# LucaAmbrogioni/Brancher

Measured on AMD Instinct MI355X. Metric: ELBO iters/sec at num_samples=300 per GPU (300-sample-equivalent iterations, whole job), higher is better.
Workload: dtype f32

## Files before the change

brancher_amd/csrc/bsvi_internal.h:

```cpp
#pragma once
#include <hip/hip_runtime.h>
#include <stdint.h>
#include <string>
#include <vector>

#include "bsvi.h"

int bsvi_fail(int code, const std::string& msg);
#define BSVI_CHECK_STRUCT(ptr, type)                                                                              \
    do {                                                                                                          \
        if ((ptr)->struct_size != sizeof(type))                                                                   \
            return bsvi_fail(BSVI_ERR_INVALID, std::string(#type "::struct_size is ") + std::to_string((ptr)->struct_size) + \
                             ", this library's sizeof is " + std::to_string(sizeof(type)) +                       \
                             ": the binding was written against another revision of include/bsvi.h");             \
    } while (0)
int bsvi_xgemm_nt(const uint16_t* X, const int32_t* rows, const uint16_t* Wp, long plane_stride, float* C, int ldc,
                  int M, int N, int Kp, void* stream);

int bsvi_xgemm_nt_t(const uint16_t* X, const int32_t* rows, const uint16_t* Wp, long plane_stride, float* Ct, int ldct,
                    int M, int N, int Kp, void* stream);
int bsvi_gemm_f32(int mode, const float* A, int lda, const float* B, int ldb, float* C, int ldc, int M, int N, int K, void* stream);

namespace bsvi_spec { struct Spec; }

struct bsvi_program {
    bsvi_program_desc d;
    void* dev_blob = nullptr;
    const uint4* code = nullptr;
    const uint4* aux = nullptr;
    const bsvi_record* records = nullptr;
    const bsvi_uniform_entry* uniform = nullptr;
    const float* consts = nullptr;
    const uint32_t* pu_ptr = nullptr;
    const uint32_t* pu_idx = nullptr;
    int max_lds = 0;
    bool generic = false;
    const bsvi_program* shares[8] = {};
    uint32_t n_shares = 0;
    bsvi_spec::Spec* spec = nullptr;
};

namespace bsvi_spec {

enum Mode { MODE_SUMS = 0, MODE_STEP = 1, MODE_LOOP = 2 };

Spec* create(const bsvi_program_desc& desc, std::string& why);
void destroy(Spec* s);
int upload(Spec* s);
const std::string& source(const Spec* s, int variant);
int compile(const std::string& src, std::vector<char>& code, std::string& log);
int obtain(const std::string& src, std::vector<char>& code, std::string& log, int* origin);
int last_origin();
std::string cache_directory();
std::string compiler_identity();
size_t workspace_bytes(const Spec* s, uint32_t n_local);
bool applies(const Spec* s, uint32_t n_local, int mode);
struct Launch {
    const bsvi_elbo_args* a = nullptr;
    int mode = MODE_SUMS;
    const bsvi_opt_cfg* cfg = nullptr;
    float* params = nullptr;
    float* state = nullptr;
    const uint8_t* mask = nullptr;
    const uint8_t* mask_first = nullptr;
    uint32_t pretraining_iterations = 0, n_iterations = 1;
    float* loss_slot = nullptr;
    float* finite_slot = nullptr;
    void* workspace = nullptr;
    const void* xchg = nullptr;
};
int launch(Spec* s, const bsvi_program* p, const Launch& L);
void geometry(const Spec* s, uint32_t n_local, int mode, uint32_t* n_blocks, uint32_t* n_threads, uint32_t* lds_bytes);

}

const void* bsvi_exchange_descriptor(bsvi_exchange* x, uint32_t n);
```

brancher_amd/csrc/elbo_kernel.hip:

```cpp
#include <hip/hip_runtime.h>
#include <stdint.h>
#include <stdio.h>
#include <stdlib.h>
#include <stdarg.h>
#include <string.h>
#include <mutex>
#include <type_traits>
#include <string>
#include <vector>

#include "bsvi.h"
#include "bsvi_device.h"
#include "bsvi_internal.h"

namespace bsvi {


struct KParams {
    const uint4* code;
    const uint4* aux;
    const bsvi_uniform_entry* uniform;
    const float* consts;
    const float* params;
    const float* obs;
// ... 1880 lines not shown
    for (uint32_t v = 0; v < n_shares; ++v) {
        if (!shares[v]) return fail(BSVI_ERR_INVALID, "null program share");
        if (shares[v]->d.n_uniform != p->d.n_uniform || shares[v]->d.n_uniform_grad != p->d.n_uniform_grad ||
            shares[v]->d.n_slots != p->d.n_slots || shares[v]->d.n_params != p->d.n_params ||
            shares[v]->d.n_code > p->d.n_code || (shares[v]->generic && !p->generic))
            return fail(BSVI_ERR_INVALID, "a program share does not match the program's tables");
    }
    for (uint32_t v = 0; v < n_shares; ++v) p->shares[v] = shares[v];
    p->n_shares = n_shares;
    return BSVI_OK;
}

extern "C" int bsvi_persistent_split_shares(const bsvi_program* p, uint32_t n_local) {
    if (!p || !n_local || !multi_persistent_applies(p, n_local)) return 1;
    if (p->spec && bsvi_spec::applies(p->spec, n_local, bsvi_spec::MODE_LOOP)) return 1;
    const char* e = getenv("BSVI_PERSISTENT_SHARES");
    const uint32_t waves = (n_local + 63) / 64;
    uint32_t want = e ? (uint32_t)atoi(e) : 2u;
    if (want > 8) want = 8;
    while (want > 1 && (waves * want > kMaxMultiWg || want == 5 || want == 7)) --want;
    return (int)(want < 1 ? 1 : want);
}

extern "C" int bsvi_train_persistent_split(const bsvi_program* p, const bsvi_program* const* shares, uint32_t n_shares,
                                           const bsvi_elbo_args* a, const bsvi_opt_cfg* cfg,
                                           float* params_dev, float* state_dev, const uint8_t* active_mask_dev,
                                           const uint8_t* active_mask_first_dev, uint32_t pretraining_iterations,
                                           uint32_t n_iterations, float* loss_curve_dev, float* finite_dev) {
    if (a) BSVI_CHECK_STRUCT(a, bsvi_elbo_args);
    if (!shares || n_shares < 2 || n_shares > 8) return fail(BSVI_ERR_INVALID, "2..8 program shares expected");
    for (uint32_t v = 0; v < n_shares; ++v) {
        if (!shares[v]) return fail(BSVI_ERR_INVALID, "null program share");
        if (shares[v]->d.n_uniform != p->d.n_uniform || shares[v]->d.n_uniform_grad != p->d.n_uniform_grad ||
            shares[v]->d.n_slots != p->d.n_slots || shares[v]->d.n_params != p->d.n_params ||
            shares[v]->d.n_code > p->d.n_code || (shares[v]->generic && !p->generic))
            return fail(BSVI_ERR_INVALID, "a program share does not match the program's tables");
    }
    return train_persistent_impl(p, shares, n_shares, a, cfg, params_dev, state_dev, active_mask_dev, active_mask_first_dev,
                                 pretraining_iterations, n_iterations, loss_curve_dev, finite_dev);
}

static int train_persistent_impl(const bsvi_program* p, const bsvi_program* const* shares, uint32_t n_shares,
                                 const bsvi_elbo_args* a, const bsvi_opt_cfg* cfg,
                                 float* params_dev, float* state_dev, const uint8_t* active_mask_dev,
                                 const uint8_t* active_mask_first_dev, uint32_t pretraining_iterations,
                                 uint32_t n_iterations, float* loss_curve_dev, float* finite_dev) {
    if (!p || !a) return fail(BSVI_ERR_INVALID, "null argument");
    int rc = check_cfg(cfg);
    if (rc) return rc;
    if (!a->out_dev || !params_dev || !active_mask_dev || !active_mask_first_dev || !loss_curve_dev || !finite_dev)
        return fail(BSVI_ERR_INVALID, "null argument");
    if (a->n_samples_local != a->n_samples_global) return fail(BSVI_ERR_INVALID, "persistent trainer is the single-GPU path");
    if (a->offset_dev) return fail(BSVI_ERR_INVALID, "the in-kernel training loop counts its own iterations: offset_dev must be null");
    {
        const int sp = try_spec(p, a, bsvi_spec::MODE_LOOP, cfg, params_dev, state_dev, active_mask_dev, active_mask_first_dev,
                                pretraining_iterations, n_iterations, loss_curve_dev, finite_dev);
        if (sp) return sp < 0 ? sp : BSVI_OK;
    }
    if (!state_dev) return fail(BSVI_ERR_INVALID, "state_dev is null and this call does not run on the specialised kernel");
    const bool multi = multi_persistent_applies(p, a->n_samples_local);
    Geometry g = choose_geometry(p, a->n_samples_local, true);
    if (multi && g.n_blocks != 1) {
        g = Geometry();
        g.n_waves = (a->n_samples_local + 63) / 64; g.n_blocks = 1; g.mode = SM_LACC; g.lpw = 64;
    }
    if (g.n_blocks != 1) return fail(BSVI_ERR_RESOURCE, "sample count does not fit one workgroup");
    PParams P;
    memset(&P, 0, sizeof(P));
    bsvi_elbo_args aa = *a;
    aa.params_dev = params_dev;
    rc = fill_kparams(p, &aa, g, P.K);
    if (rc) return rc;
    fill_rparams(p, g, P.K, params_dev, a->out_dev, P.R);
    P.R.state = state_dev; P.R.active_mask = active_mask_dev; P.R.cfg = *cfg; P.R.do_finalize = 1; P.R.do_step = 1;
    P.n_iterations = n_iterations; P.loss_curve = loss_curve_dev; P.finite_curve = finite_dev;
    P.active_mask_first = active_mask_first_dev; P.pretraining_iterations = pretraining_iterations;
    hipStream_t st = (hipStream_t)a->stream;
    if (shares && !multi) return fail(BSVI_ERR_INVALID, "program shares need the multi-workgroup trainer");
    if (multi) {
        const uint32_t sample_waves = g.n_waves;
        const uint32_t n_wg = sample_waves * (shares ? n_shares : 1u);
        if (n_wg > kMaxMultiWg) return fail(BSVI_ERR_INVALID, "too many workgroups for the exchange region");
        if (shares) {
            P.n_shares = n_shares;
            for (uint32_t v = 0; v < n_shares; ++v) {
                P.share_code[v] = shares[v]->code; P.share_aux[v] = shares[v]->aux; P.share_n_code[v] = shares[v]->d.n_code;
            }
        }
        Geometry g1 = g;
        g1.n_waves = 1; g1.n_blocks = n_wg;
        g1.stash = !p->generic && lds_need(p, 1, SM_LACC, 64, true) <= (size_t)p->max_lds;
        g1.lds_bytes = lds_need(p, 1, SM_LACC, 64, g1.stash);
        g1.n_pad = n_wg * 64;
        rc = fill_kparams(p, &aa, g1, P.K);
        if (rc) return rc;
        char* region = (char*)a->workspace_dev + base_ws_bytes(p, a->n_samples_local);
        P.mw_counter = (uint32_t*)region;
        P.mw_xchg = (float*)(region + 256);
        P.mw_params = P.mw_xchg + mw_xchg_floats(p);
        P.mw_stride = mw_stride(p);
        P.mw_state = P.mw_params + (size_t)(kMaxMultiWg - 1) * P.mw_stride;
        HIP_TRY(hipMemsetAsync(region, 0, 256 + mw_xchg_floats(p) * sizeof(float), st));
        dim3 mgrid(n_wg), mblock(64);
        if (p->generic) hipLaunchKernelGGL((persistent_multi_kernel<SM_LACC, true>), mgrid, mblock, g1.lds_bytes, st, P);
        else hipLaunchKernelGGL((persistent_multi_kernel<SM_LACC, false>), mgrid, mblock, g1.lds_bytes, st, P);
        HIP_TRY(hipGetLastError());
        return BSVI_OK;
    }
    dim3 grid(1), block(g.n_waves * 64);
#define BSVI_LAUNCH_P(SM_, GEN_) hipLaunchKernelGGL((persistent_kernel<SM_, GEN_>), grid, block, g.lds_bytes, st, P)
    if (p->generic) {
        if (g.mode == SM_LACC) BSVI_LAUNCH_P(SM_LACC, true); else if (g.mode == SM_ZG) BSVI_LAUNCH_P(SM_ZG, true); else BSVI_LAUNCH_P(SM_WSUM, true);
    } else {
        if (g.mode == SM_LACC) BSVI_LAUNCH_P(SM_LACC, false); else if (g.mode == SM_ZG) BSVI_LAUNCH_P(SM_ZG, false); else BSVI_LAUNCH_P(SM_WSUM, false);
    }
#undef BSVI_LAUNCH_P
    HIP_TRY(hipGetLastError());
    return BSVI_OK;
}

extern "C" size_t bsvi_program_source(const bsvi_program_desc* desc, int variant, char* buf, size_t capacity) {
    if (validate(desc) != BSVI_OK) return 0;
    std::string why;
    bsvi_spec::Spec* sp = bsvi_spec::create(*desc, why);
    if (!sp) { fail(BSVI_ERR_UNSUPPORTED, "program not specialised: " + why); return 0; }
    const std::string& src = bsvi_spec::source(sp, variant);
    const size_t need = src.size() + 1;
    if (buf && capacity >= need) memcpy(buf, src.c_str(), need);
    bsvi_spec::destroy(sp);
    return need;
}

extern "C" int bsvi_jit_compile(const char* source, size_t* code_bytes) {
    if (!source) return fail(BSVI_ERR_INVALID, "null source");
    std::vector<char> code;
    std::string log;
    const int rc = bsvi_spec::compile(source, code, log);
    if (rc) return fail(rc, log);
    if (code_bytes) *code_bytes = code.size();
    return BSVI_OK;
}

extern "C" int bsvi_jit_load(const char* source, size_t* code_bytes, int* origin) {
    if (!source) return fail(BSVI_ERR_INVALID, "null source");
    std::vector<char> code;
    std::string log;
    const int rc = bsvi_spec::obtain(source, code, log, origin);
    if (rc) return fail(rc, log);
    if (code_bytes) *code_bytes = code.size();
    return BSVI_OK;
}

extern "C" int bsvi_jit_last_origin(void) { return bsvi_spec::last_origin(); }

extern "C" size_t bsvi_jit_cache_dir(char* buf, size_t capacity) {
    const std::string dir = bsvi_spec::cache_directory();
    if (buf && capacity > dir.size()) memcpy(buf, dir.c_str(), dir.size() + 1);
    return dir.size() + 1;
}

extern "C" size_t bsvi_jit_compiler_identity(char* buf, size_t capacity) {
    const std::string id = bsvi_spec::compiler_identity();
    if (buf && capacity > id.size()) memcpy(buf, id.c_str(), id.size() + 1);
    return id.size() + 1;
}

extern "C" int bsvi_program_engine(const bsvi_program* p, uint32_t n_local, int mode, uint32_t* n_blocks, uint32_t* n_threads,
                                   uint32_t* lds_bytes) {
    if (!p) return 0;
    if (!p->spec || !bsvi_spec::applies(p->spec, n_local, mode)) return 0;
    bsvi_spec::geometry(p->spec, n_local, mode, n_blocks, n_threads, lds_bytes);
    return 1;
}

extern "C" int bsvi_max_lds_bytes(const bsvi_program* p) { return p ? p->max_lds : 0; }

extern "C" int bsvi_query_geometry(const bsvi_program* p, uint32_t n_local, uint32_t* n_blocks, uint32_t* n_waves,
                                   uint32_t* zglobal, uint64_t* lds_bytes) {
    if (!p) return fail(BSVI_ERR_INVALID, "null argument");
    Geometry g = choose_geometry(p, n_local, false);
    if (!g.n_blocks) return fail(BSVI_ERR_RESOURCE, "program does not fit the LDS budget");
    if (n_blocks) *n_blocks = g.n_blocks;
    if (n_waves) *n_waves = g.n_waves;
    if (zglobal) *zglobal = (uint32_t)g.mode | (g.lpw << 8);
    if (lds_bytes) *lds_bytes = g.lds_bytes;
    return BSVI_OK;
}

extern "C" int bsvi_debug_math(int fn, int dist, const float* x_dev, const float* p0_dev, const float* p1_dev,
                               float* out_dev, uint32_t n, void* stream) {
    if (!x_dev || !p0_dev || !p1_dev || !out_dev || !n) return fail(BSVI_ERR_INVALID, "null argument");
    hipLaunchKernelGGL(debug_math_kernel, dim3((n + 127) / 128), dim3(128), 0, (hipStream_t)stream, fn, dist, x_dev,
                       p0_dev, p1_dev, out_dev, n);
    HIP_TRY(hipGetLastError());
    return BSVI_OK;
}

#include "dense_kernel.inc"
#include "bnn_kernel.inc"

namespace bsvi {
__global__ void __launch_bounds__(256) minibatch_gather_kernel(const float* dataset, uint32_t DS, uint32_t row, uint32_t B, const int32_t* indices_in,
                                                                uint32_t seed_lo, uint32_t seed_hi, uint32_t off_lo, uint32_t off_hi, float* dst, int32_t* indices_out) {
    const uint32_t i = blockIdx.x * 256u + threadIdx.x;
    if (i >= B * row) return;
    const uint32_t b = i / row, e = i - b * row;
    DParams Dm;
    Dm.indices_in = indices_in; Dm.DS = DS;
    Dm.offset_lo = off_lo; Dm.offset_hi = off_hi; Dm.seed_lo = seed_lo; Dm.seed_hi = seed_hi;
    const uint32_t r = minibatch_index(Dm, b);
    dst[i] = dataset[(size_t)r * row + e];
    if (indices_out && e == 0u) indices_out[b] = (int32_t)r;
}
}

extern "C" int bsvi_minibatch_gather(const float* dataset_dev, uint32_t dataset_size, uint32_t row_floats, uint32_t batch_size,
                                     const int32_t* indices_dev, uint64_t seed, uint64_t offset, float* dst_dev, int32_t* indices_out_dev,
                                     void* stream) {
    if (!dataset_dev || !dst_dev || !dataset_size || !row_floats || !batch_size) return fail(BSVI_ERR_INVALID, "null argument");
    if (batch_size > dataset_size) return fail(BSVI_ERR_INVALID, "bsvi_minibatch_gather: batch_size exceeds dataset_size");
    if ((uint64_t)batch_size * row_floats >= (1ull << 31)) return fail(BSVI_ERR_RESOURCE, "bsvi_minibatch_gather: minibatch too large");
    const uint32_t n = batch_size * row_floats;
    hipLaunchKernelGGL(bsvi::minibatch_gather_kernel, dim3((n + 255) / 256), dim3(256), 0, (hipStream_t)stream, dataset_dev, dataset_size,
                       row_floats, batch_size, indices_dev, (uint32_t)seed, (uint32_t)(seed >> 32), (uint32_t)offset, (uint32_t)(offset >> 32),
                       dst_dev, indices_out_dev);
    HIP_TRY(hipGetLastError());
    return BSVI_OK;
}
```

brancher_amd/csrc/spec_main.h:

```cpp
#pragma once

namespace bsvi {

#if defined(__HIP_DEVICE_COMPILE__)
#define SPEC_CONST_AS __attribute__((address_space(4)))
#define SPEC_RELOAD_ARGS() asm volatile("" : "+s"(ka))
#else
#define SPEC_CONST_AS
#define SPEC_RELOAD_ARGS()
#endif

#define SPEC_TAB_PTR (4 * SPEC_N_UNIFORM)
#define SPEC_TAB_POS (SPEC_TAB_PTR + SPEC_N_PARAMS + 1)
#define SPEC_TAB_IDX (SPEC_TAB_POS + SPEC_N_POS)
#define SPEC_TAB_MASK (SPEC_TAB_IDX + SPEC_N_POS)

__device__ __forceinline__ void spec_lds_barrier() {
#if defined(__HIP_DEVICE_COMPILE__)
    asm volatile("s_waitcnt lgkmcnt(0)\n\ts_barrier" ::: "memory");
#endif
}

__device__ __noinline__ float spec_utransform_rare(uint32_t t, float x) { return utransform((int)t, x); }
__device__ __noinline__ float spec_utransform_grad_rare(uint32_t t, float x) { return utransform_grad((int)t, x); }
#ifndef SPEC_RARE_TRANSFORMS
#define SPEC_RARE_TRANSFORMS 1
#endif
#ifndef SPEC_UT_MASK
#define SPEC_UT_MASK 0xFFu
#endif
__device__ __forceinline__ float utransform_common(uint32_t t, float x) {
#if SPEC_RARE_TRANSFORMS
    if (t > BSVI_UT_SIGMOID) return spec_utransform_rare(t, x);
#endif
    const float soft = ((SPEC_UT_MASK >> BSVI_UT_SOFTPLUS) & 1u) ? softplusf_(x) : x;
    const float sig = ((SPEC_UT_MASK >> BSVI_UT_SIGMOID) & 1u) ? sigmoidf_(x) : x;
    return t == BSVI_UT_IDENTITY ? x : (t == BSVI_UT_SOFTPLUS ? soft : sig);
}
__device__ __forceinline__ float spec_utransform_grad(uint32_t t, float x) {
#if SPEC_RARE_TRANSFORMS
    if (t > BSVI_UT_SIGMOID) return spec_utransform_grad_rare(t, x);
#endif
    const float s = spec_rcp(1.0f + __expf(-x));
    const float soft = x > 20.0f ? 1.0f : s;
    return t == BSVI_UT_IDENTITY ? 1.0f : (t == BSVI_UT_SOFTPLUS ? soft : s * (1.0f - s));
}
__device__ __forceinline__ void spec_store_uniform(uint32_t k, float u) {
    spec_lds[k] = u;
    spec_lds[SPEC_OFF_UR + k] = spec_rcp(u);
    spec_lds[SPEC_OFF_UL + k] = spec_log(u);
}
__device__ __forceinline__ void spec_publish_uniform(const uint32_t* TAB, uint32_t k, float x) {
    const uint32_t w1 = TAB[4 * k + 1];
    spec_store_uniform(k, __uint_as_float(TAB[4 * k + 2]) + __uint_as_float(TAB[4 * k + 3]) * utransform_common(w1 & 0xFFu, x));
}

struct SpecOwn {
    float theta, s0, s1, s2, st;
    float a[2], b[2];
    uint32_t pos[2], k[2], tr[2];
    uint32_t n, mask;
    double p1, p2;
};
__device__ __forceinline__ void spec_own_store_products(spec_f4* row, const SpecOwn& o) {
    const unsigned long long a = __double_as_longlong(o.p1), b = __double_as_longlong(o.p2);
    row[4] = spec_f4{__uint_as_float((uint32_t)a), __uint_as_float((uint32_t)(a >> 32)), __uint_as_float((uint32_t)b), __uint_as_float((uint32_t)(b >> 32))};
}
__device__ __forceinline__ void spec_own_store(spec_f4* row, const SpecOwn& o) {
    row[0] = spec_f4{o.theta, o.s0, o.s1, o.s2};
    row[1] = spec_f4{o.st, o.a[0], o.b[0], o.a[1]};
    row[2] = spec_f4{o.b[1], __uint_as_float(o.pos[0]), __uint_as_float(o.pos[1]), __uint_as_float(o.k[0])};
    row[3] = spec_f4{__uint_as_float(o.k[1]), __uint_as_float(o.tr[0] | (o.tr[1] << 8) | (o.n << 16) | (o.mask << 24)), 0.0f, 0.0f};
    spec_own_store_products(row, o);
}
__device__ __forceinline__ SpecOwn spec_own_load(const spec_f4* row) {
    const spec_f4 q0 = row[0], q1 = row[1], q2 = row[2], q3 = row[3], q4 = row[4];
    SpecOwn o;
    o.p1 = __longlong_as_double((long long)(((unsigned long long)__float_as_uint(q4.y) << 32) | __float_as_uint(q4.x)));
    o.p2 = __longlong_as_double((long long)(((unsigned long long)__float_as_uint(q4.w) << 32) | __float_as_uint(q4.z)));
    o.theta = q0.x; o.s0 = q0.y; o.s1 = q0.z; o.s2 = q0.w;
    o.st = q1.x; o.a[0] = q1.y; o.b[0] = q1.z; o.a[1] = q1.w;
    o.b[1] = q2.x; o.pos[0] = __float_as_uint(q2.y); o.pos[1] = __float_as_uint(q2.z); o.k[0] = __float_as_uint(q2.w);
    o.k[1] = __float_as_uint(q3.x);
    const uint32_t meta = __float_as_uint(q3.y);
    o.tr[0] = meta & 0xFFu; o.tr[1] = (meta >> 8) & 0xFFu; o.n = (meta >> 16) & 0xFFu; o.mask = meta >> 24;
    return o;
}

#if defined(SPEC_WITH_EXCHANGE) && !SPEC_DIAG && !SPEC_ACCUMULATE_CHUNKS
#define SPEC_EXCHANGE 1
__device__ __forceinline__ unsigned long long* spec_xentry(unsigned char* region, uint32_t parity, uint32_t r, uint32_t capacity, uint32_t world) {
    return reinterpret_cast<unsigned long long*>(region + XCHG_HEADER_WORDS * 4 + (size_t)2 * world * capacity * 4) + ((size_t)parity * world + r) * capacity;
}
__device__ __forceinline__ void spec_xput(const SpecExchange* xg, uint32_t seq, uint32_t k, float v) {
    const uint32_t world = xg->world, rank = xg->rank, cap = xg->capacity, parity = seq & 1u;
    const unsigned long long e = ((unsigned long long)seq << 32) | __float_as_uint(v);
    for (uint32_t p = 0; p < world; ++p)
        __hip_atomic_store(spec_xentry(xg->peer[p], parity, rank, cap, world) + k, e, __ATOMIC_RELAXED, __HIP_MEMORY_SCOPE_SYSTEM);
}
__device__ __forceinline__ bool spec_xget(const SpecExchange* xg, uint32_t seq, uint32_t k, float& v) {
    const uint32_t world = xg->world, rank = xg->rank, cap = xg->capacity, parity = seq & 1u;
    unsigned char* const region = xg->peer[rank];
    uint32_t* const abort_word = reinterpret_cast<uint32_t*>(region) + XCHG_MAX_RANKS * XCHG_FLAG_STRIDE;
    unsigned long long t0 = 0;
    for (uint32_t round = 0;; ++round) {
        unsigned long long e[XCHG_MAX_RANKS];
#pragma unroll
        for (uint32_t r = 0; r < XCHG_MAX_RANKS; ++r) {
            e[r] = (unsigned long long)seq << 32;
            if (r < world) e[r] = __hip_atomic_load(spec_xentry(region, parity, r, cap, world) + k, __ATOMIC_RELAXED, __HIP_MEMORY_SCOPE_SYSTEM);
        }
        bool all = true;
        float t = 0.0f;
#pragma unroll
        for (uint32_t r = 0; r < XCHG_MAX_RANKS; ++r) {
            all = all && (uint32_t)(e[r] >> 32) == seq;
            if (r < world) t += __uint_as_float((uint32_t)e[r]);
        }
        if (all) {
            v = t;
            return __hip_atomic_load(abort_word, __ATOMIC_RELAXED, __HIP_MEMORY_SCOPE_SYSTEM) == 0u;
        }
        if (round == 0u) t0 = wall_clock64();
        if (__hip_atomic_load(abort_word, __ATOMIC_RELAXED, __HIP_MEMORY_SCOPE_SYSTEM) != 0u) return false;
        if (wall_clock64() - t0 > xg->timeout_ticks) {
            for (uint32_t p = 0; p < world; ++p)
                __hip_atomic_store(reinterpret_cast<uint32_t*>(xg->peer[p]) + XCHG_MAX_RANKS * XCHG_FLAG_STRIDE, seq, __ATOMIC_RELAXED, __HIP_MEMORY_SCOPE_SYSTEM);
            return false;
        }
        __builtin_amdgcn_s_sleep(1);
    }
}
#if !SPEC_GENERIC_OWNERS
__device__ __forceinline__ bool spec_exchange(const SpecExchange* xg, uint32_t seq, uint32_t l, bool has_param, float& vs, float& vb, float& gsum) {
    const uint32_t world = xg->world, rank = xg->rank, cap = xg->capacity, parity = seq & 1u;
    uint32_t* const abort_word = reinterpret_cast<uint32_t*>(xg->peer[rank]) + XCHG_MAX_RANKS * XCHG_FLAG_STRIDE;
    const uint32_t aborted = __hip_atomic_load(abort_word, __ATOMIC_RELAXED, __HIP_MEMORY_SCOPE_SYSTEM);
    const unsigned long long tag = (unsigned long long)seq << 32;
    for (uint32_t p = 0; p < world; ++p) {
        unsigned long long* const row = spec_xentry(xg->peer[p], parity, rank, cap, world);
        if (l == 0u) {
            __hip_atomic_store(row, tag | __float_as_uint(vs), __ATOMIC_RELAXED, __HIP_MEMORY_SCOPE_SYSTEM);
            __hip_atomic_store(row + 1, tag | __float_as_uint(vb), __ATOMIC_RELAXED, __HIP_MEMORY_SCOPE_SYSTEM);
        }
        if (has_param) __hip_atomic_store(row + BSVI_OUT_HEADER + l, tag | __float_as_uint(gsum), __ATOMIC_RELAXED, __HIP_MEMORY_SCOPE_SYSTEM);
    }
    unsigned char* const region = xg->peer[rank];
    unsigned long long t0 = 0;
    bool gave_up = false;
    float ts, tb, tg;
    for (uint32_t round = 0;; ++round) {
        unsigned long long e0[XCHG_MAX_RANKS], e1[XCHG_MAX_RANKS], eg[XCHG_MAX_RANKS];
#pragma unroll
        for (uint32_t r = 0; r < XCHG_MAX_RANKS; ++r) {
            e0[r] = e1[r] = eg[r] = tag;
            if (r < world) {
                const unsigned long long* const row = spec_xentry(region, parity, r, cap, world);
                e0[r] = __hip_atomic_load(row, __ATOMIC_RELAXED, __HIP_MEMORY_SCOPE_SYSTEM);
                e1[r] = __hip_atomic_load(row + 1, __ATOMIC_RELAXED, __HIP_MEMORY_SCOPE_SYSTEM);
                if (has_param) eg[r] = __hip_atomic_load(row + BSVI_OUT_HEADER + l, __ATOMIC_RELAXED, __HIP_MEMORY_SCOPE_SYSTEM);
            }
        }
        bool all = true;
        ts = 0.0f; tb = 0.0f; tg = 0.0f;
#pragma unroll
        for (uint32_t r = 0; r < XCHG_MAX_RANKS; ++r) {
            all = all && (uint32_t)(e0[r] >> 32) == seq && (uint32_t)(e1[r] >> 32) == seq && (uint32_t)(eg[r] >> 32) == seq;
            if (r < world) { ts += __uint_as_float((uint32_t)e0[r]); tb += __uint_as_float((uint32_t)e1[r]); tg += __uint_as_float((uint32_t)eg[r]); }
        }
        if (__all((int)all)) break;
        if (round == 0u) t0 = wall_clock64();
        if (__hip_atomic_load(abort_word, __ATOMIC_RELAXED, __HIP_MEMORY_SCOPE_SYSTEM) != 0u) { gave_up = true; break; }
        if (wall_clock64() - t0 > xg->timeout_ticks) {
            gave_up = true;
            if (l < world) __hip_atomic_store(reinterpret_cast<uint32_t*>(xg->peer[l]) + XCHG_MAX_RANKS * XCHG_FLAG_STRIDE, seq, __ATOMIC_RELAXED, __HIP_MEMORY_SCOPE_SYSTEM);
            if (l == 0u) atomicAdd(abort_word + 1, 1u);
            break;
        }
        __builtin_amdgcn_s_sleep(1);
    }
    if (gave_up || aborted != 0u) return false;
    vs = ts; vb = tb; gsum = tg;
    return true;
}
#endif
#else
#define SPEC_EXCHANGE 0
#endif

#if defined(SPEC_WAVES_PER_EU)
#define SPEC_VGPR_ATTR __attribute__((amdgpu_waves_per_eu(SPEC_WAVES_PER_EU, SPEC_WAVES_PER_EU)))
#elif defined(SPEC_NUM_VGPR)
#define SPEC_VGPR_ATTR __attribute__((amdgpu_num_vgpr(SPEC_NUM_VGPR)))
#else
#define SPEC_VGPR_ATTR
#endif
#ifndef SPEC_BOUND_THREADS
#define SPEC_BOUND_THREADS SPEC_MAX_THREADS
#endif
extern "C" __global__ void __launch_bounds__(SPEC_BOUND_THREADS) SPEC_VGPR_ATTR bsvi_spec_kernel(const SpecArgs A_unused) {
    (void)A_unused;
    const SPEC_CONST_AS char* ka = (const SPEC_CONST_AS char*)__builtin_amdgcn_kernarg_segment_ptr();
#define SPEC_A ((const SPEC_CONST_AS SpecArgs*)ka)
    const uint32_t tid = threadIdx.x, nthreads = blockDim.x, W = nthreads >> 6, wave = tid >> 6, lane = tid & 63u;
    const uint32_t G = gridDim.x;
    float* const WS = spec_lds + SPEC_OFF_WS;
    float* const RED = spec_lds + SPEC_OFF_RED;
    float* const PS = spec_lds + SPEC_OFF_PS;
    uint32_t* const TAB = reinterpret_cast<uint32_t*>(spec_lds + SPEC_OFF_TAB);
    float* const WSw = WS + wave * SPEC_WS_PAD;

    SpecLane T;
    T.lane = lane;
    T.n = blockIdx.x * nthreads + tid;
    T.active = false; T.nc = 0; T.nidx = 0;
    T.vz = T.n >> 31;
    T.tile = wave * SPEC_TR_FLOATS + lane;
    const uint32_t sample_base = SPEC_A->sample_base;
    const uint32_t n_chunks = (SPEC_A->n_local + G * nthreads - 1u) / (G * nthreads);
    const uint32_t mode = SPEC_A->mode;
    const bool step = mode != SPEC_MODE_SUMS;
    const uint32_t n_it = (mode == SPEC_MODE_LOOP) ? SPEC_A->n_iterations : 1u;

    {
        const uint32_t* uniform = reinterpret_cast<const uint32_t*>(SPEC_A->uniform);
        const uint32_t* pu_ptr = SPEC_A->pu_ptr;
        const uint32_t* pu_pos = SPEC_A->pu_pos;
        const uint32_t* pu_idx = SPEC_A->pu_idx;
        const float* obs = SPEC_A->obs;
        const float* params = SPEC_A->params;
        const float* state = SPEC_A->state;
        const uint8_t* mask = SPEC_A->mask;
        const uint8_t* mask_first = SPEC_A->mask_first;
        const bool h_uni = tid < 4u * SPEC_N_UNIFORM, h_ptr = tid < SPEC_N_PARAMS + 1u, h_pos = tid < SPEC_N_POS,
                   h_obs = tid < SPEC_N_OBS, h_par = tid < SPEC_N_PARAMS;
        uint32_t r_uni = 0, r_ptr = 0, r_pos = 0, r_idx = 0, r_mask = 0;
        float r_obs = 0.0f, r_par = 0.0f, r_st[4] = {0.0f, 0.0f, 0.0f, 0.0f};
        const bool h_uni2 = tid + nthreads < 4u * SPEC_N_UNIFORM;
        uint32_t r_uni2 = 0;
        if (h_uni) r_uni = uniform[tid];
        if (h_uni2) r_uni2 = uniform[tid + nthreads];
        if (h_ptr) r_ptr = pu_ptr[tid];
        if (h_pos) { r_pos = pu_pos[tid]; r_idx = pu_idx[tid]; }
        if (h_obs) r_obs = obs[tid];
        if (h_par) {
            r_par = params[tid];
            if (step) {
                if (state) {
#pragma unroll
                    for (uint32_t s = 0; s < 4u; ++s) r_st[s] = state[(size_t)s * SPEC_N_PARAMS + tid];
                }
                r_mask = (mask[tid] ? 1u : 0u) | (mask_first[tid] ? 2u : 0u);
            }
        }
        asm volatile("" ::: "memory");
        if (h_uni) TAB[tid] = r_uni;
        if (h_uni2) TAB[tid + nthreads] = r_uni2;
        if (h_ptr) TAB[SPEC_TAB_PTR + tid] = r_ptr;
        if (h_pos) { TAB[SPEC_TAB_POS + tid] = r_pos; TAB[SPEC_TAB_IDX + tid] = r_idx; }
        if (h_obs) spec_lds[SPEC_N_UNIFORM + tid] = r_obs;
        if (h_par) {
            PS[tid] = r_par;
            if (step) {
#pragma unroll
                for (uint32_t s = 0; s < 4u; ++s) PS[(1u + s) * SPEC_NP_PAD + tid] = r_st[s];
                TAB[SPEC_TAB_MASK + tid] = r_mask;
            }
        }
        for (uint32_t i = tid + 2u * nthreads; i < 4u * SPEC_N_UNIFORM; i += nthreads) TAB[i] = uniform[i];
        for (uint32_t i = tid + nthreads; i < SPEC_N_PARAMS + 1u; i += nthreads) TAB[SPEC_TAB_PTR + i] = pu_ptr[i];
        for (uint32_t j = tid + nthreads; j < SPEC_N_POS; j += nthreads) { TAB[SPEC_TAB_POS + j] = pu_pos[j]; TAB[SPEC_TAB_IDX + j] = pu_idx[j]; }
        for (uint32_t i = tid + nthreads; i < SPEC_N_OBS; i += nthreads) spec_lds[SPEC_N_UNIFORM + i] = obs[i];
        for (uint32_t i = tid + nthreads; i < SPEC_N_PARAMS; i += nthreads) {
            PS[i] = params[i];
            if (step) {
#pragma unroll
                for (uint32_t s = 0; s < 4u; ++s)
                    PS[(1u + s) * SPEC_NP_PAD + i] = state ? state[(size_t)s * SPEC_N_PARAMS + i] : 0.0f;
                TAB[SPEC_TAB_MASK + i] = (mask[i] ? 1u : 0u) | (mask_first[i] ? 2u : 0u);
            }
        }
        __syncthreads();
        const float* consts = SPEC_A->consts;
        for (uint32_t k = tid; k < SPEC_N_UNIFORM; k += nthreads) {
            const uint32_t src = TAB[4 * k], w1 = TAB[4 * k + 1];
            spec_publish_uniform(TAB, k, ((w1 >> 8) & 0xFFu) ? PS[src] : consts[src]);
        }
    }

    spec_f4* const OWN = reinterpret_cast<spec_f4*>(spec_lds + SPEC_OFF_OWN);
#ifndef SPEC_OWNER_WAVE
#define SPEC_OWNER_WAVE 1u
#endif
#if SPEC_TILE && SPEC_KEEP_NOISE && SPEC_KEEP_NOISE <= 68 && !SPEC_GENERIC_OWNERS && !SPEC_DIAG && !SPEC_ACCUMULATE_CHUNKS \
    && !defined(SPEC_DEBUG_NO_DRAW) && !defined(SPEC_NO_EARLY_DRAW) && !defined(SPEC_DEBUG_LATE_FREE) && defined(SPEC_WITH_DRAW_WAVE)
#define SPEC_DRAW_WAVE 1
    const uint32_t WSN = (SPEC_A->n_local + 63u) / 64u;
    const bool has_draw_wave = mode == SPEC_MODE_LOOP && G == 1u && W >= 2u && WSN < W;
    const uint32_t fed_index = W == 2u ? 0u : 1u;
    const bool draw_service = has_draw_wave && W - WSN >= 3u;
    const bool draw_wave = __builtin_amdgcn_readfirstlane((has_draw_wave && (draw_service ? wave >= WSN : wave == W - 1u)) ? 1 : 0) != 0;
    const bool fed_wave = __builtin_amdgcn_readfirstlane((has_draw_wave && (draw_service ? wave < WSN : wave == fed_index)) ? 1 : 0) != 0;
    float* const NZ = spec_lds + SPEC_OFF_TR + (draw_service ? WSN * SPEC_TR_FLOATS + wave * (SPEC_KEEP_NOISE * 64u) : (W - 1u) * SPEC_TR_FLOATS) + lane;
    float* const NZB = spec_lds + SPEC_OFF_TR + WSN * SPEC_TR_FLOATS + lane;
    if (draw_wave) for (uint32_t k = lane; k < SPEC_WS_PAD; k += 64u) WSw[k] = 0.0f;
#else
#define SPEC_DRAW_WAVE 0
    const bool has_draw_wave = false, draw_wave = false, fed_wave = false;
    const uint32_t fed_index = 1u;
#endif
#if SPEC_DRAW_WAVE && defined(SPEC_WITH_DRAW_OWNERS) && !SPEC_EXCHANGE
#define SPEC_DRAW_OWNERS 1
    const uint32_t own_wave = WSN + ((1u - WSN) & 3u);
#else
#define SPEC_DRAW_OWNERS 0
#endif
#if SPEC_DRAW_OWNERS
    const uint32_t own_base = own_wave * 64u;
#else
    const uint32_t own_base = has_draw_wave ? fed_index * 64u
                            : (!SPEC_GENERIC_OWNERS && SPEC_OWNER_WAVE * 64u + SPEC_N_PARAMS <= nthreads) ? SPEC_OWNER_WAVE * 64u : 0u;
#endif
    const uint32_t oid = tid - own_base;
    bool own_fast = false;
#if SPEC_DRAW_OWNERS
    SpecOwn own = {};
#endif
    if (oid < SPEC_N_PARAMS) {
        const uint32_t j0 = TAB[SPEC_TAB_PTR + oid], j1 = TAB[SPEC_TAB_PTR + oid + 1];
        if (j1 - j0 <= 2u) {
            own_fast = true;
#if !SPEC_DRAW_OWNERS
            SpecOwn own;
#endif
            own.n = j1 - j0;
            own.mask = 0;
            own.theta = PS[oid];
            own.s0 = own.s1 = own.s2 = own.st = 0.0f;
            own.p1 = own.p2 = 1.0;
            own.a[0] = own.a[1] = own.b[0] = own.b[1] = 0.0f;
            own.pos[0] = own.pos[1] = own.k[0] = own.k[1] = own.tr[0] = own.tr[1] = 0;
            if (step) {
                own.s0 = PS[SPEC_NP_PAD + oid]; own.s1 = PS[2 * SPEC_NP_PAD + oid];
                own.s2 = PS[3 * SPEC_NP_PAD + oid]; own.st = PS[4 * SPEC_NP_PAD + oid];
                own.mask = TAB[SPEC_TAB_MASK + oid];
                const bsvi_opt_cfg cfg0 = SPEC_A->cfg;
                if (cfg0.kind != BSVI_OPT_SGD && own.st != 0.0f) {
                    own.p1 = pow((double)cfg0.beta1, (double)own.st);
                    own.p2 = pow((double)cfg0.beta2, (double)own.st);
                }
            }
#pragma unroll
            for (uint32_t e = 0; e < 2u; ++e) {
                if (e < own.n) {
                    const uint32_t k = TAB[SPEC_TAB_IDX + j0 + e];
                    own.pos[e] = TAB[SPEC_TAB_POS + j0 + e];
                    own.k[e] = k;
                    own.tr[e] = TAB[4 * k + 1] & 0xFFu;
                    own.a[e] = __uint_as_float(TAB[4 * k + 2]);
                    own.b[e] = __uint_as_float(TAB[4 * k + 3]);
                }
            }
#if !SPEC_DRAW_OWNERS
            spec_own_store(OWN + 5 * oid, own);
#endif
        }
    }

    SPEC_RELOAD_ARGS();
    SpecBody B0;
    B0.n_local = SPEC_A->n_local;
    B0.seed_lo = SPEC_A->seed_lo;
    B0.seed_hi = SPEC_A->seed_hi;
#if SPEC_DIAG
    B0.noise = SPEC_A->noise;
    B0.samples_out = SPEC_A->samples_out;
    B0.noise_out = SPEC_A->noise_out;
    B0.fvalue_out = SPEC_A->fvalue_out;
    B0.f_weight = SPEC_A->f_weight;
    B0.q_weight = SPEC_A->q_weight;
#else
    B0.noise = nullptr; B0.samples_out = nullptr; B0.noise_out = nullptr; B0.fvalue_out = nullptr;
    B0.f_weight = nullptr; B0.q_weight = nullptr;
#endif
    unsigned long long off0 = ((unsigned long long)SPEC_A->offset_hi << 32) | SPEC_A->offset_lo;
    if (const unsigned long long* const offset_dev = SPEC_A->offset_dev) off0 += *offset_dev;
    const uint32_t n_global = SPEC_A->n_global;
    const uint32_t pretraining = SPEC_A->pretraining_iterations;
#if SPEC_ACCUMULATE_CHUNKS
#define SPEC_LOOP_MANY 1
#define SPEC_GEN_OVER 0x7fff0000u
    const unsigned int gen0 = 0;
    if (G > 1 && mode == SPEC_MODE_LOOP && blockIdx.x != 0 &&
        __hip_atomic_load(SPEC_A->ticket + 64, __ATOMIC_RELAXED, __HIP_MEMORY_SCOPE_AGENT) >= SPEC_GEN_OVER) return;
#else
#define SPEC_LOOP_MANY 0
#endif
#if SPEC_EXCHANGE
    uint32_t xseq0 = 0;
    if (const SpecExchange* const xg0 = SPEC_A->xchg) xseq0 = reinterpret_cast<const uint32_t*>(xg0->peer[xg0->rank])[XCHG_CALLS_WORD + 1];
#endif

#if defined(SPEC_DEBUG_STAMPS)
    unsigned long long stamp[12] = {0, 0, 0, 0, 0, 0, 0, 0, 0, 0, 0, 0};
#define SPEC_STAMP(i) if (it == n_it / 2) stamp[i] = __builtin_amdgcn_s_memtime()
    unsigned long long rstamp[6] = {0, 0, 0, 0, 0, 0};
#define SPEC_RSTAMP(i) if (it == n_it / 2) rstamp[i] = __builtin_amdgcn_s_memtime()
#define SPEC_RSTAMP_NEXT() if (it == n_it / 2 + 1u) rstamp[5] = __builtin_amdgcn_s_memtime()
#define SPEC_RSTAMP_WRITE()                                                                                              \
    if (lane == 0u && SPEC_A->loss_slot && n_it > 16u + 8u * SPEC_MAX_WAVES) {                                           \
        asm volatile("s_waitcnt vmcnt(0)" ::: "memory");                                                                 \
        for (int i = 1; i < 6; ++i) SPEC_A->loss_slot[16u + 8u * wave + i] = (float)(rstamp[i] - rstamp[0]);               \
        SPEC_A->loss_slot[16u + 8u * wave] = 1.0f;                                                                       \
    }
#else
#define SPEC_STAMP(i)
#define SPEC_RSTAMP(i)
#define SPEC_RSTAMP_NEXT()
#define SPEC_RSTAMP_WRITE()
#endif
#if SPEC_KEEP_NOISE && !SPEC_DIAG && !SPEC_ACCUMULATE_CHUNKS && !defined(SPEC_DEBUG_NO_DRAW) && !defined(SPEC_NO_EARLY_DRAW)
#define SPEC_EARLY_DRAW 1
    SpecNoise Z;
    bool noise_ready = false;
#else
#define SPEC_EARLY_DRAW 0
#endif
#if SPEC_DRAW_WAVE
    if (draw_service && draw_wave) {
        if (lane == 0u) { RED[8 + 2 * wave] = 0.0f; RED[9 + 2 * wave] = 0.0f; }
        const uint32_t n_draw = W - WSN, k = wave - WSN;
        const uint32_t first = k;
        uint32_t before = 0;
        for (uint32_t j = 0; j < k; ++j) before += (((WSN + j) & 3u) != 1u) ? 1u : 0u;
        const uint32_t second = n_draw + before;
        const bool has_first = first < WSN, has_second = (wave & 3u) != 1u && second < WSN;
        auto draw_for = [&](uint32_t target, unsigned long long offn, SpecNoise& Zd) {
            SpecLane Tn = T;
            Tn.n = target * 64u + lane;
            Tn.active = Tn.n < B0.n_local;
            Tn.nc = Tn.active ? Tn.n : (B0.n_local - 1u);
            Tn.nidx = sample_base + Tn.nc;
            Tn.off_lo = (uint32_t)offn;
            Tn.off_hi = (uint32_t)(offn >> 32);
            Tn.vz = T.vz;
            spec_draw(B0, Tn, Zd);
        };
#if SPEC_DRAW_OWNERS
        (void)has_first; (void)has_second;
        const uint32_t kown = own_wave - WSN, n_other = n_draw - 1u, rest = WSN - 1u;
        const uint32_t j = k < kown ? k : k - 1u, per = rest / n_other, extra = rest % n_other;
        const uint32_t set_a = __builtin_amdgcn_readfirstlane(1u + j * per + (j < extra ? j : extra));
        const uint32_t n_sets = __builtin_amdgcn_readfirstlane(per + (j < extra ? 1u : 0u));
        const bool owners = __builtin_amdgcn_readfirstlane(wave == own_wave ? 1 : 0) != 0;
        for (uint32_t it = 0; it < n_it; ++it) {
            const bool more = it + 1u < n_it, last = !more;
            spec_lds_barrier();
            SPEC_RSTAMP(0);
            SPEC_RSTAMP_NEXT();
            SpecNoise Za, Zb;
            float fac[2] = {0.0f, 0.0f};
            AdamBias bias = {1.0, 1.0, 0.0f, 0.0f};
            if (owners) {
                SPEC_RELOAD_ARGS();
                const bsvi_opt_cfg cfg = SPEC_A->cfg;
#pragma unroll
                for (uint32_t e = 0; e < 2u; ++e) fac[e] = own.b[e] * spec_utransform_grad(own.tr[e], own.theta);
                if (cfg.kind != BSVI_OPT_SGD) bias = optimizer_adam_bias(cfg, own.p1, own.p2);
                if (more) {
                    draw_for(0u, off0 + it + 1u, Za);
                    float* const buf = NZB + (((it + 1u) & 1u) ? WSN * (SPEC_KEEP_NOISE * 64u) : 0u);
#pragma unroll
                    for (uint32_t r = 0; r < SPEC_KEEP_NOISE; ++r) buf[64u * r] = Za.z[r];
                }
            } else if (more) {
                draw_for(set_a, off0 + it + 1u, Za);
                if (n_sets > 1u) draw_for(set_a + 1u, off0 + it + 1u, Zb);
            }
            SPEC_RSTAMP(1);
            spec_lds_barrier();
            SPEC_RSTAMP(2);
            if (owners) {
                SPEC_RELOAD_ARGS();
                float* const out = SPEC_A->out;
                float* const loss_slot = SPEC_A->loss_slot;
                float* const finite_slot = SPEC_A->finite_slot;
                const bsvi_opt_cfg cfg = SPEC_A->cfg;
                float vs = 0.0f, vb = 0.0f;
#pragma unroll
                for (uint32_t w = 0; w < SPEC_MAX_WAVES; ++w) {
                    const float a = RED[8 + 2 * w], b = RED[9 + 2 * w];
                    vs += w < W ? a : 0.0f;
                    vb += w < W ? b : 0.0f;
                }
                float tot[2];
#pragma unroll
                for (uint32_t e = 0; e < 2u; ++e) tot[e] = spec_pos_total(WS, own.pos[e], W);
                const float finite = isfinite(vs) ? 1.0f : 0.0f;
                const float loss = -vs / (float)n_global;
                if (oid == 0u) {
                    if (last) { out[0] = vs; out[1] = vb; out[2] = loss; out[3] = finite; }
                    if (loss_slot) loss_slot[it] = loss;
                    if (finite_slot) finite_slot[it] = finite;
                }
                const float scale = -1.0f / (float)n_global;
                const uint32_t mask_bit = it <= pretraining ? 2u : 1u;
                if (own_fast) {
                    float gsum = 0.0f;
#pragma unroll
                    for (uint32_t e = 0; e < 2u; ++e) {
                        const float term = tot[e] * fac[e];
                        gsum += e < own.n ? term : 0.0f;
                    }
                    const float grad = gsum * scale;
                    SPEC_RSTAMP(3);
                    if (last) out[BSVI_OUT_HEADER + oid] = grad;
                    if (finite != 0.0f && (own.mask & mask_bit)) {
                        if (cfg.kind == BSVI_OPT_SGD) {
                            optimizer_apply(cfg, own.theta, own.s0, own.s1, own.s2, own.st, grad);
                        } else {
                            optimizer_apply_adam_biased(cfg, own.theta, own.s0, own.s1, own.s2, own.st, grad, bias);
                            own.p1 = bias.p1;
                            own.p2 = bias.p2;
                        }
                    }
                    if (last) {
                        float* const params = SPEC_A->params;
                        float* const state = SPEC_A->state;
                        params[oid] = own.theta;
                        if (state) {
                            state[oid] = own.s0;
                            state[(size_t)SPEC_N_PARAMS + oid] = own.s1;
                            state[2 * (size_t)SPEC_N_PARAMS + oid] = own.s2;
                            state[3 * (size_t)SPEC_N_PARAMS + oid] = own.st;
                        }
                    } else {
                        const float g0 = utransform_common(own.tr[0], own.theta);
                        float g1 = g0;
                        if (own.n == 2u && own.tr[1] != own.tr[0]) g1 = utransform_common(own.tr[1], own.theta);
                        if (own.n > 0u) spec_store_uniform(own.k[0], own.a[0] + own.b[0] * g0);
                        if (own.n > 1u) spec_store_uniform(own.k[1], own.a[1] + own.b[1] * g1);
                    }
                }
            } else if (more) {
#pragma unroll
                for (uint32_t r = 0; r < SPEC_KEEP_NOISE; ++r) NZB[set_a * (SPEC_KEEP_NOISE * 64u) + 64u * r] = Za.z[r];
                if (n_sets > 1u) {
#pragma unroll
                    for (uint32_t r = 0; r < SPEC_KEEP_NOISE; ++r) NZB[(set_a + 1u) * (SPEC_KEEP_NOISE * 64u) + 64u * r] = Zb.z[r];
                }
            }
            SPEC_RSTAMP(4);
        }
        SPEC_RSTAMP_WRITE();
        return;
#else
        for (uint32_t it = 0; it < n_it; ++it) {
            const bool more = it + 1u < n_it;
            spec_lds_barrier();
            SPEC_RSTAMP(0);
            SPEC_RSTAMP_NEXT();
            SpecNoise Za;
            if (more && has_first) draw_for(first, off0 + it + 1u, Za);
            SPEC_RSTAMP(1);
            spec_lds_barrier();
            SPEC_RSTAMP(2);
            if (more) {
                if (has_first) {
#pragma unroll
                    for (uint32_t r = 0; r < SPEC_KEEP_NOISE; ++r) NZB[first * (SPEC_KEEP_NOISE * 64u) + 64u * r] = Za.z[r];
                }
                if (has_second) {
                    SpecNoise Zb;
                    draw_for(second, off0 + it + 1u, Zb);
#pragma unroll
                    for (uint32_t r = 0; r < SPEC_KEEP_NOISE; ++r) NZB[second * (SPEC_KEEP_NOISE * 64u) + 64u * r] = Zb.z[r];
                }
            }
            SPEC_RSTAMP(4);
        }
        SPEC_RSTAMP_WRITE();
        return;
#endif
    }
#endif
    for (uint32_t it = 0; it < n_it; ++it) {
        SPEC_STAMP(0);
        float lane_value = 0.0f, lane_bad = 0.0f;
        for (uint32_t chunk = 0; chunk < n_chunks; ++chunk) {
            SpecBody B = B0;
#if SPEC_DIAG
            if (B.noise) B.noise += (size_t)it * SPEC_N_NOISE * B.n_local;
#endif
            T.n = (chunk * G + blockIdx.x) * nthreads + tid;
            T.active = T.n < B.n_local;
            T.nc = T.active ? T.n : (B.n_local - 1u);
            T.nidx = sample_base + T.nc;
            const unsigned long long off = off0 + it;
            T.f = 0.0f;
            T.lq = 0.0f;
#if SPEC_DIAG
            T.gw = B.f_weight ? B.f_weight[T.nc] : 1.0f;
#else
            T.gw = 1.0f;
#endif
            T.off_lo = (uint32_t)off;
            T.off_hi = (uint32_t)(off >> 32);
#if !SPEC_EARLY_DRAW
            SpecNoise Z;
#endif
#if defined(SPEC_DEBUG_NO_DRAW)
            for (uint32_t r = 0; r < (SPEC_KEEP_NOISE ? SPEC_KEEP_NOISE : 1); ++r) Z.z[r] = 0.25f;
#elif SPEC_EARLY_DRAW
#if defined(SPEC_DEBUG_LATE_FREE)
            if (!noise_ready && (!((SPEC_DEBUG_LATE_FREE >> wave) & 1u) || it == 0u)) spec_draw(B, T, Z);
#else
            if (!noise_ready && !draw_wave && !(fed_wave && it > 0u)) spec_draw(B, T, Z);
#endif
#else
            spec_draw(B, T, Z);
#endif
            SPEC_STAMP(1);
            if (chunk == 0) {
                spec_lds_barrier();
                SPEC_RSTAMP(0);
                SPEC_RSTAMP_NEXT();
#if SPEC_ACCUMULATE_CHUNKS
                for (uint32_t k = lane; k < SPEC_WS_CELLS; k += 64u) WSw[k] = 0.0f;
#endif
            }
#if SPEC_DRAW_WAVE
            if (fed_wave && it > 0u) {
#if SPEC_DRAW_OWNERS
                const float* const nz = NZ + ((wave == 0u && (it & 1u)) ? WSN * (SPEC_KEEP_NOISE * 64u) : 0u);
#else
                const float* const nz = NZ;
#endif
#pragma unroll
                for (uint32_t r = 0; r < SPEC_KEEP_NOISE; ++r) Z.z[r] = nz[64u * r];
            }
#endif
            SPEC_STAMP(2);
#if !defined(SPEC_DEBUG_NO_BODY)
            if (!draw_wave) {
                spec_body(B, T, Z, WSw);
#if SPEC_TILE
                spec_du_flush(spec_lds + SPEC_OFF_TR + wave * SPEC_TR_FLOATS, WSw, lane);
#endif
            }
#endif
            SPEC_STAMP(3);
            const float value = (SPEC_ESTIMATOR == BSVI_EST_BLACKBOX) ? (T.lq * T.f + T.f) : T.f;
            lane_value += T.active ? value : 0.0f;
            lane_bad += (T.active && !isfinite(value)) ? 1.0f : 0.0f;
        }
        const float vsum = wave_sum(lane_value);
        const float bad = wave_sum(lane_bad);
        if (lane == 0) { RED[8 + 2 * wave] = vsum; RED[9 + 2 * wave] = bad; }
        SPEC_STAMP(4);
#if SPEC_EARLY_DRAW
        noise_ready = false;
#ifndef SPEC_EARLY_MASK
#define SPEC_EARLY_MASK (1u | (1u << SPEC_OWNER_WAVE))
#endif
#if defined(SPEC_DEBUG_LATE_FREE)
        if (((SPEC_EARLY_MASK >> wave) & 1u) && !((SPEC_DEBUG_LATE_FREE >> wave) & 1u) && n_chunks == 1u && it + 1u < n_it) {
#else
        if (((SPEC_EARLY_MASK >> wave) & 1u) && !has_draw_wave && n_chunks == 1u && it + 1u < n_it) {
#endif
            const unsigned long long off = off0 + it + 1u;
            SpecLane Tn = T;
            Tn.off_lo = (uint32_t)off;
            Tn.off_hi = (uint32_t)(off >> 32);
            spec_draw(B0, Tn, Z);
            noise_ready = true;
        }
#endif
        SPEC_RSTAMP(1);
        spec_lds_barrier();
        SPEC_STAMP(5);
        SPEC_RSTAMP(2);
#if SPEC_DRAW_OWNERS
        SPEC_RSTAMP(4);
        continue;
#endif
#if SPEC_DRAW_WAVE
        if (draw_wave && it + 1u < n_it) {
            const unsigned long long off = off0 + it + 1u;
            SpecLane Tn = T;
            Tn.n = fed_index * 64u + lane;
            Tn.active = Tn.n < B0.n_local;
            Tn.nc = Tn.active ? Tn.n : (B0.n_local - 1u);
            Tn.nidx = sample_base + Tn.nc;
            Tn.off_lo = (uint32_t)off;
            Tn.off_hi = (uint32_t)(off >> 32);
            SpecNoise Zf;
            spec_draw(B0, Tn, Zf);
#pragma unroll
            for (uint32_t r = 0; r < SPEC_KEEP_NOISE; ++r) NZ[64u * r] = Zf.z[r];
        }
#endif

        uint32_t rows = W;
        if (G > 1) {
            SPEC_RELOAD_ARGS();
            float* const partials = SPEC_A->partials;
            unsigned int* const ticket = SPEC_A->ticket;
            const uint32_t stride = 2u + SPEC_N_POS;
            float* mine = partials + (size_t)blockIdx.x * stride;
            for (uint32_t k = tid; k < SPEC_N_POS; k += nthreads) mine[2 + k] = spec_pos_total(WS, k, W);
            if (tid == 0) {
                float s = 0.0f, c = 0.0f;
                for (uint32_t w = 0; w < W; ++w) { s += RED[8 + 2 * w]; c += RED[9 + 2 * w]; }
                mine[0] = s;
                mine[1] = c;
            }
            __syncthreads();
#if SPEC_LOOP_MANY
            if (mode == SPEC_MODE_LOOP) {
                unsigned int* const gen = ticket + 64;
                const unsigned int target = gen0 + it + 1u;
                if (blockIdx.x != 0) {
                    if (tid == 0) {
                        __hip_atomic_fetch_add(ticket, 1u, __ATOMIC_RELEASE, __HIP_MEMORY_SCOPE_AGENT);
                        const unsigned long long t0 = wall_clock64();
                        unsigned int seen;
                        bool over = false;
                        while ((int)((seen = __hip_atomic_load(gen, __ATOMIC_ACQUIRE, __HIP_MEMORY_SCOPE_AGENT)) - target) < 0) {
                            if (wall_clock64() - t0 > 400000000ull) { over = true; break; }
                            __builtin_amdgcn_s_sleep(2);
                        }
                        RED[3] = (over || seen >= SPEC_GEN_OVER) ? 1.0f : 0.0f;
                    }
                    __syncthreads();
                    if (RED[3] != 0.0f) return;
                    if (it + 1u == n_it) return;
                    float* const params = SPEC_A->params;
                    for (uint32_t i = tid; i < SPEC_N_PARAMS; i += nthreads)
                        PS[i] = __hip_atomic_load(params + i, __ATOMIC_RELAXED, __HIP_MEMORY_SCOPE_AGENT);
                    __syncthreads();
                    const float* const consts = SPEC_A->consts;
                    (void)consts;
                    for (uint32_t k = tid; k < SPEC_N_UNIFORM; k += nthreads) {
                        const uint32_t src = TAB[4 * k], w1 = TAB[4 * k + 1];
                        if ((w1 >> 8) & 0xFFu) spec_publish_uniform(TAB, k, PS[src]);
                    }
                    continue;
                }
                if (tid == 0) {
                    const unsigned long long t0 = wall_clock64();
                    bool late = false;
                    while (__hip_atomic_load(ticket, __ATOMIC_ACQUIRE, __HIP_MEMORY_SCOPE_AGENT) != G - 1u) {
                        if (wall_clock64() - t0 > 400000000ull) { late = true; break; }
                        __builtin_amdgcn_s_sleep(2);
                    }
                    RED[3] = late ? 1.0f : 0.0f;
                }
                __syncthreads();
                if (RED[3] != 0.0f) {
                    SPEC_RELOAD_ARGS();
                    float* const loss_slot = SPEC_A->loss_slot;
                    float* const finite_slot = SPEC_A->finite_slot;
                    float* const out = SPEC_A->out;
                    const float nanv = __int_as_float(0x7fc00000);
                    for (uint32_t k = it + tid; k < n_it; k += nthreads) {
                        if (loss_slot) loss_slot[k] = nanv;
                        if (finite_slot) finite_slot[k] = 0.0f;
                    }
                    if (tid == 0) {
                        out[0] = nanv; out[1] = 1.0f; out[2] = nanv; out[3] = 0.0f;
                        __hip_atomic_store(ticket, 0u, __ATOMIC_RELAXED, __HIP_MEMORY_SCOPE_AGENT);
                        __hip_atomic_store(gen, SPEC_GEN_OVER, __ATOMIC_RELEASE, __HIP_MEMORY_SCOPE_AGENT);
                    }
                    return;
                }
            } else
#endif
            {
                if (tid == 0) {
                    const unsigned int t = __hip_atomic_fetch_add(ticket, 1u, __ATOMIC_ACQ_REL, __HIP_MEMORY_SCOPE_AGENT);
                    RED[2] = (t == G - 1u) ? 1.0f : 0.0f;
                }
                __syncthreads();
                if (RED[2] == 0.0f) return;
            }
            float* const SL = spec_lds + SPEC_OFF_SCR;
            for (uint32_t i = tid; i < 4u * stride; i += nthreads) {
                const uint32_t sl = i & 3u, c = i >> 2;
                float s = 0.0f;
                uint32_t b = sl;
                for (; b + 28u < G; b += 32u) {
                    float v[8];
#pragma unroll
                    for (uint32_t u = 0; u < 8u; ++u)
                        v[u] = __hip_atomic_load(&partials[(size_t)(b + 4u * u) * stride + c], __ATOMIC_RELAXED, __HIP_MEMORY_SCOPE_AGENT);
#pragma unroll
                    for (uint32_t u = 0; u < 8u; ++u) s += v[u];
                }
                for (; b < G; b += 4u)
                    s += __hip_atomic_load(&partials[(size_t)b * stride + c], __ATOMIC_RELAXED, __HIP_MEMORY_SCOPE_AGENT);
                SL[i] = s;
            }
            __syncthreads();
            for (uint32_t c = tid; c < stride; c += nthreads) {
                const float s = (SL[4 * c] + SL[4 * c + 1]) + (SL[4 * c + 2] + SL[4 * c + 3]);
                if (c < 2u) {
                    RED[8 + c] = s;
                } else {
                    WS[SPEC_WS_CELL(c - 2u)] = s;
#if !SPEC_TILE
                    WS[4u * (c - 2u) + 1u] = 0.0f; WS[4u * (c - 2u) + 2u] = 0.0f; WS[4u * (c - 2u) + 3u] = 0.0f;
#endif
                }
            }
            if (tid == 0) {
                __hip_atomic_store(ticket, 0u, __ATOMIC_RELAXED, __HIP_MEMORY_SCOPE_AGENT);
            }
            __syncthreads();
            rows = 1;
        }

        SPEC_RELOAD_ARGS();
        float* const out = SPEC_A->out;
        float* const loss_slot = SPEC_A->loss_slot;
        float* const finite_slot = SPEC_A->finite_slot;
        const bsvi_opt_cfg cfg = SPEC_A->cfg;
        float vs = 0.0f, vb = 0.0f;
#pragma unroll
        for (uint32_t w = 0; w < SPEC_MAX_WAVES; ++w) {
            const float a = RED[8 + 2 * w], b = RED[9 + 2 * w];
            vs += w < rows ? a : 0.0f;
            vb += w < rows ? b : 0.0f;
        }
#if SPEC_EXCHANGE
        const SpecExchange* const xg = SPEC_A->xchg;
#if SPEC_GENERIC_OWNERS
        const bool xrun = xg != nullptr && mode == SPEC_MODE_LOOP;
        float xgsum = 0.0f;
        if (xrun) {
            const uint32_t xseq = xseq0 + it + 1u;
            if (tid == own_base) { spec_xput(xg, xseq, 0u, vs); spec_xput(xg, xseq, 1u, vb); }
            if (own_fast) {
                const SpecOwn own = spec_own_load(OWN + 5 * oid);
                float g = 0.0f;
#pragma unroll
                for (uint32_t e = 0; e < 2u; ++e) {
                    const float term = spec_pos_total(WS, own.pos[e], rows) * (own.b[e] * spec_utransform_grad(own.tr[e], own.theta));
                    g += e < own.n ? term : 0.0f;
                }
                spec_xput(xg, xseq, BSVI_OUT_HEADER + oid, g);
            }
            for (uint32_t i = tid; i < SPEC_N_PARAMS; i += nthreads) {
                if (i == oid && own_fast) continue;
                const float theta = PS[i];
                const uint32_t j0 = TAB[SPEC_TAB_PTR + i], j1 = TAB[SPEC_TAB_PTR + i + 1];
                float g = 0.0f;
                for (uint32_t j = j0; j < j1; ++j) {
                    const uint32_t pos = TAB[SPEC_TAB_POS + j], k = TAB[SPEC_TAB_IDX + j];
                    g += spec_pos_total(WS, pos, rows) * (__uint_as_float(TAB[4 * k + 3]) * spec_utransform_grad(TAB[4 * k + 1] & 0xFFu, theta));
                }
                spec_xput(xg, xseq, BSVI_OUT_HEADER + i, g);
            }
            bool ok = spec_xget(xg, xseq, 0u, vs);
            ok = spec_xget(xg, xseq, 1u, vb) && ok;
            if (own_fast) ok = spec_xget(xg, xseq, BSVI_OUT_HEADER + oid, xgsum) && ok;
            if (!ok) vs = __int_as_float(0x7fc00000);
            if (tid == own_base && it + 1u == n_it) reinterpret_cast<uint32_t*>(xg->peer[xg->rank])[XCHG_CALLS_WORD + 1] = xseq0 + n_it;
        }
#else
        const bool xrun = xg != nullptr && mode == SPEC_MODE_LOOP && (tid >> 6) == (own_base >> 6);
        float xgsum = 0.0f;
        if (xrun) {
            if (own_fast) {
                const SpecOwn own = spec_own_load(OWN + 5 * oid);
                float tot[2];
#pragma unroll
                for (uint32_t e = 0; e < 2u; ++e) tot[e] = spec_pos_total(WS, own.pos[e], rows);
#pragma unroll
                for (uint32_t e = 0; e < 2u; ++e) {
                    const float term = tot[e] * (own.b[e] * spec_utransform_grad(own.tr[e], own.theta));
                    xgsum += e < own.n ? term : 0.0f;
                }
            }
            if (!spec_exchange(xg, xseq0 + it + 1u, oid, own_fast, vs, vb, xgsum)) vs = __int_as_float(0x7fc00000);
            if (oid == 0u && it + 1u == n_it) reinterpret_cast<uint32_t*>(xg->peer[xg->rank])[XCHG_CALLS_WORD + 1] = xseq0 + n_it;
        }
#endif
#endif
        const float finite = isfinite(vs) ? 1.0f : 0.0f;
        const float loss = -vs / (float)n_global;
        SPEC_STAMP(7);
        if (tid == own_base) {
            if (it + 1u == n_it) { out[0] = vs; out[1] = vb; }
            if (step) {
                if (it + 1u == n_it) { out[2] = loss; out[3] = finite; }
                if (loss_slot) loss_slot[it] = loss;
                if (finite_slot) finite_slot[it] = finite;
            }
        }
        const float scale = step ? -1.0f / (float)n_global : 1.0f;
        const bool last = it + 1u == n_it;
        const uint32_t mask_bit = (mode == SPEC_MODE_LOOP && it <= pretraining) ? 2u : 1u;
        if (own_fast) {
            SpecOwn own = spec_own_load(OWN + 5 * oid);
            float tot[2];
#pragma unroll
            for (uint32_t e = 0; e < 2u; ++e) tot[e] = spec_pos_total(WS, own.pos[e], rows);
            float gsum = 0.0f;
#pragma unroll
            for (uint32_t e = 0; e < 2u; ++e) {
                const float term = tot[e] * (own.b[e] * spec_utransform_grad(own.tr[e], own.theta));
                gsum += e < own.n ? term : 0.0f;
            }
#if SPEC_EXCHANGE
            if (xrun) gsum = xgsum;
#endif
            const float grad = gsum * scale;
            SPEC_STAMP(8);
            SPEC_RSTAMP(3);
            if (last || !step) out[BSVI_OUT_HEADER + oid] = grad;
            if (step) {
                if (finite != 0.0f && (own.mask & mask_bit))
                    optimizer_apply_running(cfg, own.theta, own.s0, own.s1, own.s2, own.st, grad, own.p1, own.p2);
                SPEC_STAMP(9);
#if SPEC_LOOP_MANY
                if (G > 1 && !last) __hip_atomic_store(SPEC_A->params + oid, own.theta, __ATOMIC_RELAXED, __HIP_MEMORY_SCOPE_AGENT);
#endif
                if (last) {
                    float* const params = SPEC_A->params;
                    float* const state = SPEC_A->state;
                    params[oid] = own.theta;
                    if (state) {
                        state[oid] = own.s0;
                        state[(size_t)SPEC_N_PARAMS + oid] = own.s1;
                        state[2 * (size_t)SPEC_N_PARAMS + oid] = own.s2;
                        state[3 * (size_t)SPEC_N_PARAMS + oid] = own.st;
                    }
                } else {
#pragma unroll
                    for (uint32_t e = 0; e < 2u; ++e)
                        if (e < own.n) spec_store_uniform(own.k[e], own.a[e] + own.b[e] * utransform_common(own.tr[e], own.theta));
                    OWN[5 * oid] = spec_f4{own.theta, own.s0, own.s1, own.s2};
                    spec_lds[SPEC_OFF_OWN + SPEC_OWN_WORDS * oid + 4] = own.st;
                    if (cfg.kind != BSVI_OPT_SGD) spec_own_store_products(OWN + 5 * oid, own);
                }
            }
        }
#if SPEC_GENERIC_OWNERS
        for (uint32_t i = tid; i < SPEC_N_PARAMS; i += nthreads) {
            if (i == oid && own_fast) continue;
            const float theta = PS[i];
            const uint32_t j0 = TAB[SPEC_TAB_PTR + i], j1 = TAB[SPEC_TAB_PTR + i + 1];
            float gsum = 0.0f;
            for (uint32_t j = j0; j < j1; ++j) {
                const uint32_t pos = TAB[SPEC_TAB_POS + j], k = TAB[SPEC_TAB_IDX + j];
                gsum += spec_pos_total(WS, pos, rows) * (__uint_as_float(TAB[4 * k + 3]) * spec_utransform_grad(TAB[4 * k + 1] & 0xFFu, theta));
            }
#if SPEC_EXCHANGE
            bool xok = true;
            if (xrun) xok = spec_xget(xg, xseq0 + it + 1u, BSVI_OUT_HEADER + i, gsum);
#else
            const bool xok = true;
#endif
            const float grad = gsum * scale;
            if (last || !step) out[BSVI_OUT_HEADER + i] = grad;
            if (step && xok && finite != 0.0f && (TAB[SPEC_TAB_MASK + i] & mask_bit))
                optimizer_update(cfg, PS, PS + SPEC_NP_PAD, SPEC_NP_PAD, i, grad);
            if (!step) continue;
            if (last) {
                float* const params = SPEC_A->params;
                float* const state = SPEC_A->state;
                params[i] = PS[i];
                if (state) {
#pragma unroll
                    for (uint32_t s = 0; s < 4u; ++s) state[(size_t)s * SPEC_N_PARAMS + i] = PS[(1u + s) * SPEC_NP_PAD + i];
                }
            } else {
                const float theta2 = PS[i];
                for (uint32_t j = j0; j < j1; ++j) spec_publish_uniform(TAB, TAB[SPEC_TAB_IDX + j], theta2);
#if SPEC_LOOP_MANY
                if (G > 1) __hip_atomic_store(SPEC_A->params + i, theta2, __ATOMIC_RELAXED, __HIP_MEMORY_SCOPE_AGENT);
#endif
            }
        }
#endif
#if SPEC_LOOP_MANY
        if (G > 1 && mode == SPEC_MODE_LOOP) {
            __threadfence();
            __syncthreads();
            if (tid == 0) __hip_atomic_store(SPEC_A->ticket + 64, gen0 + it + 1u, __ATOMIC_RELEASE, __HIP_MEMORY_SCOPE_AGENT);
        }
#endif
        SPEC_STAMP(6);
        SPEC_RSTAMP(4);
    }
    SPEC_RSTAMP_WRITE();
#if defined(SPEC_DEBUG_STAMPS)
    float* const loss_slot = SPEC_A->loss_slot;
    if (tid == 0 && loss_slot && n_it > 16) {
        asm volatile("s_waitcnt vmcnt(0)" ::: "memory");
        for (int i = 1; i < 12; ++i) loss_slot[i] = (float)(stamp[i] - stamp[0]);
    }
#endif
#undef SPEC_A
}

}
```

brancher_amd/csrc/spec_prelude.h:

```cpp
#pragma once
#include "bsvi_device.h"
#include "spec_args.h"

namespace bsvi {

struct SpecBody {
    const float* noise;
    float* samples_out;
    float* noise_out;
    float* fvalue_out;
    const float* f_weight;
    const float* q_weight;
    uint32_t n_local, seed_lo, seed_hi;
};

struct SpecLane {
    float f, lq;
    float gw;
    uint32_t n, nc;
    uint32_t nidx;
    uint32_t lane;
    uint32_t off_lo, off_hi;
    uint32_t vz;
    uint32_t tile;
    bool active;
};

#ifndef SPEC_KEEP_NOISE
#define SPEC_KEEP_NOISE 0
#endif
struct SpecNoise { float z[SPEC_KEEP_NOISE ? SPEC_KEEP_NOISE : 1]; };

__device__ __forceinline__ float spec_log(float x) { return __builtin_amdgcn_logf(x) * 0.6931471805599453f; }
__device__ __forceinline__ float spec_rcp(float x) { return __builtin_amdgcn_rcpf(x); }

__device__ __forceinline__ float spec_naff_lp(float v, float loc, float rS, float lS) {
    const float u = (v - loc) * rS;
    return -0.5f * (u * u) - lS - kLogSqrt2Pi;
}
__device__ __forceinline__ void spec_naff_sink(float w, float v, float loc, float rS, float lS, float& f, float& gloc, float& gS) {
    const float u = (v - loc) * rS;
    f += w * (-0.5f * (u * u) - lS - kLogSqrt2Pi);
    gloc = w * u * rS;
    gS = w * (u * u - 1.0f) * rS;
}
__device__ __forceinline__ void spec_naff_lp_bwd(float gw, float v, float loc, float rS, float& gv, float& gloc, float& gS) {
    const float d = v - loc, t = d * (rS * rS);
    gv = -gw * t;
    gloc = gw * t;
    gS = gw * (d * t * rS - rS);
}

__device__ __forceinline__ void spec_normals4(const SpecBody& A, const SpecLane& T, uint32_t g,
                                              float& z0, float& z1, float& z2, float& z3) {
    const u32x4 x = philox4x32(T.nidx, g | 0x80000000u, T.off_lo, T.off_hi, A.seed_lo, A.seed_hi);
    box_muller_fast(x.x, x.y, z0, z1);
    box_muller_fast(x.z, x.w, z2, z3);
}
__device__ __forceinline__ uint32_t spec_opaque(uint32_t x) {
#if defined(__HIP_DEVICE_COMPILE__)
    asm volatile("" : "+s"(x));
#endif
    return x;
}
__device__ __forceinline__ PhiloxKey spec_key(const SpecBody& A, const SpecLane& T) {
    return PhiloxKey{T.nidx, A.seed_lo, A.seed_hi, T.off_lo, T.off_hi};
}

#ifndef SPEC_GENERIC_OWNERS
#define SPEC_GENERIC_OWNERS 1
#endif
#ifndef SPEC_ACCUMULATE_CHUNKS
#define SPEC_ACCUMULATE_CHUNKS 0
#endif
#define SPEC_MAX_WAVES (SPEC_MAX_THREADS / 64)
#define SPEC_U_PAD ((SPEC_N_UNIFORM + SPEC_N_OBS + 3) / 4 * 4)
#define SPEC_NU_PAD ((SPEC_N_UNIFORM + 3) / 4 * 4)
#ifndef SPEC_TILE
#define SPEC_TILE 0
#endif
#if SPEC_TILE
#define SPEC_WS_PAD ((SPEC_N_POS + 3) / 4 * 4 + 4)
#define SPEC_TR_STRIDE 68
#define SPEC_TR_FLOATS (64 * SPEC_TR_STRIDE)
#else
#define SPEC_WS_PAD (4 * SPEC_N_POS + 4)
#define SPEC_TR_FLOATS 0
#endif
#define SPEC_RED_FLOATS (2 * SPEC_MAX_WAVES + 8)
#define SPEC_NP_PAD ((SPEC_N_PARAMS + 3) / 4 * 4 + 4)
#define SPEC_TAB_WORDS ((4 * SPEC_N_UNIFORM + (2 * SPEC_N_PARAMS + 1) + 2 * SPEC_N_POS + 3) / 4 * 4 + 4)
#define SPEC_SCR_FLOATS (4 * (SPEC_N_POS + 2) + 4)
#define SPEC_OFF_UR SPEC_U_PAD
#define SPEC_OFF_UL (SPEC_OFF_UR + SPEC_NU_PAD)
#define SPEC_OFF_WS (SPEC_OFF_UL + SPEC_NU_PAD)
#define SPEC_OFF_RED (SPEC_OFF_WS + SPEC_MAX_WAVES * SPEC_WS_PAD)
#define SPEC_OFF_PS (SPEC_OFF_RED + SPEC_RED_FLOATS)
#define SPEC_OFF_TAB (SPEC_OFF_PS + 5 * SPEC_NP_PAD)
#define SPEC_OWN_ROWS (SPEC_N_PARAMS < SPEC_MAX_THREADS ? SPEC_N_PARAMS : SPEC_MAX_THREADS)
#define SPEC_OFF_OWN (SPEC_OFF_TAB + SPEC_TAB_WORDS)
#define SPEC_OWN_WORDS 20
#define SPEC_OFF_SCR (SPEC_OFF_OWN + SPEC_OWN_WORDS * SPEC_OWN_ROWS)
#define SPEC_OFF_TR (SPEC_OFF_SCR + SPEC_SCR_FLOATS)
#define SPEC_LDS_FLOATS (SPEC_OFF_TR + SPEC_MAX_WAVES * SPEC_TR_FLOATS)
__shared__ __attribute__((aligned(16))) float spec_lds[SPEC_LDS_FLOATS];

#define SPEC_U(k) spec_lds[(k) + T.vz]
#define SPEC_UR(k) spec_lds[SPEC_OFF_UR + (k) + T.vz]
#define SPEC_UL(k) spec_lds[SPEC_OFF_UL + (k) + T.vz]

typedef float spec_f4 __attribute__((ext_vector_type(4)));

__device__ __forceinline__ float spec_row_sum(float x) {
    x += dpp_f<0xB1>(x);
    x += dpp_f<0x4E>(x);
    x += dpp_f<0x141>(x);
    x += dpp_f<0x140>(x);
    return x;
}
#if SPEC_TILE
#define SPEC_DU(pos, val) spec_lds[SPEC_OFF_TR + T.tile + (pos) * SPEC_TR_STRIDE] = T.active ? (val) : 0.0f
__device__ __forceinline__ void spec_du_flush(const float* TRw, float* WSw, uint32_t lane) {
    asm volatile("s_waitcnt lgkmcnt(0)" ::: "memory");
    if (lane < SPEC_N_POS) {
        const spec_f4* row = reinterpret_cast<const spec_f4*>(TRw + lane * SPEC_TR_STRIDE);
        spec_f4 s = row[0];
#pragma unroll
        for (uint32_t q = 1; q < 16u; ++q) s += row[q];
        const float t = (s.x + s.y) + (s.z + s.w);
#if SPEC_ACCUMULATE_CHUNKS
        WSw[lane] += t;
#else
        WSw[lane] = t;
#endif
    }
    asm volatile("s_waitcnt lgkmcnt(0)" ::: "memory");
}
#elif SPEC_ACCUMULATE_CHUNKS
#define SPEC_DU(pos, val) { float* const c_ = WSw + 4u * (pos) + (T.lane >> 4); *c_ = *c_ + spec_row_sum(T.active ? (val) : 0.0f); }
#else
#define SPEC_DU(pos, val) WSw[4u * (pos) + (T.lane >> 4)] = spec_row_sum(T.active ? (val) : 0.0f)
#endif
#if SPEC_TILE
#define SPEC_WS_CELLS SPEC_N_POS
#define SPEC_WS_CELL(pos) (pos)
#else
#define SPEC_WS_CELLS (4u * SPEC_N_POS)
#define SPEC_WS_CELL(pos) (4u * (pos))
#endif
__device__ __forceinline__ float spec_pos_total(const float* WS, uint32_t pos, uint32_t rows) {
    float s = 0.0f;
#pragma unroll
    for (uint32_t w = 0; w < SPEC_MAX_WAVES; ++w) {
#if SPEC_TILE
        const float t = WS[w * SPEC_WS_PAD + pos];
#else
        const spec_f4 q = *reinterpret_cast<const spec_f4*>(WS + w * SPEC_WS_PAD + 4u * pos);
        const float t = (q.x + q.y) + (q.z + q.w);
#endif
        s += w < rows ? t : 0.0f;
    }
    return s;
}

}
```

brancher_amd/csrc/specialize.cpp:

```cpp
#include <hip/hip_runtime.h>
#include <hip/hiprtc.h>
#include <math.h>
#include <stdarg.h>
#include <stdio.h>
#include <stdlib.h>
#include <string.h>
#include <dlfcn.h>
#include <errno.h>
#include <fcntl.h>
#include <link.h>
#include <sys/stat.h>
#include <sys/types.h>
#include <unistd.h>

#include <algorithm>
#include <map>
#include <mutex>
#include <set>
#include <string>
#include <vector>

#include "bsvi.h"
#include "bsvi_internal.h"
#include "spec_args.h"
#include "jit_headers.inc"

namespace bsvi_spec {

using bsvi::SpecArgs;

namespace {

struct Insn { uint32_t w0, dst, a, b, c, s, imm0, imm1; };

constexpr size_t kMaxVisits = 12000;
constexpr uint32_t kKeepEpsRows = 64;
constexpr uint32_t kRescheduleAboveSlots = 40;
constexpr uint32_t kFenceAboveCode = 100;
constexpr const char* kJitOptionMark = "// bsvi-jit-option: ";
constexpr uint32_t kFenceEvery = 4;
constexpr uint32_t kBasicRegallocAboveCode = 700;
constexpr uint32_t kAccumulateEntries = 1u << 30;

std::string fmt(const char* f, ...) {
    char buf[512];
    va_list ap;
    va_start(ap, f);
    vsnprintf(buf, sizeof buf, f, ap);
    va_end(ap);
    return buf;
}

std::string flit(uint32_t bits) {
    float x;
    memcpy(&x, &bits, 4);
    if (!isfinite(x)) return fmt("__uint_as_float(0x%08xu)", bits);
    if (x == (float)(long long)x && fabsf(x) < 1e6f) return fmt("%.1ff", (double)x);
    return fmt("%.9gf", (double)x);
}

class Emitter {
public:
    Emitter(const bsvi_program_desc& d, bool diag) : d_(d), diag_(diag) {
        keep_eps_ = d.n_noise <= kKeepEpsRows;
        direct_du_ = d.n_uniform_grad > kAccumulateEntries;
        reschedule_ = d.n_slots > kRescheduleAboveSlots;
        for (uint32_t pc = 0; pc < d.n_code; ++pc) {
            const Insn I = insn(pc);
            const uint32_t op = I.w0 & 0xFFu;
            if ((op == BSVI_OP_NAFF || op == BSVI_OP_NODE) && (((I.w0 >> 8) & 0xFFu) & BSVI_F_WF) && d.estimator != BSVI_EST_BLACKBOX) reschedule_ = false;
        }
        two_pass_ = reschedule_ && d.estimator == BSVI_EST_BLACKBOX && !(getenv("BSVI_SPEC_TWO_PASS") && getenv("BSVI_SPEC_TWO_PASS")[0] == '0');
        if (d.estimator == BSVI_EST_BLACKBOX && !two_pass_) reschedule_ = false;
        du_total_.assign(d.n_uniform_grad, 0);
        du_seen_.assign(d.n_uniform_grad, 0);
    }

    bool run(std::string& why) {
        counting_ = true;
        walk();
        if (visits_ > kMaxVisits) { why = fmt("unrolled stream has %zu instruction visits (limit %zu)", visits_, kMaxVisits); return false; }
        counting_ = false;
        body_.clear();
        fwd_groups_.clear(); rev_groups_.clear(); node_rows_.clear();
        walk();
        for (uint32_t k = 0; k < d_.n_uniform_grad; ++k)
            if (!du_total_[k]) complete(k, "0.0f");
        return true;
    }

    const std::string& body() const { return body_; }
    bool keeps_noise() const { return keep_eps_; }
    std::string draw() const {
        std::string s;
        if (!keep_eps_) return s;
        std::set<uint32_t> groups;
        for (uint32_t r : normal_rows_) groups.insert(r >> 2);
        std::string philox;
        for (uint32_t g : groups) {
            philox += fmt("        { float z0, z1, z2, z3; spec_normals4(A, T, %uu, z0, z1, z2, z3);", g);
            for (uint32_t j = 0; j < 4; ++j)
                if (normal_rows_.count(4 * g + j)) philox += fmt(" Z.z[%u] = z%u;", 4 * g + j, j);
            philox += " }\n";
        }
        if (!diag_) return "    {\n" + philox + "    }\n";
        s += "    if (A.noise) {\n";
        for (uint32_t r : normal_rows_) s += fmt("        Z.z[%u] = A.noise[(size_t)%uu * A.n_local + T.nc];\n", r, r);
        s += "    } else {\n" + philox + "    }\n";
        return s;
    }
    const std::vector<uint32_t>& order() const { return order_; }
    std::string declarations() const {
        std::string s;
        for (uint32_t i = 0; i < d_.n_slots; ++i) s += fmt("    float v_%u = 0.0f, a_%u = 0.0f;\n", i, i);
        if (!direct_du_) for (uint32_t k = 0; k < d_.n_uniform_grad; ++k) if (du_total_[k]) s += fmt("    float du_%u = 0.0f;\n", k);
        for (uint32_t g : all_groups_) s += fmt("    float pn_%u_0 = 0.0f, pn_%u_1 = 0.0f, pn_%u_2 = 0.0f, pn_%u_3 = 0.0f;\n", g, g, g, g);
        for (uint32_t r : eps_rows_) s += fmt("    float ez_%u = 0.0f;\n", r);
        for (uint32_t r : all_node_rows_) s += fmt("    float ns_%u = 0.0f;\n", r);
        return s;
    }

private:
    const bsvi_program_desc& d_;
    bool diag_;
    bool keep_eps_ = true, counting_ = true, direct_du_ = false, reschedule_ = true, two_pass_ = false;
    int sink_mode_ = 0;
    size_t visits_ = 0;
    std::string body_;
    std::vector<uint32_t> du_total_, du_seen_, order_;
    std::set<uint32_t> fwd_groups_, rev_groups_, all_groups_, eps_rows_, node_rows_, all_node_rows_, normal_rows_;

    Insn insn(uint32_t pc) const {
        Insn I;
        memcpy(&I, d_.code + 8 * (size_t)pc, 32);
        return I;
    }
    void line(const std::string& s) { if (!counting_) { body_ += "    "; body_ += s; body_ += "\n"; } }

    struct Opnd { bool lane; uint32_t idx; };
    static Opnd resolve(uint32_t o, uint32_t e) {
        const bool lane = o >> 31;
        const uint32_t step = ((o >> 30) & 1u) * (lane ? 8u : 4u);
        const uint32_t off = (o & 0x3FFFFFFFu) + e * step;
        return Opnd{lane, lane ? off / 8u : off / 4u};
    }
    std::string val(uint32_t o, uint32_t e) const {
        const Opnd p = resolve(o, e);
        return p.lane ? fmt("v_%u", p.idx) : fmt("SPEC_U(%u)", p.idx);
    }
    void complete(uint32_t k, const std::string& expr) {
        if (counting_) return;
        const uint32_t pos = (uint32_t)order_.size();
        order_.push_back(k);
        line(fmt("SPEC_DU(%uu, %s);", pos, expr.c_str()));
    }
    void add_adj(uint32_t o, uint32_t e, const std::string& expr) {
        const Opnd p = resolve(o, e);
        if (p.lane) { line(fmt("a_%u += %s;", p.idx, expr.c_str())); return; }
        if (p.idx >= d_.n_uniform_grad) return;
        if (counting_) { ++du_total_[p.idx]; return; }
        if (direct_du_) { complete(p.idx, expr); return; }
        line(fmt("du_%u += %s;", p.idx, expr.c_str()));
        if (++du_seen_[p.idx] == du_total_[p.idx]) complete(p.idx, fmt("du_%u", p.idx));
    }

    std::string rcp_of(uint32_t o, uint32_t e) const {
        const Opnd p = resolve(o, e);
        return p.lane ? fmt("spec_rcp(v_%u)", p.idx) : fmt("SPEC_UR(%u)", p.idx);
    }
    std::string log_of(uint32_t o, uint32_t e) const {
        const Opnd p = resolve(o, e);
        return p.lane ? fmt("spec_log(v_%u)", p.idx) : fmt("SPEC_UL(%u)", p.idx);
    }

    std::string normal_var(uint32_t row, bool reverse) {
        const uint32_t g = row >> 2, j = row & 3u;
        std::set<uint32_t>& have = (reverse && !keep_eps_) ? rev_groups_ : fwd_groups_;
        if (!have.count(g)) {
            have.insert(g);
            all_groups_.insert(g);
            const std::string gs = (reverse && !keep_eps_) ? std::string("spec_opaque(") + fmt("%uu", g) + ")" : fmt("%uu", g);
            if (diag_) line(fmt("if (!noise) spec_normals4(A, T, %s, pn_%u_0, pn_%u_1, pn_%u_2, pn_%u_3);", gs.c_str(), g, g, g, g));
            else line(fmt("spec_normals4(A, T, %s, pn_%u_0, pn_%u_1, pn_%u_2, pn_%u_3);", gs.c_str(), g, g, g, g));
        }
        return fmt("pn_%u_%u", g, j);
    }
    std::string eps_forward(uint32_t row) {
        if (keep_eps_) { normal_rows_.insert(row); return fmt("Z.z[%u]", row); }
        const std::string pn = normal_var(row, false);
        if (!diag_) return pn;
        eps_rows_.insert(row);
        line(fmt("ez_%u = noise ? noise[(size_t)%uu * A.n_local + T.nc] : %s;", row, row, pn.c_str()));
        return fmt("ez_%u", row);
    }
    std::string eps_reverse(uint32_t row) {
        if (keep_eps_) return fmt("Z.z[%u]", row);
        const std::string pn = normal_var(row, true);
        if (!diag_) return pn;
        line(fmt("ez_%u = noise ? noise[(size_t)%uu * A.n_local + T.nc] : %s;", row, row, pn.c_str()));
        return fmt("ez_%u", row);
    }
    void diag_outputs(uint32_t row, const std::string& v, const std::string& noise) {
        if (!diag_) return;
        line(fmt("if (T.active) { if (A.samples_out) A.samples_out[(size_t)%uu * A.n_local + T.n] = %s; "
                 "if (A.noise_out) A.noise_out[(size_t)%uu * A.n_local + T.n] = %s; }", row, v.c_str(), row, noise.c_str()));
    }

    void forward(const Insn& I, uint32_t e, bool nodes) {
        const uint32_t op = I.w0 & 0xFFu, flags = (I.w0 >> 8) & 0xFFu, dist = (I.w0 >> 16) & 0xFFu;
        if (op == BSVI_OP_NAFF) {
            if (!nodes) return;
            ++visits_;
            if (counting_) return;
            line("{");
            line(fmt("  const float loc = %s * %s + %s;", val(I.a, e).c_str(), val(I.b, e).c_str(), val(I.c, e).c_str()));
            std::string v = val(I.dst, e);
            if (flags & BSVI_F_SAMPLE) {
                const uint32_t row = resolve(I.dst, e).idx;
                const std::string eps = eps_forward(row);
                if (flags & BSVI_F_GIVEN) line(fmt("  %s = %s;", v.c_str(), eps.c_str()));
                else line(fmt("  %s = loc + %s * %s;", v.c_str(), eps.c_str(), val(I.s, e).c_str()));
                diag_outputs(row, v, eps);
            }
            if (flags & (BSVI_F_ENT | BSVI_F_LOGP | BSVI_F_WF)) line(fmt("  const float lS = %s;", log_of(I.s, e).c_str()));
            if (flags & BSVI_F_ENT) line(fmt("  %s += %s * (kHalfLog2PiE + lS);", ftarget(), flit(I.imm1).c_str()));
            if (flags & (BSVI_F_LOGP | BSVI_F_WF)) {
                line(fmt("  const float lp = spec_naff_lp(%s, loc, %s, lS);", v.c_str(), rcp_of(I.s, e).c_str()));
                line(fmt("  %s += %s * lp;", ftarget(), flit(I.imm0).c_str()));
                if ((flags & BSVI_F_WF) && sink_mode_ != 2) line("  T.lq += lp;");
            }
            line("}");
        } else if (op == BSVI_OP_BIN) {
            ++visits_;
            if (counting_) return;
            const std::string a = val(I.a, e), b = val(I.b, e), y = val(I.dst, e);
            switch (flags) {
            case BSVI_B_ADD: line(fmt("%s = %s + %s;", y.c_str(), a.c_str(), b.c_str())); break;
            case BSVI_B_SUB: line(fmt("%s = %s - %s;", y.c_str(), a.c_str(), b.c_str())); break;
            case BSVI_B_MUL: line(fmt("%s = %s * %s;", y.c_str(), a.c_str(), b.c_str())); break;
            case BSVI_B_DIV: line(fmt("%s = %s / %s;", y.c_str(), a.c_str(), b.c_str())); break;
            case BSVI_B_POW: line(fmt("%s = pow_ff(%s, %s);", y.c_str(), a.c_str(), b.c_str())); break;
            default: line(fmt("%s = (%s == %s) ? 1.0f : 0.0f;", y.c_str(), a.c_str(), b.c_str())); break;
            }
        } else if (op == BSVI_OP_UN) {
            ++visits_;
            if (counting_) return;
            line(fmt("%s = unop<true>(%uu, %s, %s);", val(I.dst, e).c_str(), flags, val(I.a, e).c_str(), flit(I.imm0).c_str()));
        } else if (op == BSVI_OP_NODE) {
            if (!nodes) return;
            ++visits_;
            if (counting_) return;
            line("{");
            line(fmt("  const float p0 = %s, p1 = %s;", val(I.a, e).c_str(), val(I.b, e).c_str()));
            const std::string v = val(I.dst, e);
            if (flags & BSVI_F_SAMPLE) {
                const uint32_t row = resolve(I.dst, e).idx;
                node_rows_.insert(row);
                all_node_rows_.insert(row);
                const std::string draw = fmt("{ const float2 dr = philox_draw(spec_key(A, T), %u, p0, p1, %uu); %s = dr.x; ns_%u = dr.y; }",
                                             dist, row, v.c_str(), row);
                if (diag_) {
                    const std::string given = (flags & BSVI_F_GIVEN) ? fmt("ns_%u", row) : fmt("sample_from_noise_generic(%u, p0, p1, ns_%u)", dist, row);
                    line(fmt("  if (noise) { ns_%u = noise[(size_t)%uu * A.n_local + T.nc]; %s = %s; } else %s", row, row, v.c_str(), given.c_str(), draw.c_str()));
                } else {
                    line("  " + draw);
                }
                diag_outputs(row, v, fmt("ns_%u", row));
            }
            if (flags & BSVI_F_ENT) line(fmt("  %s += %s * entropy_generic(%u, p0, p1);", ftarget(), flit(I.imm1).c_str(), dist));
            if (flags & (BSVI_F_LOGP | BSVI_F_WF)) {
                line(fmt("  const float lp = logp_generic(%u, %s, p0, p1);", dist, v.c_str()));
                line(fmt("  %s += %s * lp;", ftarget(), flit(I.imm0).c_str()));
                if ((flags & BSVI_F_WF) && sink_mode_ != 2) line("  T.lq += lp;");
            }
            line("}");
        }
    }

    const char* ftarget() const { return sink_mode_ == 2 ? "f_dead" : "T.f"; }

    std::string wg(uint32_t imm) const { return diag_ ? "(" + flit(imm) + " * T.gw)" : flit(imm); }

    void naff_sink(const Insn& I, uint32_t e) {
        ++visits_;
        const std::string A = val(I.a, e), B = val(I.b, e);
        if (sink_mode_ == 1) {
            line(fmt("T.f += %s * spec_naff_lp(%s, %s * %s + %s, %s, %s);", flit(I.imm0).c_str(), val(I.dst, e).c_str(), A.c_str(), B.c_str(),
                     val(I.c, e).c_str(), rcp_of(I.s, e).c_str(), log_of(I.s, e).c_str()));
            return;
        }
        if (!counting_) {
            line("{");
            line(fmt("  float gl, gs; spec_naff_sink(%s, %s, %s * %s + %s, %s, %s, %s, gl, gs);", flit(I.imm0).c_str(), val(I.dst, e).c_str(),
                     A.c_str(), B.c_str(), val(I.c, e).c_str(), rcp_of(I.s, e).c_str(), log_of(I.s, e).c_str(), ftarget()));
            if (diag_) line("  gl *= T.gw; gs *= T.gw;");
        }
        add_adj(I.dst, e, "-gl");
        add_adj(I.a, e, "gl * " + B);
        add_adj(I.b, e, "gl * " + A);
        add_adj(I.c, e, "gl");
        add_adj(I.s, e, "gs");
        line("}");
    }

    void backward(const Insn& I, uint32_t e) {
        const uint32_t op = I.w0 & 0xFFu, flags = (I.w0 >> 8) & 0xFFu, dist = (I.w0 >> 16) & 0xFFu;
        ++visits_;
        if (op == BSVI_OP_NAFF) {
            const std::string A = val(I.a, e), B = val(I.b, e), v = val(I.dst, e);
            if (!counting_) {
                line("{");
                line(fmt("  const float rS = %s, loc = %s * %s + %s;", rcp_of(I.s, e).c_str(), A.c_str(), B.c_str(), val(I.c, e).c_str()));
                line("  float gv = 0.0f, gl = 0.0f, gs = 0.0f;");
                if (flags & (BSVI_F_LOGP | BSVI_F_WF)) {
                    const std::string gw = (flags & BSVI_F_WF) ? fmt("(%s + fweight)", wg(I.imm0).c_str()) : wg(I.imm0);
                    line(fmt("  spec_naff_lp_bwd(%s, %s, loc, rS, gv, gl, gs);", gw.c_str(), v.c_str()));
                }
                if (flags & BSVI_F_ENT) line(fmt("  gs += %s * rS;", wg(I.imm1).c_str()));
            }
            if (flags & BSVI_F_SAMPLE) {
                if (!counting_) {
                    const Opnd dst = resolve(I.dst, e);
                    const std::string eps = eps_reverse(dst.idx);
                    line(fmt("  const float zb = a_%u + gv;", dst.idx));
                    line("  gl += zb;");
                    line(fmt("  gs += zb * %s;", eps.c_str()));
                }
            } else {
                add_adj(I.dst, e, "gv");
            }
            add_adj(I.a, e, "gl * " + B);
            add_adj(I.b, e, "gl * " + A);
            add_adj(I.c, e, "gl");
            add_adj(I.s, e, "gs");
            line("}");
        } else if (op == BSVI_OP_BIN) {
            const std::string a = val(I.a, e), b = val(I.b, e);
            const Opnd dst = resolve(I.dst, e);
            const std::string g = fmt("a_%u", dst.idx), y = fmt("v_%u", dst.idx);
            switch (flags) {
            case BSVI_B_ADD: add_adj(I.a, e, g); add_adj(I.b, e, g); break;
            case BSVI_B_SUB: add_adj(I.a, e, g); add_adj(I.b, e, "-" + g); break;
            case BSVI_B_MUL: add_adj(I.a, e, g + " * " + b); add_adj(I.b, e, g + " * " + a); break;
            case BSVI_B_DIV:
                line(fmt("{ const float ga = %s / %s;", g.c_str(), b.c_str()));
                add_adj(I.a, e, "ga");
                add_adj(I.b, e, "-ga * " + y);
                line("}");
                break;
            case BSVI_B_POW:
                line(fmt("{ const float g = %s, pa = %s, pb = %s;", g.c_str(), a.c_str(), b.c_str()));
                add_adj(I.a, e, "g * pb * pow_ff(pa, pb - 1.0f)");
                add_adj(I.b, e, "((g == 0.0f) ? 0.0f : g * " + y + " * logf(pa))");
                line("}");
                break;
            default: break;
            }
        } else if (op == BSVI_OP_UN) {
            const Opnd dst = resolve(I.dst, e);
            const std::string a = val(I.a, e);
            add_adj(I.a, e, fmt("a_%u * unop_grad<true>(%uu, %s, v_%u, %s)", dst.idx, flags, a.c_str(), dst.idx, flit(I.imm0).c_str()));
        } else if (op == BSVI_OP_NODE) {
            const std::string v = val(I.dst, e);
            if (!counting_) {
                line("{");
                line(fmt("  const float p0 = %s, p1 = %s;", val(I.a, e).c_str(), val(I.b, e).c_str()));
                line("  float gv = 0.0f, g0 = 0.0f, g1 = 0.0f;");
                if (flags & (BSVI_F_LOGP | BSVI_F_WF)) {
                    const std::string gw = (flags & BSVI_F_WF) ? fmt("(%s + fweight)", wg(I.imm0).c_str()) : wg(I.imm0);
                    line(fmt("  { const float4 r = logp_bwd_generic(%u, %s, p0, p1, %s); gv += r.x; g0 += r.y; g1 += r.z; }", dist, v.c_str(), gw.c_str()));
                }
                if (flags & BSVI_F_ENT)
                    line(fmt("  { const float2 r = entropy_bwd_generic(%u, p0, p1, %s); g0 += r.x; g1 += r.y; }", dist, wg(I.imm1).c_str()));
            }
            if (flags & BSVI_F_SAMPLE) {
                if (!counting_) {
                    const Opnd dst = resolve(I.dst, e);
                    const bool base = dist == BSVI_DIST_LOGNORMAL || dist == BSVI_DIST_CAUCHY || dist == BSVI_DIST_LAPLACE;
                    const std::string noise = base ? fmt("ns_%u", dst.idx) : v;
                    line(fmt("  { const float2 r = sample_bwd_generic(%u, %s, p0, p1, %s, a_%u + gv); g0 += r.x; g1 += r.y; }",
                             dist, v.c_str(), noise.c_str(), dst.idx));
                }
            } else {
                add_adj(I.dst, e, "gv");
            }
            add_adj(I.a, e, "g0");
            add_adj(I.b, e, "g1");
            line("}");
        }
    }

    void zero_temps(uint32_t base, uint32_t n) {
        for (uint32_t t = 0; t < n; ++t) line(fmt("a_%u = 0.0f;", base + t));
    }

    struct Item { uint32_t first, n, n_elems, temp_base, n_temps; bool bracket, sink; };
    std::vector<Item> items() const {
        std::vector<Item> v;
        for (uint32_t pc = 0; pc < d_.n_code;) {
            const Insn I = insn(pc);
            const bool sink = (I.w0 >> 24) & BSVI_R_SINK;
            if ((I.w0 & 0xFFu) == BSVI_OP_REC_BEGIN) {
                v.push_back(Item{pc + 1, I.dst, I.a, I.b, I.c, true, sink});
                pc += I.dst + 2;
            } else {
                v.push_back(Item{pc, 1, 1, 0, 0, false, sink});
                pc += 1;
            }
        }
        return v;
    }
    void emit_forward(const Item& R) {
        if (!R.bracket) {
            const Insn I = insn(R.first);
            if (R.sink && (I.w0 & 0xFFu) == BSVI_OP_NAFF) { naff_sink(I, 0); return; }
            forward(I, 0, true);
            if (R.sink && sink_mode_ != 1) backward(I, 0);
            return;
        }
        for (uint32_t e = 0; e < R.n_elems && visits_ <= kMaxVisits; ++e) {
            for (uint32_t j = 0; j < R.n; ++j) forward(insn(R.first + j), e, true);
            if (R.sink && sink_mode_ != 1) {
                zero_temps(R.temp_base, R.n_temps);
                for (uint32_t j = R.n; j-- > 0;) backward(insn(R.first + j), e);
            }
        }
    }
    void emit_reverse(const Item& R) {
        if (!R.bracket) { backward(insn(R.first), 0); return; }
        for (uint32_t e = R.n_elems; e-- > 0 && visits_ <= kMaxVisits;) {
            for (uint32_t j = 0; j < R.n; ++j) forward(insn(R.first + j), e, false);
            zero_temps(R.temp_base, R.n_temps);
            for (uint32_t j = R.n; j-- > 0;) backward(insn(R.first + j), e);
        }
    }
    void slots_of(const Item& R, std::set<uint32_t>& reads, std::set<uint32_t>& writes) const {
        for (uint32_t j = 0; j < R.n; ++j) {
            const Insn I = insn(R.first + j);
            const uint32_t op = I.w0 & 0xFFu, flags = (I.w0 >> 8) & 0xFFu;
            const uint32_t ops[5] = {I.dst, I.a, I.b, I.c, I.s};
            const int n_opnd = (op == BSVI_OP_NAFF) ? 5 : ((op == BSVI_OP_UN) ? 2 : 3);
            const bool defines = op == BSVI_OP_BIN || op == BSVI_OP_UN || (flags & BSVI_F_SAMPLE);
            for (uint32_t e = 0; e < R.n_elems; ++e)
                for (int k = 0; k < n_opnd; ++k) {
                    const Opnd p = resolve(ops[k], e);
                    if (!p.lane) continue;
                    if (k == 0 && defines) writes.insert(p.idx); else reads.insert(p.idx);
                }
        }
    }

    void walk() {
        visits_ = 0;
        const std::vector<Item> recs = items();
        std::vector<std::pair<int, int>> key(recs.size(), std::make_pair(-1, -1));
        std::vector<int> def_of(d_.n_slots, -1);
        std::vector<uint32_t> rorder;
        for (uint32_t r = 0; r < recs.size(); ++r) {
            if (recs[r].sink) continue;
            std::set<uint32_t> rd, wr;
            slots_of(recs[r], rd, wr);
            bool samples = false;
            for (uint32_t j = 0; j < recs[r].n; ++j) {
                const Insn I = insn(recs[r].first + j);
                const uint32_t op = I.w0 & 0xFFu;
                if ((op == BSVI_OP_NAFF || op == BSVI_OP_NODE) && (((I.w0 >> 8) & 0xFFu) & BSVI_F_SAMPLE)) samples = true;
            }
            int anchor = (int)r;
            if (!samples && reschedule_) {
                int a = -1;
                for (uint32_t sl : rd) {
                    if (sl >= recs[r].temp_base && sl < recs[r].temp_base + recs[r].n_temps) continue;
                    if (def_of[sl] >= 0 && key[def_of[sl]].first > a) a = key[def_of[sl]].first;
                }
                if (a >= 0) anchor = a;
            }
            key[r] = std::make_pair(anchor, (int)r);
            for (uint32_t sl : wr) def_of[sl] = (int)r;
            rorder.push_back(r);
        }
        std::sort(rorder.begin(), rorder.end(), [&](uint32_t x, uint32_t y) { return key[x] > key[y]; });
        std::vector<std::vector<uint32_t>> deferred(recs.size());
        std::vector<int> home(recs.size(), -1);
        if (reschedule_) {
            for (uint32_t r = 0; r < recs.size(); ++r) {
                if (!recs[r].sink) continue;
                std::set<uint32_t> rd, wr;
                slots_of(recs[r], rd, wr);
                int first = -1;
                for (uint32_t sl : rd) {
                    if (sl >= recs[r].temp_base && sl < recs[r].temp_base + recs[r].n_temps) continue;
                    const int dr = def_of[sl];
                    if (dr >= 0 && (uint32_t)dr < r && (first < 0 || key[dr] > key[first])) first = dr;
                }
                if (first >= 0) { home[r] = first; deferred[first].push_back(r); }
            }
        }
        const bool fence = d_.n_code > kFenceAboveCode;
        uint32_t since = 0;
        auto maybe_fence = [&]() { if (fence && ++since >= kFenceEvery) { since = 0; line("asm volatile(\"\" ::: \"memory\"); __builtin_amdgcn_sched_barrier(0);"); } };
        if (two_pass_) line("float f_dead = 0.0f; (void)f_dead;");
        for (uint32_t r = 0; r < recs.size(); ++r) {
            if (home[r] >= 0 && !two_pass_) continue;
            sink_mode_ = home[r] >= 0 ? 1 : 0;
            emit_forward(recs[r]);
            sink_mode_ = 0;
            maybe_fence();
            if (visits_ > kMaxVisits) return;
        }
        if (diag_) line("const float fweight = A.q_weight ? A.q_weight[T.nc] : T.f * T.gw; (void)fweight;");
        else line("const float fweight = T.f; (void)fweight;");
        if (fence) {
            line("asm volatile(\"\" ::: \"memory\");");
            for (uint32_t s0 = 0; s0 < d_.n_slots; s0 += 16) {
                std::string ops;
                for (uint32_t sl = s0; sl < d_.n_slots && sl < s0 + 16; ++sl) ops += fmt("%s\"+v\"(v_%u)", sl == s0 ? "" : ", ", sl);
                line("asm volatile(\"\" : " + ops + ");");
            }
        }
        for (uint32_t r : rorder) {
            sink_mode_ = two_pass_ ? 2 : 0;
            for (uint32_t sidx : deferred[r]) emit_forward(recs[sidx]);
            sink_mode_ = 0;
            emit_reverse(recs[r]);
            maybe_fence();
            if (visits_ > kMaxVisits) return;
        }
        if (diag_) line("if (A.fvalue_out && T.active) { A.fvalue_out[T.n] = T.f; A.fvalue_out[(size_t)A.n_local + T.n] = T.lq; }");
    }
};

}

struct Variant {
    std::string src;
    hipModule_t module = nullptr;
    hipFunction_t fn = nullptr;
    bool failed = false;
    int per_cu = 0;
};

enum { GEOM_ONE = 0, GEOM_MANY = 1 };
struct Geom { uint32_t max_threads = 0, lds_bytes = 0; };

struct Spec {
    uint32_t n_params = 0, n_uniform = 0, n_ugrad = 0, n_obs = 0, n_noise = 0;
    uint32_t n_pos = 0;
    Geom geom[2];
    std::vector<uint32_t> pu_ptr_host, pu_pos_host, pu_idx_host;
    Variant variant[7];
    bool exchange_ok = false;
    void* dev = nullptr;
    unsigned int* tickets = nullptr;
    const uint32_t* pu_ptr = nullptr;
    const uint32_t* pu_pos = nullptr;
    const uint32_t* pu_idx = nullptr;
    uint32_t n_cus = 256;
    bool draw_wave_ok = false;
    uint32_t launch_seq = 0;
    std::mutex mu;
};

static uint32_t many_waves() {
    static const uint32_t w = [] { const char* e = getenv("BSVI_SPEC_MANY_WAVES"); const int v = e ? atoi(e) : 2; return (uint32_t)(v < 2 ? 2 : v > 4 ? 4 : v); }();
    return w;
}
static bool tiled(uint32_t n_pos, int geom) {
    static const bool many_tile = [] { const char* e = getenv("BSVI_SPEC_MANY_TILE"); return !(e && e[0] == '0'); }();
    if (geom == 1  && (!many_tile || many_waves() > 2)) return false;
    return n_pos <= 64;
}
static uint32_t lds_floats(uint32_t n_params, uint32_t n_uniform, uint32_t n_obs, uint32_t n_pos, uint32_t max_threads, int geom) {
    const uint32_t W = max_threads / 64;
    const uint32_t u_pad = (n_uniform + n_obs + 3) / 4 * 4, nu_pad = (n_uniform + 3) / 4 * 4;
    const uint32_t ws_pad = tiled(n_pos, geom) ? (n_pos + 3) / 4 * 4 + 4 : 4 * n_pos + 4;
    const uint32_t np_pad = (n_params + 3) / 4 * 4 + 4, tab = (4 * n_uniform + (2 * n_params + 1) + 2 * n_pos + 3) / 4 * 4 + 4;
    const uint32_t own = 20 * (n_params < max_threads ? n_params : max_threads), scr = 4 * (n_pos + 2) + 4;
    return u_pad + 2 * nu_pad + W * ws_pad + (2 * W + 8) + 5 * np_pad + tab + own + scr + (tiled(n_pos, geom) ? W * 64 * 68 : 0);
}

Spec* create(const bsvi_program_desc& d, std::string& why) {
    if (!d.n_code) { why = "empty program"; return nullptr; }
    Spec* s = new Spec();
    s->n_params = d.n_params; s->n_uniform = d.n_uniform; s->n_ugrad = d.n_uniform_grad; s->n_obs = d.n_obs; s->n_noise = d.n_noise;
    {
        Emitter E(d, false);
        if (!E.run(why)) { delete s; return nullptr; }
        const std::vector<uint32_t>& order = E.order();
        s->n_pos = (uint32_t)order.size();
        std::vector<std::vector<uint32_t>> pos_of(d.n_uniform_grad);
        for (uint32_t p = 0; p < order.size(); ++p) pos_of[order[p]].push_back(p);
        s->pu_ptr_host.assign(1, 0u);
        for (uint32_t i = 0; i < d.n_params; ++i) {
            for (uint32_t j = d.param_uniform_ptr[i]; j < d.param_uniform_ptr[i + 1]; ++j)
                for (uint32_t p : pos_of[d.param_uniform_idx[j]]) { s->pu_pos_host.push_back(p); s->pu_idx_host.push_back(d.param_uniform_idx[j]); }
            s->pu_ptr_host.push_back((uint32_t)s->pu_pos_host.size());
        }
    }
    const uint32_t live = 2 * d.n_slots + (d.n_noise <= kKeepEpsRows ? d.n_noise : 0) + (d.n_uniform_grad <= kAccumulateEntries ? d.n_uniform_grad : 0) + 40;
    auto fit = [&](uint32_t threads, Geom& g) {
        g.max_threads = threads;
        g.lds_bytes = lds_floats(d.n_params, d.n_uniform, d.n_obs, s->n_pos, threads, (int)(&g - s->geom)) * 4u;
        return g.lds_bytes <= 160u * 1024u;
    };
    bool ok = (live <= 232 && fit(512, s->geom[GEOM_ONE])) || fit(256, s->geom[GEOM_ONE]);
    ok = ok && fit(256, s->geom[GEOM_MANY]);
    if (!ok) { why = "the program's tables do not fit LDS"; delete s; return nullptr; }
    bool all_fast = d.n_params <= 64;
    for (uint32_t i = 0; i < d.n_params && all_fast; ++i) all_fast = s->pu_ptr_host[i + 1] - s->pu_ptr_host[i] <= 2;
    s->draw_wave_ok = all_fast && tiled(s->n_pos, GEOM_ONE) && d.n_noise > 0 && d.n_noise <= kKeepEpsRows;
    uint32_t ut_mask = 0;
    for (uint32_t k = 0; k < d.n_uniform; ++k) ut_mask |= 1u << (d.uniform[k].transform & 31u);
    const bool rare_transforms = (ut_mask >> (BSVI_UT_SIGMOID + 1)) != 0;
    for (int gi = 0; gi < 2; ++gi) {
        const Geom& G = s->geom[gi];
        for (int v = 0; v < 2; ++v) {
            Emitter E(d, v == 1);
            if (!E.run(why)) { delete s; return nullptr; }
            std::string src;
            src += "// generated by libbsvi (specialize.cpp) from a model program: do not edit\n";
            src += "#define BSVI_SPECIALIZED 1\n";
            const char* const slp = getenv("BSVI_JIT_SLP");
            if (slp ? slp[0] == '0' : (d.n_code > kFenceAboveCode && d.estimator == BSVI_EST_BLACKBOX))
                src += std::string(kJitOptionMark) + "-fno-slp-vectorize\n";
            const char* const ra = getenv("BSVI_JIT_REGALLOC");
            if (ra ? ra[0] == 'b' : d.n_code > kBasicRegallocAboveCode)
                src += std::string(kJitOptionMark) + "-mllvm\n" + kJitOptionMark + "-vgpr-regalloc=basic\n";
            src += fmt("#define SPEC_N_PARAMS %u\n#define SPEC_N_UNIFORM %u\n#define SPEC_N_UGRAD %u\n#define SPEC_N_OBS %u\n#define SPEC_N_NOISE %u\n",
                       d.n_params, d.n_uniform, d.n_uniform_grad, d.n_obs, d.n_noise);
            src += fmt("#define SPEC_N_POS %u\n", s->n_pos);
            src += fmt("#define SPEC_ESTIMATOR %u\n#define SPEC_MAX_THREADS %u\n#define SPEC_DIAG %d\n", d.estimator, G.max_threads, v);
            src += fmt("#define SPEC_ACCUMULATE_CHUNKS %d\n#define SPEC_TILE %d\n", gi == GEOM_MANY ? 1 : 0, tiled(s->n_pos, gi) ? 1 : 0);
            if (gi == GEOM_MANY && many_waves() > 2) src += fmt("#define SPEC_BOUND_THREADS %u\n", 256u * many_waves());
            src += fmt("#define SPEC_KEEP_NOISE %u\n", E.keeps_noise() ? d.n_noise : 0u);
            src += fmt("#define SPEC_GENERIC_OWNERS %d\n", all_fast ? 0 : 1);
            src += fmt("#define SPEC_RARE_TRANSFORMS %d\n#define SPEC_UT_MASK 0x%xu\n", rare_transforms ? 1 : 0, ut_mask);
            src += "#include \"spec_prelude.h\"\n";
            src += "namespace bsvi {\n";
            src += "__device__ __forceinline__ void spec_draw(const SpecBody& A, const SpecLane& T, SpecNoise& Z) {\n";
            src += "    (void)A; (void)T; (void)Z;\n";
            src += E.draw();
            src += "}\n";
            src += "__device__ __forceinline__ void spec_body(const SpecBody& A, SpecLane& T, const SpecNoise& Z, float* WSw) {\n";
            src += "    (void)Z;\n";
            if (v == 1) src += "    const float* const noise = A.noise;\n";
            src += E.declarations();
            src += E.body();
            src += "}\n}  // namespace bsvi\n";
            src += "#include \"spec_main.h\"\n";
            s->variant[2 * gi + v].src = std::move(src);
        }
    }
    s->variant[4].src = "#define SPEC_WITH_DRAW_WAVE 1\n" + s->variant[0].src;
    s->variant[6].src = "#define SPEC_WITH_DRAW_WAVE 1\n#define SPEC_WITH_DRAW_OWNERS 1\n" + s->variant[0].src;
    s->exchange_ok = true;
    s->variant[5].src = std::string("#define SPEC_WITH_EXCHANGE 1\n") + (s->draw_wave_ok ? "#define SPEC_WITH_DRAW_WAVE 1\n" : "") + s->variant[0].src;
    return s;
}

void destroy(Spec* s) {
    if (!s) return;
    for (Variant& v : s->variant) if (v.module) (void)hipModuleUnload(v.module);
    if (s->dev) (void)hipFree(s->dev);
    delete s;
}

int upload(Spec* s) {
    const size_t n_ptr = s->pu_ptr_host.size(), n_pos = s->pu_pos_host.size();
    const size_t bytes = 512 + (n_ptr + 2 * n_pos) * 4 + 256;
    hipError_t e = hipMalloc(&s->dev, bytes);
    if (e != hipSuccess) return bsvi_fail(BSVI_ERR_HIP, std::string("hipMalloc (specialiser tables): ") + hipGetErrorString(e));
    std::vector<uint32_t> host(128 + n_ptr + 2 * n_pos, 0u);
    std::copy(s->pu_ptr_host.begin(), s->pu_ptr_host.end(), host.begin() + 128);
    std::copy(s->pu_pos_host.begin(), s->pu_pos_host.end(), host.begin() + 128 + n_ptr);
    std::copy(s->pu_idx_host.begin(), s->pu_idx_host.end(), host.begin() + 128 + n_ptr + n_pos);
    e = hipMemset(s->dev, 0, bytes);
    if (e == hipSuccess) e = hipMemcpy(s->dev, host.data(), host.size() * 4, hipMemcpyHostToDevice);
    if (e != hipSuccess) return bsvi_fail(BSVI_ERR_HIP, std::string("specialiser tables: ") + hipGetErrorString(e));
    s->tickets = (unsigned int*)s->dev;
    s->pu_ptr = (const uint32_t*)s->dev + 128;
    s->pu_pos = s->pu_ptr + n_ptr;
    s->pu_idx = s->pu_pos + n_pos;
    int dev = 0, cus = 0;
    if (hipGetDevice(&dev) == hipSuccess && hipDeviceGetAttribute(&cus, hipDeviceAttributeMultiprocessorCount, dev) == hipSuccess && cus > 0)
        s->n_cus = (uint32_t)cus;
    return BSVI_OK;
}

const std::string& source(const Spec* s, int variant) { return s->variant[(variant >= 4 && variant <= 6) ? variant : (variant & 3)].src; }

static const char* kJitOptions[] = {"--offload-arch=gfx950", "-O3", "-std=c++17", "-Xclang", "-target-feature", "-Xclang", "-packed-fp32-ops"};
static const int kJitOptionCount = (int)(sizeof(kJitOptions) / sizeof(kJitOptions[0]));

int compile(const std::string& src, std::vector<char>& code, std::string& log) {
    hiprtcProgram prog = nullptr;
    hiprtcResult r = hiprtcCreateProgram(&prog, src.c_str(), "bsvi_spec.hip", kJitHeaderCount, kJitHeaderTexts, kJitHeaderNames);
    if (r != HIPRTC_SUCCESS) { log = std::string("hiprtcCreateProgram: ") + hiprtcGetErrorString(r); return BSVI_ERR_HIP; }
    std::vector<std::string> extra;
    for (size_t at = src.find(kJitOptionMark); at != std::string::npos; at = src.find(kJitOptionMark, at + 1)) {
        const size_t b = at + strlen(kJitOptionMark), e = src.find('\n', b);
        extra.push_back(src.substr(b, e == std::string::npos ? std::string::npos : e - b));
    }
    std::vector<const char*> opts(kJitOptions, kJitOptions + kJitOptionCount);
    for (const std::string& o : extra) opts.push_back(o.c_str());
    r = hiprtcCompileProgram(prog, (int)opts.size(), opts.data());
    size_t n = 0;
    if (hiprtcGetProgramLogSize(prog, &n) == HIPRTC_SUCCESS && n > 1) {
        log.resize(n);
        (void)hiprtcGetProgramLog(prog, &log[0]);
    }
    if (r != HIPRTC_SUCCESS) {
        log = std::string("hiprtcCompileProgram: ") + hiprtcGetErrorString(r) + "\n" + log;
        (void)hiprtcDestroyProgram(&prog);
        return BSVI_ERR_HIP;
    }
    size_t cs = 0;
    r = hiprtcGetCodeSize(prog, &cs);
    if (r == HIPRTC_SUCCESS) { code.resize(cs); r = hiprtcGetCode(prog, code.data()); }
    (void)hiprtcDestroyProgram(&prog);
    if (r != HIPRTC_SUCCESS) { log = std::string("hiprtcGetCode: ") + hiprtcGetErrorString(r); return BSVI_ERR_HIP; }
    if (const char* dump = getenv("BSVI_JIT_DUMP")) {
        if (FILE* f = fopen(dump, "wb")) { fwrite(code.data(), 1, code.size(), f); fclose(f); }
    }
    return BSVI_OK;
}

static std::mutex g_cache_mu;
static std::map<std::string, std::vector<char>> g_code_cache;

namespace disk_cache {

struct Hash128 { uint64_t a = 0xcbf29ce484222325ull, b = 0x9ae16a3b2f90404full; };
static void feed(Hash128& h, const void* data, size_t n) {
    const unsigned char* p = (const unsigned char*)data;
    for (size_t i = 0; i < n; ++i) {
        h.a = (h.a ^ p[i]) * 0x100000001b3ull;
        h.b = (h.b + p[i] + 0x9e3779b97f4a7c15ull) * 0xff51afd7ed558ccdull;
        h.b ^= h.b >> 29;
    }
}
static void feed(Hash128& h, const std::string& s) { const uint64_t n = s.size(); feed(h, &n, 8); feed(h, s.data(), s.size()); }

static bool enabled() {
    const char* e = getenv("BSVI_JIT_CACHE");
    return !(e && e[0] == '0');
}

static std::string directory() {
    if (const char* d = getenv("BSVI_CACHE_DIR")) if (d[0]) return d;
    if (const char* x = getenv("XDG_CACHE_HOME")) if (x[0]) return std::string(x) + "/brancher_amd/jit";
    if (const char* h = getenv("HOME")) if (h[0]) return std::string(h) + "/.cache/brancher_amd/jit";
    return fmt("/tmp/brancher_amd-%u/jit", (unsigned)getuid());
}

static bool make_dirs(const std::string& path) {
    for (size_t i = 1; i <= path.size(); ++i)
        if (i == path.size() || path[i] == '/') {
            const std::string part = path.substr(0, i);
            if (mkdir(part.c_str(), 0700) != 0 && errno != EEXIST) return false;
        }
    return true;
}

static bool trusted(const std::string& dir) {
    struct stat st;
    if (lstat(dir.c_str(), &st) != 0) return false;
    return S_ISDIR(st.st_mode) && st.st_uid == getuid() && (st.st_mode & (S_IWGRP | S_IWOTH)) == 0;
}

static int identity_cb(struct dl_phdr_info* info, size_t, void* data) {
    const char* name = info->dlpi_name;
    if (!name || !*name) return 0;
    const char* base = strrchr(name, '/');
    base = base ? base + 1 : name;
    const char* const parts[] = {"libamd_comgr", "libhiprtc", "libLLVM", "libclang-cpp", "libclang.so"};
    bool is_part = false;
    for (const char* p : parts) is_part = is_part || strncmp(base, p, strlen(p)) == 0;
    if (!is_part) return 0;
    struct stat st;
    std::string& id = *(std::string*)data;
    id += name;
    if (stat(name, &st) == 0) id += fmt(":%lld:%lld", (long long)st.st_size, (long long)st.st_mtime);
    id += ";";
    return 0;
}
std::string compiler_identity() {
    std::string s;
    dl_iterate_phdr(identity_cb, &s);
    return s;
}
static bool identity_resolved(const std::string& id) { return id.find("amd_comgr") != std::string::npos; }

static std::string key_of(const std::string& src) {
    static const Hash128 base = [] {
        Hash128 h;
        for (int i = 0; i < kJitHeaderCount; ++i) { feed(h, std::string(kJitHeaderNames[i])); feed(h, std::string(kJitHeaderTexts[i])); }
        for (int i = 0; i < kJitOptionCount; ++i) feed(h, std::string(kJitOptions[i]));
        int major = 0, minor = 0, runtime = 0;
        (void)hiprtcVersion(&major, &minor);
        (void)hipRuntimeGetVersion(&runtime);
        feed(h, fmt("hiprtc %d.%d runtime %d abi %d", major, minor, runtime, BSVI_ABI_VERSION));
        return h;
    }();
    Hash128 h = base;
    feed(h, compiler_identity());
    feed(h, src);
    return fmt("%016llx%016llx", (unsigned long long)h.a, (unsigned long long)h.b);
}

struct Header { char magic[8]; uint64_t size, ha, hb; };
static const char kMagic[8] = {'B', 'S', 'V', 'I', 'C', 'O', '0', '1'};

static bool load(const std::string& key, std::vector<char>& code) {
    const std::string dir = directory();
    if (!trusted(dir)) return false;
    const std::string path = dir + "/" + key + ".co";
    const int fd = open(path.c_str(), O_RDONLY | O_NOFOLLOW | O_CLOEXEC);
    FILE* f = fd >= 0 ? fdopen(fd, "rb") : nullptr;
    if (!f) { if (fd >= 0) close(fd); return false; }
    Header H;
    bool ok = fread(&H, sizeof H, 1, f) == 1 && memcmp(H.magic, kMagic, 8) == 0 && H.size > 0 && H.size < (1ull << 30);
    if (ok) {
        code.resize(H.size);
        ok = fread(code.data(), 1, H.size, f) == H.size && fgetc(f) == EOF;
    }
    fclose(f);
    if (ok) {
        Hash128 h;
        feed(h, code.data(), code.size());
        ok = h.a == H.ha && h.b == H.hb;
    }
    if (!ok) code.clear();
    return ok;
}

static void store(const std::string& key, const std::vector<char>& code) {
    const std::string dir = directory();
    if (!make_dirs(dir) || !trusted(dir)) return;
    Header H;
    memcpy(H.magic, kMagic, 8);
    H.size = code.size();
    Hash128 h;
    feed(h, code.data(), code.size());
    H.ha = h.a; H.hb = h.b;
    const std::string tmp = dir + "/" + key + fmt(".tmp.%d", (int)getpid());
    const int fd = open(tmp.c_str(), O_WRONLY | O_CREAT | O_EXCL | O_NOFOLLOW | O_CLOEXEC, 0600);
    FILE* f = fd >= 0 ? fdopen(fd, "wb") : nullptr;
    if (!f) { if (fd >= 0) close(fd); return; }
    const bool ok = fwrite(&H, sizeof H, 1, f) == 1 && fwrite(code.data(), 1, code.size(), f) == code.size();
    if (fclose(f) != 0 || !ok || rename(tmp.c_str(), (dir + "/" + key + ".co").c_str()) != 0) (void)remove(tmp.c_str());
}

}

static thread_local int t_last_source = 0;

int obtain(const std::string& text, std::vector<char>& code, std::string& log, int* origin) {
    {
        std::lock_guard<std::mutex> g(g_cache_mu);
        auto it = g_code_cache.find(text);
        if (it != g_code_cache.end()) code = it->second;
    }
    int from = 2;
    if (code.empty()) {
        std::string src = text;
        const bool tuned = getenv("BSVI_SPEC_DEFINES") != nullptr;
        if (tuned) src = std::string(getenv("BSVI_SPEC_DEFINES")) + "\n" + src;
        const bool on_disk = disk_cache::enabled() && !getenv("BSVI_JIT_DUMP");
        const bool lookup = on_disk && disk_cache::identity_resolved(disk_cache::compiler_identity());
        if (lookup && disk_cache::load(disk_cache::key_of(src), code)) {
            from = 3;
        } else {
            const int rc = compile(src, code, log);
            if (rc) return rc;
            from = 1;
            if (on_disk && disk_cache::identity_resolved(disk_cache::compiler_identity())) disk_cache::store(disk_cache::key_of(src), code);
        }
        std::lock_guard<std::mutex> g(g_cache_mu);
        if (!tuned) g_code_cache[text] = code;
    }
    t_last_source = from;
    if (origin) *origin = from;
    return BSVI_OK;
}

int last_origin() { return t_last_source; }
std::string cache_directory() { return disk_cache::enabled() ? disk_cache::directory() : std::string(); }
std::string compiler_identity() { return disk_cache::compiler_identity(); }

static int ensure_compiled(Spec* s, int v) {
    Variant& V = s->variant[v];
    if (V.fn) return BSVI_OK;
    if (V.failed) return BSVI_ERR_UNSUPPORTED;
    std::vector<char> code;
    std::string log;
    if (obtain(V.src, code, log, nullptr)) {
        V.failed = true;
        if (getenv("BSVI_DEBUG")) fprintf(stderr, "bsvi: specialised kernel did not compile:\n%s\n", log.c_str());
        return bsvi_fail(BSVI_ERR_UNSUPPORTED, "specialised kernel did not compile: " + log.substr(0, 400));
    }
    hipError_t e = hipModuleLoadData(&V.module, code.data());
    if (e == hipSuccess) e = hipModuleGetFunction(&V.fn, V.module, "bsvi_spec_kernel");
    if (e != hipSuccess) {
        V.failed = true;
        V.fn = nullptr;
        return bsvi_fail(BSVI_ERR_HIP, std::string("loading the specialised kernel: ") + hipGetErrorString(e));
    }
    return BSVI_OK;
}

struct Geo { uint32_t blocks, threads; int geom; bool draw_wave = false; uint32_t extra_waves = 0; bool draw_owners = false; };
static bool draw_wave() {
    const char* e = getenv("BSVI_SPEC_DRAW_WAVE");
    return !(e && e[0] == '0');
}
static bool draw_service() {
    const char* e = getenv("BSVI_SPEC_DRAW_SERVICE");
    return !(e && e[0] == '0');
}
static bool owner_wave() {
    const char* e = getenv("BSVI_SPEC_OWNER_WAVE");
    return !(e && e[0] == '0');
}
static Geo geo(const Spec* s, uint32_t n_local, int mode = MODE_SUMS, bool exchange = false) {
    const uint32_t waves = (n_local + 63) / 64;
    if (waves <= s->geom[GEOM_ONE].max_threads / 64) {
        const bool extra = mode == MODE_LOOP && s->draw_wave_ok && draw_wave() && waves <= 4 && waves + 1 <= s->geom[GEOM_ONE].max_threads / 64
                           && !s->variant[exchange ? 5 : 4].failed;
        const uint32_t n_service = waves == 4 ? 4u : 3u;
        const bool service = mode == MODE_LOOP && s->draw_wave_ok && draw_wave() && draw_service() && waves >= 4 && waves <= 5
                             && waves + n_service <= s->geom[GEOM_ONE].max_threads / 64 && (size_t)s->n_noise * 64u * waves <= (size_t)n_service * 64u * 68u
                             && !s->variant[exchange ? 5 : 4].failed;
        const uint32_t more = service ? n_service : extra ? 1u : 0u;
        const bool owners = service && (size_t)s->n_noise * 64u * (waves + 1u) <= (size_t)n_service * 64u * 68u;
        return Geo{1, (waves + more) * 64, GEOM_ONE, more != 0u, more, owners};
    }
    const uint32_t threads = s->geom[GEOM_MANY].max_threads;
    uint32_t blocks = (n_local + threads - 1) / threads;
    uint32_t per_cu = many_waves();
    while (per_cu > 1u && s->geom[GEOM_MANY].lds_bytes * per_cu > 160u * 1024u) --per_cu;
    if (blocks > per_cu * s->n_cus) blocks = per_cu * s->n_cus;
    return Geo{blocks, threads, GEOM_MANY};
}

void geometry(const Spec* s, uint32_t n_local, int mode, uint32_t* n_blocks, uint32_t* n_threads, uint32_t* lds_bytes) {
    const Geo g = geo(s, n_local, mode);
    if (n_blocks) *n_blocks = g.blocks;
    if (n_threads) *n_threads = g.threads;
    if (lds_bytes) *lds_bytes = s->geom[g.geom].lds_bytes;
}

size_t workspace_bytes(const Spec* s, uint32_t n_local) {
    const Geo g = geo(s, n_local);
    return ((size_t)g.blocks * (2 + s->n_pos) * 4 + 255) / 256 * 256 + 256;
}

bool applies(const Spec* s, uint32_t n_local, int mode) {
    if (!s || !n_local) return false;
    const char* e = getenv("BSVI_JIT");
    if (e && e[0] == '0') return false;
    const Geo g = geo(s, n_local);
    if (s->variant[2 * g.geom].failed || s->variant[2 * g.geom + 1].failed) return false;
    if (mode == MODE_LOOP && g.blocks != 1) {
        const char* m = getenv("BSVI_SPEC_LOOP_MANY");
        return !(m && m[0] == '0');
    }
    return true;
}

int launch(Spec* s, const bsvi_program* p, const Launch& L) {
    const bsvi_elbo_args* a = L.a;
    if (!a->params_dev && s->n_params) return bsvi_fail(BSVI_ERR_INVALID, "params_dev is null");
    if (!a->obs_dev && s->n_obs) return bsvi_fail(BSVI_ERR_INVALID, "obs_dev is null");
    if (!a->out_dev) return bsvi_fail(BSVI_ERR_INVALID, "out_dev is null");
    if (!a->n_samples_local || !a->n_samples_global) return bsvi_fail(BSVI_ERR_INVALID, "zero samples");
    Geo g = geo(s, a->n_samples_local, L.mode, L.xchg != nullptr);
    int v = 2 * g.geom + ((a->noise_dev || a->samples_out_dev || a->noise_out_dev || a->fvalue_out_dev || a->f_weight_dev || a->q_weight_dev) ? 1 : 0);
    if (L.xchg && !(L.mode == MODE_LOOP && g.blocks == 1 && v == 0 && s->exchange_ok))
        return bsvi_fail(BSVI_ERR_UNSUPPORTED, "the in-loop exchange serves the one-workgroup training loop with Philox noise and no per-sample outputs");
    uint32_t seq;
    {
        std::lock_guard<std::mutex> lock(s->mu);
        if (L.xchg) {
            const int rc5 = ensure_compiled(s, 5);
            if (rc5) return rc5;
            v = 5;
        }
        else if (g.draw_owners && v == 0 && owner_wave()) {
            const int rc6 = ensure_compiled(s, 6);
            if (rc6) return rc6;
            v = 6;
        }
        else if (g.draw_wave && v == 0 && ensure_compiled(s, 4) == BSVI_OK) v = 4;
        else if (g.draw_wave) { g.threads -= 64 * g.extra_waves; g.draw_wave = false; }
        const int rc = ensure_compiled(s, v);
        if (rc) return rc;
        seq = s->launch_seq++;
    }
    if (g.blocks > 1 && !L.workspace) return bsvi_fail(BSVI_ERR_INVALID, "workspace_dev is null");
    SpecArgs A;
    memset(&A, 0, sizeof A);
    A.uniform = p->uniform; A.consts = p->consts;
    A.params = L.params ? L.params : const_cast<float*>(a->params_dev);
    A.obs = a->obs_dev; A.noise = a->noise_dev;
    A.samples_out = a->samples_out_dev; A.noise_out = a->noise_out_dev; A.fvalue_out = a->fvalue_out_dev;
    A.out = a->out_dev;
    A.partials = (float*)L.workspace;
    A.ticket = s->tickets + (seq % 64u);
    A.pu_ptr = s->pu_ptr; A.pu_pos = s->pu_pos; A.pu_idx = s->pu_idx;
    A.state = L.state; A.mask = L.mask; A.mask_first = L.mask_first ? L.mask_first : L.mask;
    A.loss_slot = L.loss_slot; A.finite_slot = L.finite_slot;
    A.n_local = a->n_samples_local; A.n_global = a->n_samples_global; A.sample_base = a->sample_base;
    A.mode = (uint32_t)L.mode;
    A.seed_lo = (uint32_t)a->seed; A.seed_hi = (uint32_t)(a->seed >> 32);
    A.offset_lo = (uint32_t)a->offset; A.offset_hi = (uint32_t)(a->offset >> 32);
    A.offset_dev = (const unsigned long long*)a->offset_dev;
    A.f_weight = a->f_weight_dev; A.q_weight = a->q_weight_dev;
    A.xchg = (const bsvi::SpecExchange*)L.xchg;
    A.n_iterations = L.n_iterations; A.pretraining_iterations = L.pretraining_iterations; A.n_params = s->n_params;
    if (L.cfg) A.cfg = *L.cfg;
    if (g.blocks > 1) {
        int per_cu = s->variant[v].per_cu;
        if (!per_cu) {
            if (hipModuleOccupancyMaxActiveBlocksPerMultiprocessor(&per_cu, s->variant[v].fn, (int)g.threads, 0) != hipSuccess || per_cu <= 0) {
                (void)hipGetLastError();
                per_cu = -1;
            }
            s->variant[v].per_cu = per_cu;
        }
        if (per_cu > 0 && g.blocks > (uint32_t)per_cu * s->n_cus) g.blocks = (uint32_t)per_cu * s->n_cus;
        if (L.mode == MODE_LOOP) {
            hipError_t me = hipMemsetAsync(A.ticket, 0, 4, (hipStream_t)a->stream);
            if (me == hipSuccess) me = hipMemsetAsync(A.ticket + 64, 0, 4, (hipStream_t)a->stream);
            if (me != hipSuccess) return bsvi_fail(BSVI_ERR_HIP, std::string("hipMemsetAsync (loop ticket): ") + hipGetErrorString(me));
        }
    }
    size_t size = sizeof A;
    void* config[] = {HIP_LAUNCH_PARAM_BUFFER_POINTER, &A, HIP_LAUNCH_PARAM_BUFFER_SIZE, &size, HIP_LAUNCH_PARAM_END};
    const hipError_t e = hipModuleLaunchKernel(s->variant[v].fn, g.blocks, 1, 1, g.threads, 1, 1, 0, (hipStream_t)a->stream, nullptr, config);
    if (e != hipSuccess) return bsvi_fail(BSVI_ERR_HIP, std::string("hipModuleLaunchKernel (specialised kernel): ") + hipGetErrorString(e));
    return BSVI_OK;
}

}
```

brancher_amd/native.py:

```python
import ctypes as C
import os

import numpy as np

_HERE = os.path.dirname(os.path.abspath(__file__))
LIB_PATH = os.path.join(_HERE, "libbsvi.so")
ABI_VERSION = 11
OUT_HEADER = 4


class NativeError(RuntimeError):
    pass


class Sized(C.Structure):

    def __init__(self, *args, **kw):
        super().__init__(*args, **kw)
        self.struct_size = C.sizeof(self)


class UniformEntry(C.Structure):
    _fields_ = [("src", C.c_uint32), ("transform", C.c_uint8), ("is_param", C.c_uint8),
                ("reserved", C.c_uint16), ("a", C.c_float), ("b", C.c_float)]


class Record(C.Structure):
    _fields_ = [("code_begin", C.c_uint32), ("code_end", C.c_uint32), ("n_elems", C.c_uint32),
                ("temp_base", C.c_uint32), ("n_temps", C.c_uint32), ("flags", C.c_uint32)]


class ProgramDesc(Sized):
    _fields_ = [("struct_size", C.c_uint32), ("abi_version", C.c_uint32), ("n_params", C.c_uint32), ("n_consts", C.c_uint32),
                ("n_obs", C.c_uint32), ("n_slots", C.c_uint32), ("n_noise", C.c_uint32),
                ("n_uniform", C.c_uint32), ("n_uniform_grad", C.c_uint32), ("n_records", C.c_uint32),
                ("n_code", C.c_uint32), ("estimator", C.c_uint32),
                ("uniform", C.c_void_p), ("records", C.c_void_p), ("code", C.c_void_p), ("consts", C.c_void_p),
                ("param_uniform_ptr", C.c_void_p), ("param_uniform_idx", C.c_void_p)]


class ElboArgs(Sized):
    _fields_ = [("struct_size", C.c_uint32), ("reserved0", C.c_uint32),
                ("params_dev", C.c_void_p), ("obs_dev", C.c_void_p), ("noise_dev", C.c_void_p),
                ("seed", C.c_uint64), ("offset", C.c_uint64),
                ("n_samples_local", C.c_uint32), ("n_samples_global", C.c_uint32),
                ("sample_base", C.c_uint32), ("reserved", C.c_uint32),
                ("out_dev", C.c_void_p), ("samples_out_dev", C.c_void_p), ("noise_out_dev", C.c_void_p),
                ("fvalue_out_dev", C.c_void_p), ("workspace_dev", C.c_void_p), ("stream", C.c_void_p),
                ("offset_dev", C.c_void_p), ("f_weight_dev", C.c_void_p), ("q_weight_dev", C.c_void_p)]


class OptCfg(C.Structure):
    _fields_ = [("kind", C.c_uint32), ("lr", C.c_float), ("momentum", C.c_float), ("dampening", C.c_float),
                ("weight_decay", C.c_float), ("nesterov", C.c_uint32), ("beta1", C.c_float), ("beta2", C.c_float),
                ("eps", C.c_float), ("amsgrad", C.c_uint32), ("maximize", C.c_uint32)]


class DenseDesc(Sized):
    _fields_ = [("struct_size", C.c_uint32), ("abi_version", C.c_uint32), ("n_params", C.c_uint32), ("n_consts", C.c_uint32),
                ("n_uniform", C.c_uint32), ("n_uniform_grad", C.c_uint32),
                ("n_classes", C.c_uint32), ("n_features", C.c_uint32), ("dataset_size", C.c_uint32),
                ("batch_size", C.c_uint32), ("likelihood", C.c_uint32),
                ("q_loc_u", C.c_uint32), ("q_scale_u", C.c_uint32), ("prior_loc_u", C.c_uint32),
                ("prior_scale_u", C.c_uint32), ("q_loc_stride", C.c_uint32), ("q_scale_stride", C.c_uint32),
                ("prior_loc_stride", C.c_uint32), ("prior_scale_stride", C.c_uint32),
                ("lik_weight", C.c_float), ("prior_weight", C.c_float), ("entropy_weight", C.c_float),
                ("estimator", C.c_uint32), ("reserved", C.c_uint32),
                ("uniform", C.c_void_p), ("consts", C.c_void_p), ("param_uniform_ptr", C.c_void_p),
                ("param_uniform_idx", C.c_void_p), ("dataset", C.c_void_p), ("labels", C.c_void_p)]


class DenseArgs(Sized):
    _fields_ = [("struct_size", C.c_uint32), ("reserved0", C.c_uint32),
                ("params_dev", C.c_void_p), ("noise_dev", C.c_void_p), ("indices_dev", C.c_void_p),
                ("seed", C.c_uint64), ("offset", C.c_uint64),
                ("n_samples_local", C.c_uint32), ("n_samples_global", C.c_uint32),
                ("sample_base", C.c_uint32), ("reserved", C.c_uint32),
                ("out_dev", C.c_void_p), ("noise_out_dev", C.c_void_p), ("indices_out_dev", C.c_void_p),
                ("fvalue_out_dev", C.c_void_p), ("workspace_dev", C.c_void_p), ("stream", C.c_void_p),
                ("f_weight_dev", C.c_void_p), ("q_weight_dev", C.c_void_p), ("logq_out_dev", C.c_void_p)]


DENSE_EXPORTS = {
    "bsvi_dense_create": (C.c_int, [C.POINTER(DenseDesc), C.POINTER(C.c_void_p)]),
    "bsvi_dense_destroy": (None, [C.c_void_p]),
    "bsvi_dense_workspace_bytes": (C.c_size_t, [C.c_void_p, C.c_uint32]),
    "bsvi_dense_exact_data": (C.c_int, [C.c_void_p]),
    "bsvi_dense_fwd_bwd": (C.c_int, [C.c_void_p, C.POINTER(DenseArgs)]),
    "bsvi_dense_finalize": (C.c_int, [C.c_void_p, C.c_void_p, C.c_uint32, C.c_void_p]),
    "bsvi_dense_step": (C.c_int, [C.c_void_p, C.POINTER(DenseArgs), C.POINTER(OptCfg), C.c_void_p, C.c_void_p,
                                  C.c_void_p, C.c_void_p, C.c_void_p]),
}



EXPORTS = {
    "bsvi_program_create": (C.c_int, [C.POINTER(ProgramDesc), C.POINTER(C.c_void_p)]),
    "bsvi_program_destroy": (None, [C.c_void_p]),
    "bsvi_workspace_bytes": (C.c_size_t, [C.c_void_p, C.c_uint32]),
    "bsvi_elbo_fwd_bwd": (C.c_int, [C.c_void_p, C.POINTER(ElboArgs)]),
    "bsvi_finalize": (C.c_int, [C.c_void_p, C.c_void_p, C.c_uint32, C.c_void_p]),
    "bsvi_optimizer_step": (C.c_int, [C.POINTER(OptCfg), C.c_void_p, C.c_void_p, C.c_void_p, C.c_void_p,
                                      C.c_uint32, C.c_void_p]),
    "bsvi_finalize_step": (C.c_int, [C.POINTER(OptCfg), C.c_void_p, C.c_void_p, C.c_void_p, C.c_void_p, C.c_uint32,
                                     C.c_uint32, C.c_void_p, C.c_void_p, C.c_void_p]),
    "bsvi_finalize_step_counted": (C.c_int, [C.POINTER(OptCfg), C.c_void_p, C.c_void_p, C.c_void_p, C.c_void_p, C.c_void_p,
                                             C.c_uint32, C.c_uint32, C.c_uint32, C.c_void_p, C.c_void_p, C.c_void_p,
                                             C.c_void_p]),
    "bsvi_svi_step": (C.c_int, [C.c_void_p, C.POINTER(ElboArgs), C.POINTER(OptCfg), C.c_void_p, C.c_void_p,
                                C.c_void_p, C.c_void_p, C.c_void_p]),
    "bsvi_train_persistent": (C.c_int, [C.c_void_p, C.POINTER(ElboArgs), C.POINTER(OptCfg), C.c_void_p, C.c_void_p,
                                        C.c_void_p, C.c_uint32, C.c_void_p, C.c_void_p]),
    "bsvi_train_persistent2": (C.c_int, [C.c_void_p, C.POINTER(ElboArgs), C.POINTER(OptCfg), C.c_void_p, C.c_void_p,
                                         C.c_void_p, C.c_void_p, C.c_uint32, C.c_uint32, C.c_void_p, C.c_void_p]),
    "bsvi_train_persistent_exchange": (C.c_int, [C.c_void_p, C.POINTER(ElboArgs), C.POINTER(OptCfg), C.c_void_p, C.c_void_p,
                                                 C.c_void_p, C.c_void_p, C.c_uint32, C.c_uint32, C.c_void_p, C.c_void_p, C.c_void_p]),
    "bsvi_persistent_supported": (C.c_int, [C.c_void_p, C.c_uint32]),
    "bsvi_persistent_split_shares": (C.c_int, [C.c_void_p, C.c_uint32]),
    "bsvi_program_set_shares": (C.c_int, [C.c_void_p, C.POINTER(C.c_void_p), C.c_uint32]),
    "bsvi_train_persistent_split": (C.c_int, [C.c_void_p, C.POINTER(C.c_void_p), C.c_uint32, C.POINTER(ElboArgs),
                                              C.POINTER(OptCfg), C.c_void_p, C.c_void_p, C.c_void_p, C.c_void_p,
                                              C.c_uint32, C.c_uint32, C.c_void_p, C.c_void_p]),
    "bsvi_program_source": (C.c_size_t, [C.POINTER(ProgramDesc), C.c_int, C.c_char_p, C.c_size_t]),
    "bsvi_jit_compile": (C.c_int, [C.c_char_p, C.POINTER(C.c_size_t)]),
    "bsvi_jit_load": (C.c_int, [C.c_char_p, C.POINTER(C.c_size_t), C.POINTER(C.c_int)]),
    "bsvi_jit_last_origin": (C.c_int, []),
    "bsvi_jit_cache_dir": (C.c_size_t, [C.c_char_p, C.c_size_t]),
    "bsvi_jit_compiler_identity": (C.c_size_t, [C.c_char_p, C.c_size_t]),
    "bsvi_program_engine": (C.c_int, [C.c_void_p, C.c_uint32, C.c_int, C.POINTER(C.c_uint32), C.POINTER(C.c_uint32),
                                      C.POINTER(C.c_uint32)]),
    "bsvi_max_lds_bytes": (C.c_int, [C.c_void_p]),
    "bsvi_query_geometry": (C.c_int, [C.c_void_p, C.c_uint32, C.POINTER(C.c_uint32), C.POINTER(C.c_uint32),
                                      C.POINTER(C.c_uint32), C.POINTER(C.c_uint64)]),
    "bsvi_debug_math": (C.c_int, [C.c_int, C.c_int, C.c_void_p, C.c_void_p, C.c_void_p, C.c_void_p, C.c_uint32,
                                  C.c_void_p]),
    "bsvi_debug_set_stamps": (None, [C.c_void_p]),
    "bsvi_last_error": (C.c_char_p, []),
    "bsvi_abi_version": (C.c_int, []),
    "bsvi_sizeof": (C.c_size_t, [C.c_int]),
    "bsvi_device_count": (C.c_int, []),
}
EXPORTS.update(DENSE_EXPORTS)


class BnnLayer(C.Structure):
    _fields_ = [("rows", C.c_uint32), ("cols", C.c_uint32), ("weight_row0", C.c_uint32), ("bias_row0", C.c_uint32),
                ("activation", C.c_uint32), ("reserved", C.c_uint32)]


class BnnDesc(Sized):
    _fields_ = [("struct_size", C.c_uint32), ("abi_version", C.c_uint32), ("n_params", C.c_uint32), ("n_consts", C.c_uint32),
                ("n_uniform", C.c_uint32), ("n_uniform_grad", C.c_uint32),
                ("n_layers", C.c_uint32), ("n_rows", C.c_uint32), ("n_features", C.c_uint32), ("dataset_size", C.c_uint32),
                ("batch_size", C.c_uint32), ("likelihood", C.c_uint32), ("estimator", C.c_uint32),
                ("lik_weight", C.c_float), ("prior_weight", C.c_float), ("entropy_weight", C.c_float),
                ("layers", C.c_void_p), ("row_uniform", C.c_void_p), ("uniform", C.c_void_p), ("consts", C.c_void_p),
                ("param_uniform_ptr", C.c_void_p), ("param_uniform_idx", C.c_void_p), ("dataset", C.c_void_p), ("labels", C.c_void_p)]


class BnnArgs(Sized):
    _fields_ = [("struct_size", C.c_uint32), ("reserved0", C.c_uint32),
                ("params_dev", C.c_void_p), ("noise_dev", C.c_void_p), ("indices_dev", C.c_void_p),
                ("seed", C.c_uint64), ("offset", C.c_uint64),
                ("n_samples_local", C.c_uint32), ("n_samples_global", C.c_uint32), ("sample_base", C.c_uint32), ("reserved", C.c_uint32),
                ("out_dev", C.c_void_p), ("noise_out_dev", C.c_void_p), ("indices_out_dev", C.c_void_p),
                ("fvalue_out_dev", C.c_void_p), ("logq_out_dev", C.c_void_p), ("workspace_dev", C.c_void_p), ("stream", C.c_void_p),
                ("f_weight_dev", C.c_void_p), ("q_weight_dev", C.c_void_p)]


EXPORTS.update({
    "bsvi_bnn_create": (C.c_int, [C.POINTER(BnnDesc), C.POINTER(C.c_void_p)]),
    "bsvi_bnn_destroy": (None, [C.c_void_p]),
    "bsvi_bnn_workspace_bytes": (C.c_size_t, [C.c_void_p, C.c_uint32]),
    "bsvi_bnn_exact_data": (C.c_int, [C.c_void_p]),
    "bsvi_bnn_fwd_bwd": (C.c_int, [C.c_void_p, C.POINTER(BnnArgs)]),
    "bsvi_bnn_finalize": (C.c_int, [C.c_void_p, C.c_void_p, C.c_uint32, C.c_void_p]),
    "bsvi_bnn_step": (C.c_int, [C.c_void_p, C.POINTER(BnnArgs), C.POINTER(OptCfg), C.c_void_p, C.c_void_p, C.c_void_p,
                                C.c_void_p, C.c_void_p]),
})


class MlpLayer(C.Structure):
    _fields_ = [("in_value", C.c_uint32), ("out_value", C.c_uint32), ("n_in", C.c_uint32), ("n_out", C.c_uint32),
                ("weight_off", C.c_uint32), ("bias_off", C.c_uint32), ("activation", C.c_uint32),
                ("post_add", C.c_float), ("split_col", C.c_uint32), ("activation2", C.c_uint32),
                ("post_add2", C.c_float), ("reserved", C.c_uint32)]


class AmortDesc(Sized):
    _fields_ = [("struct_size", C.c_uint32), ("reserved0", C.c_uint32), ("abi_version", C.c_uint32), ("n_params", C.c_uint32),
                ("n_features", C.c_uint32), ("latent_dim", C.c_uint32), ("dataset_size", C.c_uint32),
                ("batch_size", C.c_uint32), ("n_enc_layers", C.c_uint32), ("n_dec_layers", C.c_uint32),
                ("enc_loc_value", C.c_uint32), ("enc_scale_value", C.c_uint32),
                ("enc_loc_col", C.c_uint32), ("enc_scale_col", C.c_uint32),
                ("dec_logits_value", C.c_uint32), ("likelihood", C.c_uint32),
                ("enc_layers", C.POINTER(MlpLayer)), ("dec_layers", C.POINTER(MlpLayer)),
                ("prior_loc", C.c_void_p), ("prior_scale", C.c_void_p), ("dataset", C.c_void_p),
                ("likelihood_scale", C.c_void_p), ("prior_loc_off", C.c_uint32), ("prior_scale_off", C.c_uint32),
                ("lik_scale_off", C.c_uint32), ("lik_scale_size", C.c_uint32), ("dec_scale_value", C.c_uint32), ("reserved1", C.c_uint32)]


class AmortArgs(Sized):
    _fields_ = [("struct_size", C.c_uint32), ("reserved0", C.c_uint32),
                ("params_dev", C.c_void_p), ("noise_dev", C.c_void_p), ("indices_dev", C.c_void_p),
                ("seed", C.c_uint64), ("offset", C.c_uint64),
                ("n_samples_local", C.c_uint32), ("n_samples_global", C.c_uint32),
                ("sample_base", C.c_uint32), ("estimator", C.c_uint32),
                ("out_dev", C.c_void_p), ("noise_out_dev", C.c_void_p), ("indices_out_dev", C.c_void_p),
                ("fvalue_out_dev", C.c_void_p), ("logq_out_dev", C.c_void_p), ("workspace_dev", C.c_void_p),
                ("stream", C.c_void_p), ("f_weight_dev", C.c_void_p), ("q_weight_dev", C.c_void_p)]


EXPORTS.update({
    "bsvi_amort_create": (C.c_int, [C.POINTER(AmortDesc), C.POINTER(C.c_void_p)]),
    "bsvi_amort_destroy": (None, [C.c_void_p]),
    "bsvi_amort_workspace_bytes": (C.c_size_t, [C.c_void_p, C.c_uint32]),
    "bsvi_amort_exact_data": (C.c_int, [C.c_void_p]),
    "bsvi_amort_fwd_bwd": (C.c_int, [C.c_void_p, C.POINTER(AmortArgs)]),
    "bsvi_amort_bucket": (C.c_int, [C.c_void_p, C.POINTER(C.c_uint32), C.POINTER(C.c_uint32)]),
    "bsvi_amort_set_bucket_stream": (C.c_int, [C.c_void_p, C.c_void_p]),
    "bsvi_amort_apply": (C.c_int, [C.c_void_p, C.c_int, C.c_void_p, C.c_void_p, C.c_uint32, C.c_uint32, C.c_void_p,
                                   C.c_void_p, C.c_void_p]),
    "bsvi_debug_gemm": (C.c_int, [C.c_int, C.c_void_p, C.c_void_p, C.c_void_p, C.c_void_p, C.c_uint32, C.c_uint32,
                                  C.c_uint32, C.c_uint32, C.c_uint32, C.c_uint32, C.c_void_p, C.c_uint32, C.c_uint32,
                                  C.c_float, C.c_uint32, C.c_void_p]),
})

EXPORTS.update({
    "bsvi_allreduce": (C.c_int, [C.c_void_p, C.c_void_p, C.c_size_t, C.c_void_p]),
    "bsvi_exchange_handle_bytes": (C.c_size_t, []),
    "bsvi_exchange_create": (C.c_int, [C.c_uint32, C.c_uint32, C.c_uint32, C.POINTER(C.c_void_p)]),
    "bsvi_exchange_export": (C.c_int, [C.c_void_p, C.c_void_p]),
    "bsvi_exchange_connect": (C.c_int, [C.c_void_p, C.c_void_p]),
    "bsvi_exchange_allreduce": (C.c_int, [C.c_void_p, C.c_void_p, C.c_uint32, C.c_void_p]),
    "bsvi_exchange_status": (C.c_int, [C.c_void_p]),
    "bsvi_exchange_selftest_tagged": (C.c_int, [C.c_void_p, C.c_void_p, C.c_uint32, C.c_void_p]),
    "bsvi_minibatch_gather": (C.c_int, [C.c_void_p, C.c_uint32, C.c_uint32, C.c_uint32, C.c_void_p, C.c_uint64, C.c_uint64, C.c_void_p, C.c_void_p, C.c_void_p]),
    "bsvi_exchange_destroy": (None, [C.c_void_p]),
})

class MvnInsn(C.Structure):
    _fields_ = [("kind", C.c_uint32), ("flag", C.c_uint32), ("a", C.c_uint32), ("b", C.c_uint32), ("imm", C.c_float)]


class MvnDesc(Sized):
    _fields_ = [("struct_size", C.c_uint32), ("reserved0", C.c_uint32), ("abi_version", C.c_uint32), ("dim", C.c_uint32), ("n_code", C.c_uint32), ("n_mats", C.c_uint32),
                ("n_slot_inputs", C.c_uint32), ("n_uniform_inputs", C.c_uint32), ("value_is_latent", C.c_uint32),
                ("loc_is_param", C.c_uint32),
                ("code", C.POINTER(MvnInsn)), ("mats", C.c_void_p), ("loc", C.c_void_p), ("value", C.c_void_p),
                ("uniform_inputs", C.c_void_p), ("loc_entries", C.c_void_p), ("weight", C.c_float), ("form", C.c_uint32),
                ("value_entries", C.c_void_p), ("value_is_param", C.c_uint32), ("reserved1", C.c_uint32)]


class MvnArgs(Sized):
    _fields_ = [("struct_size", C.c_uint32), ("reserved0", C.c_uint32),
                ("params_dev", C.c_void_p), ("samples_dev", C.c_void_p), ("rows_out_dev", C.c_void_p),
                ("n_samples_local", C.c_uint32), ("value_row0", C.c_uint32), ("input_rows", C.c_uint32 * 8),
                ("stream", C.c_void_p)]


MVN_KIND = dict(MAT=0, INPUT=1, IMM=2, BIN=3, UN=4)
MVN_FORM = dict(covariance_matrix=0, scale_tril=1, precision_matrix=2)
EXPORTS.update({
    "bsvi_mvn_create": (C.c_int, [C.POINTER(MvnDesc), C.POINTER(C.c_void_p)]),
    "bsvi_mvn_destroy": (None, [C.c_void_p]),
    "bsvi_mvn_rows_out": (C.c_uint32, [C.POINTER(MvnDesc)]),
    "bsvi_mvn_eval": (C.c_int, [C.c_void_p, C.POINTER(MvnArgs)]),
    "bsvi_mvn_source": (C.c_size_t, [C.POINTER(MvnDesc), C.c_char_p, C.c_size_t]),
})


def mvn_desc(node):
    code = (MvnInsn * len(node.code))(*[MvnInsn(kind=MVN_KIND[k], flag=f, a=a, b=b, imm=imm) for k, f, a, b, imm in node.code])
    mats = np.ascontiguousarray(node.mats, dtype=np.float32)
    loc = np.ascontiguousarray(node.loc, dtype=np.float32)
    value = np.ascontiguousarray(node.value if node.value is not None else np.zeros(node.dim), dtype=np.float32)
    uni = np.ascontiguousarray(node.uniform_inputs)
    loc_entries = getattr(node, "loc_entries", None)
    loc_entries = np.ascontiguousarray(loc_entries) if loc_entries is not None else None
# ... 322 lines not shown
```

include/bsvi.h:

```cpp
#ifndef BSVI_H
#define BSVI_H

#if !defined(__HIPCC_RTC__)
#include <stddef.h>
#include <stdint.h>
#else
typedef unsigned char uint8_t;
typedef unsigned short uint16_t;
typedef unsigned int uint32_t;
typedef int int32_t;
typedef unsigned long long uint64_t;
typedef long long int64_t;
#endif

#ifdef __cplusplus
extern "C" {
#endif

#define BSVI_ABI_VERSION 11

typedef enum bsvi_struct_kind {
    BSVI_SK_UNIFORM_ENTRY = 0, BSVI_SK_RECORD = 1, BSVI_SK_PROGRAM_DESC = 2, BSVI_SK_ELBO_ARGS = 3, BSVI_SK_OPT_CFG = 4,
    BSVI_SK_DENSE_DESC = 5, BSVI_SK_DENSE_ARGS = 6, BSVI_SK_MLP_LAYER = 7, BSVI_SK_AMORT_DESC = 8, BSVI_SK_AMORT_ARGS = 9,
    BSVI_SK_MVN_INSN = 10, BSVI_SK_MVN_DESC = 11, BSVI_SK_MVN_ARGS = 12, BSVI_SK_BNN_LAYER = 13, BSVI_SK_BNN_DESC = 14,
// ... 41 lines not shown
    BSVI_B_DELTA = 5
} bsvi_binop;

typedef enum bsvi_unop {
    BSVI_U_COPY = 0, BSVI_U_NEG = 1, BSVI_U_EXP = 2, BSVI_U_LOG = 3, BSVI_U_SQRT = 4, BSVI_U_SIN = 5,
    BSVI_U_COS = 6, BSVI_U_TANH = 7, BSVI_U_ABS = 8, BSVI_U_SIGMOID = 9, BSVI_U_SOFTPLUS = 10,
    BSVI_U_RELU = 11, BSVI_U_RECIP = 12, BSVI_U_LOG1P = 13, BSVI_U_EXPM1 = 14, BSVI_U_SQUARE = 15,
    BSVI_U_P2L = 16,
    BSVI_U_POWI = 17
} bsvi_unop;

typedef enum bsvi_utransform {
    BSVI_UT_IDENTITY = 0, BSVI_UT_SOFTPLUS = 1, BSVI_UT_SIGMOID = 2, BSVI_UT_EXP = 3,
    BSVI_UT_LOG = 4, BSVI_UT_TANH = 5, BSVI_UT_SQRT = 6, BSVI_UT_SQUARE = 7
} bsvi_utransform;

typedef struct bsvi_uniform_entry {
    uint32_t src;
    uint8_t  transform;
    uint8_t  is_param;
    uint16_t reserved;
    float    a, b;
} bsvi_uniform_entry;

typedef struct bsvi_record {
    uint32_t code_begin, code_end;
    uint32_t n_elems;
    uint32_t temp_base, n_temps;
    uint32_t flags;
} bsvi_record;

typedef enum bsvi_estimator {
    BSVI_EST_PATHWISE = 0,
    BSVI_EST_BLACKBOX = 1
} bsvi_estimator;

typedef struct bsvi_program_desc {
    uint32_t struct_size;
    uint32_t abi_version;
    uint32_t n_params;
    uint32_t n_consts;
    uint32_t n_obs;
    uint32_t n_slots;
    uint32_t n_noise;
    uint32_t n_uniform;
    uint32_t n_uniform_grad;
    uint32_t n_records;
    uint32_t n_code;
    uint32_t estimator;
    const bsvi_uniform_entry* uniform;
    const bsvi_record* records;
    const uint32_t* code;
    const float* consts;
    const uint32_t* param_uniform_ptr;
    const uint32_t* param_uniform_idx;
} bsvi_program_desc;

typedef struct bsvi_program bsvi_program;

int bsvi_program_create(const bsvi_program_desc* desc, bsvi_program** out);
void bsvi_program_destroy(bsvi_program* prog);

size_t bsvi_workspace_bytes(const bsvi_program* prog, uint32_t n_samples_local);

#define BSVI_OUT_HEADER 4

typedef struct bsvi_elbo_args {
    uint32_t struct_size;
    uint32_t reserved0;
    const float* params_dev;
    const float* obs_dev;
    const float* noise_dev;
    uint64_t seed;
    uint64_t offset;
    uint32_t n_samples_local;
    uint32_t n_samples_global;
    uint32_t sample_base;
    uint32_t reserved;
    float* out_dev;
    float* samples_out_dev;
    float* noise_out_dev;
    float* fvalue_out_dev;
    void* workspace_dev;
    void* stream;
    const uint64_t* offset_dev;
    const float* f_weight_dev;
    const float* q_weight_dev;
} bsvi_elbo_args;

int bsvi_elbo_fwd_bwd(const bsvi_program* prog, const bsvi_elbo_args* args);

int bsvi_finalize(const bsvi_program* prog, float* out_dev, uint32_t n_samples_global, void* stream);

typedef enum bsvi_optimizer_kind { BSVI_OPT_SGD = 0, BSVI_OPT_ADAM = 1 } bsvi_optimizer_kind;

typedef struct bsvi_opt_cfg {
    uint32_t kind;
    float lr;
    float momentum, dampening, weight_decay;
    uint32_t nesterov;
    float beta1, beta2, eps;
    uint32_t amsgrad;
    uint32_t maximize;
} bsvi_opt_cfg;

int bsvi_optimizer_step(const bsvi_opt_cfg* cfg, float* params_dev, const float* out_dev,
                        float* state_dev, const uint8_t* active_mask_dev, uint32_t n_params,
                        void* stream);

int bsvi_finalize_step(const bsvi_opt_cfg* cfg, float* params_dev, float* out_dev, float* state_dev,
                       const uint8_t* active_mask_dev, uint32_t n_params, uint32_t n_samples_global,
                       float* loss_slot_dev, float* finite_slot_dev, void* stream);

int bsvi_finalize_step_counted(const bsvi_opt_cfg* cfg, float* params_dev, float* out_dev, float* state_dev,
                               const uint8_t* active_mask_dev, const uint8_t* active_mask_first_dev,
                               uint32_t pretraining_iterations, uint32_t n_params, uint32_t n_samples_global,
                               float* loss_curve_dev, float* finite_curve_dev, uint64_t* counters_dev, void* stream);

int bsvi_train_persistent(const bsvi_program* prog, const bsvi_elbo_args* args,
                          const bsvi_opt_cfg* cfg, float* params_dev, float* state_dev,
                          const uint8_t* active_mask_dev, uint32_t n_iterations,
                          float* loss_curve_dev, float* finite_dev);

int bsvi_train_persistent2(const bsvi_program* prog, const bsvi_elbo_args* args,
                           const bsvi_opt_cfg* cfg, float* params_dev, float* state_dev,
                           const uint8_t* active_mask_dev, const uint8_t* active_mask_first_dev,
                           uint32_t pretraining_iterations, uint32_t n_iterations,
                           float* loss_curve_dev, float* finite_dev);

struct bsvi_exchange;
int bsvi_train_persistent_exchange(const bsvi_program* prog, const bsvi_elbo_args* args, const bsvi_opt_cfg* cfg,
                                   float* params_dev, float* state_dev, const uint8_t* active_mask_dev,
                                   const uint8_t* active_mask_first_dev, uint32_t pretraining_iterations,
                                   uint32_t n_iterations, float* loss_curve_dev, float* finite_dev,
                                   struct bsvi_exchange* exchange);

int bsvi_persistent_supported(const bsvi_program* prog, uint32_t n_samples_local);
int bsvi_persistent_split_shares(const bsvi_program* p, uint32_t n_samples_local);
int bsvi_program_set_shares(bsvi_program* p, const bsvi_program* const* shares, uint32_t n_shares);
int bsvi_train_persistent_split(const bsvi_program* p, const bsvi_program* const* shares, uint32_t n_shares,
                                const bsvi_elbo_args* args, const bsvi_opt_cfg* cfg, float* params_dev, float* state_dev,
                                const uint8_t* active_mask_dev, const uint8_t* active_mask_first_dev,
                                uint32_t pretraining_iterations, uint32_t n_iterations, float* loss_curve_dev,
                                float* finite_dev);

int bsvi_svi_step(const bsvi_program* prog, const bsvi_elbo_args* args, const bsvi_opt_cfg* cfg,
                  float* params_dev, float* state_dev, const uint8_t* active_mask_dev,
                  float* loss_slot_dev, float* finite_slot_dev);

size_t bsvi_program_source(const bsvi_program_desc* desc, int variant, char* buf, size_t capacity);
int bsvi_jit_compile(const char* source, size_t* code_bytes);
int bsvi_jit_load(const char* source, size_t* code_bytes, int* origin);
int bsvi_jit_last_origin(void);
size_t bsvi_jit_cache_dir(char* buf, size_t capacity);
size_t bsvi_jit_compiler_identity(char* buf, size_t capacity);
int bsvi_program_engine(const bsvi_program* prog, uint32_t n_local, int mode, uint32_t* n_blocks, uint32_t* n_threads,
                        uint32_t* lds_bytes);

int bsvi_max_lds_bytes(const bsvi_program* prog);

int bsvi_query_geometry(const bsvi_program* prog, uint32_t n_samples_local, uint32_t* n_blocks,
                        uint32_t* n_waves, uint32_t* zglobal, uint64_t* lds_bytes);

typedef enum bsvi_dense_likelihood {
    BSVI_LIK_CATEGORICAL = 0,
    BSVI_LIK_BERNOULLI = 1
} bsvi_dense_likelihood;

typedef struct bsvi_dense_desc {
    uint32_t struct_size;
    uint32_t abi_version;
    uint32_t n_params, n_consts, n_uniform, n_uniform_grad;
    uint32_t n_classes, n_features, dataset_size, batch_size;
    uint32_t likelihood;
    uint32_t q_loc_u, q_scale_u, prior_loc_u, prior_scale_u;
    uint32_t q_loc_stride, q_scale_stride, prior_loc_stride, prior_scale_stride;
    float lik_weight, prior_weight, entropy_weight;
    uint32_t estimator;
    uint32_t reserved;
    const bsvi_uniform_entry* uniform;
    const float* consts;
    const uint32_t* param_uniform_ptr;
    const uint32_t* param_uniform_idx;
    const float* dataset;
    const float* labels;
} bsvi_dense_desc;

typedef struct bsvi_dense bsvi_dense;

typedef struct bsvi_dense_args {
    uint32_t struct_size;
    uint32_t reserved0;
    const float* params_dev;
    const float* noise_dev;
    const int32_t* indices_dev;
    uint64_t seed, offset;
    uint32_t n_samples_local, n_samples_global, sample_base, reserved;
    float* out_dev;
    float* noise_out_dev;
    int32_t* indices_out_dev;
    float* fvalue_out_dev;
    void* workspace_dev;
    void* stream;
    const float* f_weight_dev;
    const float* q_weight_dev;
    float* logq_out_dev;
} bsvi_dense_args;

int bsvi_dense_create(const bsvi_dense_desc* desc, bsvi_dense** out);
void bsvi_dense_destroy(bsvi_dense* d);
size_t bsvi_dense_workspace_bytes(const bsvi_dense* d, uint32_t n_samples_local);
int bsvi_dense_exact_data(const bsvi_dense* d);
int bsvi_dense_fwd_bwd(const bsvi_dense* d, const bsvi_dense_args* args);
int bsvi_dense_finalize(const bsvi_dense* d, float* out_dev, uint32_t n_samples_global, void* stream);
int bsvi_dense_step(const bsvi_dense* d, const bsvi_dense_args* args, const bsvi_opt_cfg* cfg,
                    float* params_dev, float* state_dev, const uint8_t* active_mask_dev,
                    float* loss_slot_dev, float* finite_slot_dev);

typedef enum bsvi_bnn_activation {
    BSVI_BNN_ACT_NONE = 0, BSVI_BNN_ACT_TANH = 1, BSVI_BNN_ACT_RELU = 2, BSVI_BNN_ACT_SIGMOID = 3, BSVI_BNN_ACT_SOFTPLUS = 4
} bsvi_bnn_activation;

typedef struct bsvi_bnn_layer {
    uint32_t rows, cols;
    uint32_t weight_row0;
    uint32_t bias_row0;
    uint32_t activation;
    uint32_t reserved;
} bsvi_bnn_layer;

typedef struct bsvi_bnn_desc {
    uint32_t struct_size;
    uint32_t abi_version;
    uint32_t n_params, n_consts, n_uniform, n_uniform_grad;
    uint32_t n_layers, n_rows, n_features, dataset_size, batch_size;
    uint32_t likelihood;
    uint32_t estimator;
    float lik_weight, prior_weight, entropy_weight;
    const bsvi_bnn_layer* layers;
    const uint32_t* row_uniform;
    const bsvi_uniform_entry* uniform;
    const float* consts;
    const uint32_t* param_uniform_ptr;
    const uint32_t* param_uniform_idx;
    const float* dataset;
    const float* labels;
} bsvi_bnn_desc;

typedef struct bsvi_bnn bsvi_bnn;

typedef struct bsvi_bnn_args {
    uint32_t struct_size;
    uint32_t reserved0;
    const float* params_dev;
    const float* noise_dev;
    const int32_t* indices_dev;
    uint64_t seed, offset;
    uint32_t n_samples_local, n_samples_global, sample_base, reserved;
    float* out_dev;
    float* noise_out_dev;
    int32_t* indices_out_dev;
    float* fvalue_out_dev;
    float* logq_out_dev;
    void* workspace_dev;
    void* stream;
    const float* f_weight_dev;
    const float* q_weight_dev;
} bsvi_bnn_args;

int bsvi_bnn_create(const bsvi_bnn_desc* desc, bsvi_bnn** out);
void bsvi_bnn_destroy(bsvi_bnn* b);
size_t bsvi_bnn_workspace_bytes(const bsvi_bnn* b, uint32_t n_samples_local);
int bsvi_bnn_exact_data(const bsvi_bnn* b);
int bsvi_bnn_fwd_bwd(const bsvi_bnn* b, const bsvi_bnn_args* args);
int bsvi_bnn_finalize(const bsvi_bnn* b, float* out_dev, uint32_t n_samples_global, void* stream);
int bsvi_bnn_step(const bsvi_bnn* b, const bsvi_bnn_args* args, const bsvi_opt_cfg* cfg, float* params_dev, float* state_dev,
                  const uint8_t* active_mask_dev, float* loss_slot_dev, float* finite_slot_dev);

typedef enum bsvi_mlp_activation {
    BSVI_ACT_NONE = 0,
    BSVI_ACT_RELU = 1,
    BSVI_ACT_SOFTPLUS = 2
} bsvi_mlp_activation;

typedef struct bsvi_mlp_layer {
    uint32_t in_value, out_value;
    uint32_t n_in, n_out;
    uint32_t weight_off, bias_off;
    uint32_t activation;
    float post_add;
    uint32_t split_col;
    uint32_t activation2;
    float post_add2;
    uint32_t reserved;
} bsvi_mlp_layer;

typedef struct bsvi_amort_desc {
    uint32_t struct_size, reserved0;
    uint32_t abi_version, n_params;
    uint32_t n_features, latent_dim, dataset_size, batch_size;
    uint32_t n_enc_layers, n_dec_layers;
    uint32_t enc_loc_value, enc_scale_value;
    uint32_t enc_loc_col, enc_scale_col;
    uint32_t dec_logits_value, likelihood;
    const bsvi_mlp_layer* enc_layers;
    const bsvi_mlp_layer* dec_layers;
// ... 153 lines not shown
```

Measured before the change: 283,200.

## Add lean owner-wave chain and constant-folded affine codegen in specialised kernel

Adds a lean owner path for the draw-owners variant, used when every parameter has a single entry. It preloads per-wave partial sums into registers, keeps the output pointers and optimizer config in scalar registers, and runs the single-entry gradient and optimizer update without the two-entry loops. The code generator now folds literal 0/1 constants in affine expressions, using exact-add helpers so results stay bit-identical. Owner geometry is restricted to launches that fill the block exactly, and the old chain stays available through an environment variable as variant 7. This adds code complexity, a trap when the wave count does not match, and a possible change in which variant is chosen for some sizes.

```diff
diff --git a/brancher_amd/csrc/bsvi_internal.h b/brancher_amd/csrc/bsvi_internal.h
--- a/brancher_amd/csrc/bsvi_internal.h
+++ b/brancher_amd/csrc/bsvi_internal.h
@@ -51,6 +51,7 @@
 int compile(const std::string& src, std::vector<char>& code, std::string& log);
 int obtain(const std::string& src, std::vector<char>& code, std::string& log, int* origin);
 int last_origin();
+int last_variant();
 std::string cache_directory();
 std::string compiler_identity();
 size_t workspace_bytes(const Spec* s, uint32_t n_local);
diff --git a/brancher_amd/csrc/elbo_kernel.hip b/brancher_amd/csrc/elbo_kernel.hip
--- a/brancher_amd/csrc/elbo_kernel.hip
+++ b/brancher_amd/csrc/elbo_kernel.hip
@@ -2056,6 +2056,7 @@
 }
 
 extern "C" int bsvi_jit_last_origin(void) { return bsvi_spec::last_origin(); }
+extern "C" int bsvi_spec_last_variant(void) { return bsvi_spec::last_variant(); }
 
 extern "C" size_t bsvi_jit_cache_dir(char* buf, size_t capacity) {
     const std::string dir = bsvi_spec::cache_directory();
diff --git a/brancher_amd/csrc/spec_main.h b/brancher_amd/csrc/spec_main.h
--- a/brancher_amd/csrc/spec_main.h
+++ b/brancher_amd/csrc/spec_main.h
@@ -4,9 +4,11 @@
 
 #if defined(__HIP_DEVICE_COMPILE__)
 #define SPEC_CONST_AS __attribute__((address_space(4)))
+#define SPEC_GLOBAL_AS __attribute__((address_space(1)))
 #define SPEC_RELOAD_ARGS() asm volatile("" : "+s"(ka))
 #else
 #define SPEC_CONST_AS
+#define SPEC_GLOBAL_AS
 #define SPEC_RELOAD_ARGS()
 #endif
 
@@ -55,6 +57,15 @@
     spec_store_uniform(k, __uint_as_float(TAB[4 * k + 2]) + __uint_as_float(TAB[4 * k + 3]) * utransform_common(w1 & 0xFFu, x));
 }
 
+#ifndef SPEC_OWN_ENTRIES
+#define SPEC_OWN_ENTRIES 2
+#endif
+__device__ __forceinline__ float spec_rows_total(const float (&r)[SPEC_MAX_WAVES]) {
+    float s = 0.0f;
+#pragma unroll
+    for (uint32_t w = 0; w < SPEC_MAX_WAVES; ++w) s += r[w];
+    return s;
+}
 struct SpecOwn {
     float theta, s0, s1, s2, st;
     float a[2], b[2];
@@ -315,6 +326,11 @@
 #else
 #define SPEC_DRAW_OWNERS 0
 #endif
+#if SPEC_DRAW_OWNERS && defined(SPEC_LEAN_CHAIN) && !defined(SPEC_DEBUG_NO_LEAN_CHAIN) && SPEC_OWN_ENTRIES == 1
+#define SPEC_LEAN_OWNERS 1
+#else
+#define SPEC_LEAN_OWNERS 0
+#endif
 #if SPEC_DRAW_OWNERS
     const uint32_t own_base = own_wave * 64u;
 #else
@@ -351,7 +367,7 @@
                 }
             }
 #pragma unroll
-            for (uint32_t e = 0; e < 2u; ++e) {
+            for (uint32_t e = 0; e < SPEC_OWN_ENTRIES; ++e) {
                 if (e < own.n) {
                     const uint32_t k = TAB[SPEC_TAB_IDX + j0 + e];
                     own.pos[e] = TAB[SPEC_TAB_POS + j0 + e];
@@ -404,13 +420,13 @@
 #if defined(SPEC_DEBUG_STAMPS)
     unsigned long long stamp[12] = {0, 0, 0, 0, 0, 0, 0, 0, 0, 0, 0, 0};
 #define SPEC_STAMP(i) if (it == n_it / 2) stamp[i] = __builtin_amdgcn_s_memtime()
-    unsigned long long rstamp[6] = {0, 0, 0, 0, 0, 0};
+    unsigned long long rstamp[7] = {0, 0, 0, 0, 0, 0, 0};
 #define SPEC_RSTAMP(i) if (it == n_it / 2) rstamp[i] = __builtin_amdgcn_s_memtime()
 #define SPEC_RSTAMP_NEXT() if (it == n_it / 2 + 1u) rstamp[5] = __builtin_amdgcn_s_memtime()
 #define SPEC_RSTAMP_WRITE()                                                                                              \
     if (lane == 0u && SPEC_A->loss_slot && n_it > 16u + 8u * SPEC_MAX_WAVES) {                                           \
         asm volatile("s_waitcnt vmcnt(0)" ::: "memory");                                                                 \
-        for (int i = 1; i < 6; ++i) SPEC_A->loss_slot[16u + 8u * wave + i] = (float)(rstamp[i] - rstamp[0]);               \
+        for (int i = 1; i < 7; ++i) SPEC_A->loss_slot[16u + 8u * wave + i] = rstamp[i] ? (float)(rstamp[i] - rstamp[0]) : 0.0f; \
         SPEC_A->loss_slot[16u + 8u * wave] = 1.0f;                                                                       \
     }
 #else
@@ -453,6 +469,11 @@
         const uint32_t set_a = __builtin_amdgcn_readfirstlane(1u + j * per + (j < extra ? j : extra));
         const uint32_t n_sets = __builtin_amdgcn_readfirstlane(per + (j < extra ? 1u : 0u));
         const bool owners = __builtin_amdgcn_readfirstlane(wave == own_wave ? 1 : 0) != 0;
+        const float own_scale = -1.0f / (float)n_global;
+        (void)own_scale;
+#if SPEC_LEAN_OWNERS
+        if (W != SPEC_MAX_WAVES) __builtin_trap();
+#endif
         for (uint32_t it = 0; it < n_it; ++it) {
             const bool more = it + 1u < n_it, last = !more;
             spec_lds_barrier();
@@ -465,7 +486,7 @@
                 SPEC_RELOAD_ARGS();
                 const bsvi_opt_cfg cfg = SPEC_A->cfg;
 #pragma unroll
-                for (uint32_t e = 0; e < 2u; ++e) fac[e] = own.b[e] * spec_utransform_grad(own.tr[e], own.theta);
+                for (uint32_t e = 0; e < SPEC_OWN_ENTRIES; ++e) fac[e] = own.b[e] * spec_utransform_grad(own.tr[e], own.theta);
                 if (cfg.kind != BSVI_OPT_SGD) bias = optimizer_adam_bias(cfg, own.p1, own.p2);
                 if (more) {
                     draw_for(0u, off0 + it + 1u, Za);
@@ -477,9 +498,96 @@
                 draw_for(set_a, off0 + it + 1u, Za);
                 if (n_sets > 1u) draw_for(set_a + 1u, off0 + it + 1u, Zb);
             }
+#if SPEC_LEAN_OWNERS
+            typedef SPEC_GLOBAL_AS float* spec_gptr;
+            spec_gptr e_out = nullptr, e_loss = nullptr, e_finite = nullptr, e_params = nullptr, e_state = nullptr;
+            bsvi_opt_cfg e_cfg = {};
+            if (owners) {
+                SPEC_RELOAD_ARGS();
+                e_out = (spec_gptr)SPEC_A->out; e_loss = (spec_gptr)SPEC_A->loss_slot; e_finite = (spec_gptr)SPEC_A->finite_slot;
+                e_params = (spec_gptr)SPEC_A->params; e_state = (spec_gptr)SPEC_A->state;
+                e_cfg = SPEC_A->cfg;
+#if defined(__HIP_DEVICE_COMPILE__)
+                asm volatile("" : "+s"(e_out), "+s"(e_loss), "+s"(e_finite), "+s"(e_params), "+s"(e_state));
+                asm volatile("" : "+s"(e_cfg.kind), "+s"(e_cfg.lr), "+s"(e_cfg.momentum), "+s"(e_cfg.dampening), "+s"(e_cfg.weight_decay),
+                             "+s"(e_cfg.nesterov), "+s"(e_cfg.beta1), "+s"(e_cfg.beta2), "+s"(e_cfg.eps), "+s"(e_cfg.amsgrad), "+s"(e_cfg.maximize));
+#endif
+            }
+#endif
             SPEC_RSTAMP(1);
             spec_lds_barrier();
             SPEC_RSTAMP(2);
+#if SPEC_LEAN_OWNERS
+            if (owners) {
+                float ra[SPEC_MAX_WAVES], rb[SPEC_MAX_WAVES], rp[SPEC_MAX_WAVES];
+                spec_f4 rq[SPEC_MAX_WAVES / 2];
+#pragma unroll
+                for (uint32_t q = 0; q < SPEC_MAX_WAVES / 2; ++q) rq[q] = reinterpret_cast<const spec_f4*>(RED + 8)[q];
+#pragma unroll
+                for (uint32_t w = 0; w < SPEC_MAX_WAVES; ++w) rp[w] = WS[w * SPEC_WS_PAD + own.pos[0]];
+#if defined(__HIP_DEVICE_COMPILE__) && SPEC_MAX_WAVES == 8
+#define SPEC_PIN8(a) "+v"(a[0]), "+v"(a[1]), "+v"(a[2]), "+v"(a[3]), "+v"(a[4]), "+v"(a[5]), "+v"(a[6]), "+v"(a[7])
+                asm volatile("" : "+v"(rq[0]), "+v"(rq[1]), "+v"(rq[2]), "+v"(rq[3]), SPEC_PIN8(rp));
+#undef SPEC_PIN8
+#endif
+#pragma unroll
+                for (uint32_t w = 0; w < SPEC_MAX_WAVES; ++w) {
+                    ra[w] = (w & 1u) ? rq[w / 2].z : rq[w / 2].x;
+                    rb[w] = (w & 1u) ? rq[w / 2].w : rq[w / 2].y;
+                }
+                const float tot = spec_rows_total(rp);
+                const float vs = spec_rows_total(ra);
+                const float finite = isfinite(vs) ? 1.0f : 0.0f;
+                const uint32_t mask_bit = it <= pretraining ? 2u : 1u;
+                float grad = 0.0f;
+                if (own_fast) {
+                    float gsum = 0.0f;
+                    const float term = tot * fac[0];
+                    gsum += own.n > 0u ? term : 0.0f;
+                    grad = gsum * own_scale;
+                    SPEC_RSTAMP(3);
+                    if (finite != 0.0f && (own.mask & mask_bit)) {
+                        if (e_cfg.kind == BSVI_OPT_SGD) {
+                            optimizer_apply(e_cfg, own.theta, own.s0, own.s1, own.s2, own.st, grad);
+                        } else {
+                            optimizer_apply_adam_biased(e_cfg, own.theta, own.s0, own.s1, own.s2, own.st, grad, bias);
+                            own.p1 = bias.p1;
+                            own.p2 = bias.p2;
+                        }
+                    }
+                    if (more) {
+                        const float g0 = utransform_common(own.tr[0], own.theta);
+                        if (own.n > 0u) spec_store_uniform(own.k[0], own.a[0] + own.b[0] * g0);
+                    }
+                }
+                asm volatile("" ::: "memory");
+                SPEC_RSTAMP(6);
+                const float loss = -vs / (float)n_global;
+                if (oid == 0u) {
+                    const float vb = spec_rows_total(rb);
+                    if (last) { e_out[0] = vs; e_out[1] = vb; e_out[2] = loss; e_out[3] = finite; }
+                    if (e_loss) e_loss[it] = loss;
+                    if (e_finite) e_finite[it] = finite;
+                }
+                if (own_fast && last) {
+                    e_out[BSVI_OUT_HEADER + oid] = grad;
+                    e_params[oid] = own.theta;
+                    if (e_state) {
+                        e_state[oid] = own.s0;
+                        e_state[(size_t)SPEC_N_PARAMS + oid] = own.s1;
+                        e_state[2 * (size_t)SPEC_N_PARAMS + oid] = own.s2;
+                        e_state[3 * (size_t)SPEC_N_PARAMS + oid] = own.st;
+                    }
+                }
+            } else if (more) {
+#pragma unroll
+                for (uint32_t r = 0; r < SPEC_KEEP_NOISE; ++r) NZB[set_a * (SPEC_KEEP_NOISE * 64u) + 64u * r] = Za.z[r];
+                if (n_sets > 1u) {
+#pragma unroll
+                    for (uint32_t r = 0; r < SPEC_KEEP_NOISE; ++r) NZB[(set_a + 1u) * (SPEC_KEEP_NOISE * 64u) + 64u * r] = Zb.z[r];
+                }
+            }
+#else
             if (owners) {
                 SPEC_RELOAD_ARGS();
                 float* const out = SPEC_A->out;
@@ -495,7 +603,7 @@
                 }
                 float tot[2];
 #pragma unroll
-                for (uint32_t e = 0; e < 2u; ++e) tot[e] = spec_pos_total(WS, own.pos[e], W);
+                for (uint32_t e = 0; e < SPEC_OWN_ENTRIES; ++e) tot[e] = spec_pos_total(WS, own.pos[e], W);
                 const float finite = isfinite(vs) ? 1.0f : 0.0f;
                 const float loss = -vs / (float)n_global;
                 if (oid == 0u) {
@@ -508,7 +616,7 @@
                 if (own_fast) {
                     float gsum = 0.0f;
 #pragma unroll
-                    for (uint32_t e = 0; e < 2u; ++e) {
+                    for (uint32_t e = 0; e < SPEC_OWN_ENTRIES; ++e) {
                         const float term = tot[e] * fac[e];
                         gsum += e < own.n ? term : 0.0f;
                     }
@@ -550,6 +658,7 @@
                     for (uint32_t r = 0; r < SPEC_KEEP_NOISE; ++r) NZB[(set_a + 1u) * (SPEC_KEEP_NOISE * 64u) + 64u * r] = Zb.z[r];
                 }
             }
+#endif
             SPEC_RSTAMP(4);
         }
         SPEC_RSTAMP_WRITE();
@@ -844,7 +953,7 @@
                 const SpecOwn own = spec_own_load(OWN + 5 * oid);
                 float g = 0.0f;
 #pragma unroll
-                for (uint32_t e = 0; e < 2u; ++e) {
+                for (uint32_t e = 0; e < SPEC_OWN_ENTRIES; ++e) {
                     const float term = spec_pos_total(WS, own.pos[e], rows) * (own.b[e] * spec_utransform_grad(own.tr[e], own.theta));
                     g += e < own.n ? term : 0.0f;
                 }
@@ -875,9 +984,9 @@
                 const SpecOwn own = spec_own_load(OWN + 5 * oid);
                 float tot[2];
 #pragma unroll
-                for (uint32_t e = 0; e < 2u; ++e) tot[e] = spec_pos_total(WS, own.pos[e], rows);
-#pragma unroll
-                for (uint32_t e = 0; e < 2u; ++e) {
+                for (uint32_t e = 0; e < SPEC_OWN_ENTRIES; ++e) tot[e] = spec_pos_total(WS, own.pos[e], rows);
+#pragma unroll
+                for (uint32_t e = 0; e < SPEC_OWN_ENTRIES; ++e) {
                     const float term = tot[e] * (own.b[e] * spec_utransform_grad(own.tr[e], own.theta));
                     xgsum += e < own.n ? term : 0.0f;
                 }
@@ -905,10 +1014,10 @@
             SpecOwn own = spec_own_load(OWN + 5 * oid);
             float tot[2];
 #pragma unroll
-            for (uint32_t e = 0; e < 2u; ++e) tot[e] = spec_pos_total(WS, own.pos[e], rows);
+            for (uint32_t e = 0; e < SPEC_OWN_ENTRIES; ++e) tot[e] = spec_pos_total(WS, own.pos[e], rows);
             float gsum = 0.0f;
 #pragma unroll
-            for (uint32_t e = 0; e < 2u; ++e) {
+            for (uint32_t e = 0; e < SPEC_OWN_ENTRIES; ++e) {
                 const float term = tot[e] * (own.b[e] * spec_utransform_grad(own.tr[e], own.theta));
                 gsum += e < own.n ? term : 0.0f;
             }
@@ -938,7 +1047,7 @@
                     }
                 } else {
 #pragma unroll
-                    for (uint32_t e = 0; e < 2u; ++e)
+                    for (uint32_t e = 0; e < SPEC_OWN_ENTRIES; ++e)
                         if (e < own.n) spec_store_uniform(own.k[e], own.a[e] + own.b[e] * utransform_common(own.tr[e], own.theta));
                     OWN[5 * oid] = spec_f4{own.theta, own.s0, own.s1, own.s2};
                     spec_lds[SPEC_OFF_OWN + SPEC_OWN_WORDS * oid + 4] = own.st;
diff --git a/brancher_amd/csrc/spec_prelude.h b/brancher_amd/csrc/spec_prelude.h
--- a/brancher_amd/csrc/spec_prelude.h
+++ b/brancher_amd/csrc/spec_prelude.h
@@ -63,6 +63,11 @@
 #endif
     return x;
 }
+__device__ __forceinline__ float spec_plus(float a, float b) {
+#pragma clang fp contract(off)
+    return a + b;
+}
+__device__ __forceinline__ float spec_exact(float x) { return spec_plus(x, 0.0f); }
 __device__ __forceinline__ PhiloxKey spec_key(const SpecBody& A, const SpecLane& T) {
     return PhiloxKey{T.nidx, A.seed_lo, A.seed_hi, T.off_lo, T.off_hi};
 }
diff --git a/brancher_amd/csrc/specialize.cpp b/brancher_amd/csrc/specialize.cpp
--- a/brancher_amd/csrc/specialize.cpp
+++ b/brancher_amd/csrc/specialize.cpp
@@ -61,7 +61,7 @@
 
 class Emitter {
 public:
-    Emitter(const bsvi_program_desc& d, bool diag) : d_(d), diag_(diag) {
+    Emitter(const bsvi_program_desc& d, bool diag, bool fold = true) : d_(d), diag_(diag), fold_(fold) {
         keep_eps_ = d.n_noise <= kKeepEpsRows;
         direct_du_ = d.n_uniform_grad > kAccumulateEntries;
         reschedule_ = d.n_slots > kRescheduleAboveSlots;
@@ -122,12 +122,13 @@
 
 private:
     const bsvi_program_desc& d_;
-    bool diag_;
+    bool diag_, fold_;
     bool keep_eps_ = true, counting_ = true, direct_du_ = false, reschedule_ = true, two_pass_ = false;
     int sink_mode_ = 0;
     size_t visits_ = 0;
     std::string body_;
     std::vector<uint32_t> du_total_, du_seen_, order_;
+    std::set<uint32_t> sum_defined_;
     std::set<uint32_t> fwd_groups_, rev_groups_, all_groups_, eps_rows_, node_rows_, all_node_rows_, normal_rows_;
 
     Insn insn(uint32_t pc) const {
@@ -148,19 +149,47 @@
         const Opnd p = resolve(o, e);
         return p.lane ? fmt("v_%u", p.idx) : fmt("SPEC_U(%u)", p.idx);
     }
+    int literal(uint32_t o, uint32_t e) const {
+        if (!fold_) return -1;
+        const Opnd p = resolve(o, e);
+        if (p.lane || p.idx >= d_.n_uniform || !d_.consts) return -1;
+        const bsvi_uniform_entry& u = d_.uniform[p.idx];
+        if (u.is_param || u.transform != BSVI_UT_IDENTITY || u.a != 0.0f || u.b != 1.0f || u.src >= d_.n_consts) return -1;
+        uint32_t bits;
+        memcpy(&bits, d_.consts + u.src, 4);
+        return bits == 0x3f800000u ? 1 : (bits == 0u ? 0 : -1);
+    }
+    std::string exact_value(uint32_t o, uint32_t e) const {
+        const Opnd p = resolve(o, e);
+        return (!p.lane || sum_defined_.count(p.idx)) ? val(o, e) : "spec_exact(" + val(o, e) + ")";
+    }
+    std::string affine(uint32_t a, uint32_t b, uint32_t c, uint32_t e) const {
+        const int la = literal(a, e), lb = literal(b, e), lc = literal(c, e);
+        if (lb == 1 || la == 1) {
+            const uint32_t x = lb == 1 ? a : b;
+            return lc == 0 ? exact_value(x, e) : "spec_plus(" + val(x, e) + ", " + val(c, e) + ")";
+        }
+        if (lc == 0) return "__builtin_fmaf(" + val(a, e) + ", " + val(b, e) + ", 0.0f)";
+        return val(a, e) + " * " + val(b, e) + " + " + val(c, e);
+    }
+    void add_adj_times(uint32_t o, uint32_t e, const std::string& g, uint32_t factor) {
+        if (literal(factor, e) == 1) add_adj(o, e, g, true);
+        else add_adj(o, e, g + " * " + val(factor, e));
+    }
     void complete(uint32_t k, const std::string& expr) {
         if (counting_) return;
         const uint32_t pos = (uint32_t)order_.size();
         order_.push_back(k);
         line(fmt("SPEC_DU(%uu, %s);", pos, expr.c_str()));
     }
-    void add_adj(uint32_t o, uint32_t e, const std::string& expr) {
+    void add_adj(uint32_t o, uint32_t e, const std::string& expr, bool unfused = false) {
         const Opnd p = resolve(o, e);
-        if (p.lane) { line(fmt("a_%u += %s;", p.idx, expr.c_str())); return; }
+        const char* const form = unfused ? "%s_%u = spec_plus(%s_%u, %s);" : "%s_%u += %s;";
+        if (p.lane) { line(unfused ? fmt(form, "a", p.idx, "a", p.idx, expr.c_str()) : fmt(form, "a", p.idx, expr.c_str())); return; }
         if (p.idx >= d_.n_uniform_grad) return;
         if (counting_) { ++du_total_[p.idx]; return; }
         if (direct_du_) { complete(p.idx, expr); return; }
-        line(fmt("du_%u += %s;", p.idx, expr.c_str()));
+        line(unfused ? fmt(form, "du", p.idx, "du", p.idx, expr.c_str()) : fmt(form, "du", p.idx, expr.c_str()));
         if (++du_seen_[p.idx] == du_total_[p.idx]) complete(p.idx, fmt("du_%u", p.idx));
     }
 
@@ -213,13 +242,13 @@
             ++visits_;
             if (counting_) return;
             line("{");
-            line(fmt("  const float loc = %s * %s + %s;", val(I.a, e).c_str(), val(I.b, e).c_str(), val(I.c, e).c_str()));
+            line(fmt("  const float loc = %s;", affine(I.a, I.b, I.c, e).c_str()));
             std::string v = val(I.dst, e);
             if (flags & BSVI_F_SAMPLE) {
                 const uint32_t row = resolve(I.dst, e).idx;
                 const std::string eps = eps_forward(row);
                 if (flags & BSVI_F_GIVEN) line(fmt("  %s = %s;", v.c_str(), eps.c_str()));
-                else line(fmt("  %s = loc + %s * %s;", v.c_str(), eps.c_str(), val(I.s, e).c_str()));
+                else { line(fmt("  %s = loc + %s * %s;", v.c_str(), eps.c_str(), val(I.s, e).c_str())); sum_defined_.insert(row); }
                 diag_outputs(row, v, eps);
             }
             if (flags & (BSVI_F_ENT | BSVI_F_LOGP | BSVI_F_WF)) line(fmt("  const float lS = %s;", log_of(I.s, e).c_str()));
@@ -283,21 +312,21 @@
 
     void naff_sink(const Insn& I, uint32_t e) {
         ++visits_;
-        const std::string A = val(I.a, e), B = val(I.b, e);
+        const std::string loc = affine(I.a, I.b, I.c, e);
         if (sink_mode_ == 1) {
-            line(fmt("T.f += %s * spec_naff_lp(%s, %s * %s + %s, %s, %s);", flit(I.imm0).c_str(), val(I.dst, e).c_str(), A.c_str(), B.c_str(),
-                     val(I.c, e).c_str(), rcp_of(I.s, e).c_str(), log_of(I.s, e).c_str()));
+            line(fmt("T.f += %s * spec_naff_lp(%s, %s, %s, %s);", flit(I.imm0).c_str(), val(I.dst, e).c_str(), loc.c_str(),
+                     rcp_of(I.s, e).c_str(), log_of(I.s, e).c_str()));
             return;
         }
         if (!counting_) {
             line("{");
-            line(fmt("  float gl, gs; spec_naff_sink(%s, %s, %s * %s + %s, %s, %s, %s, gl, gs);", flit(I.imm0).c_str(), val(I.dst, e).c_str(),
-                     A.c_str(), B.c_str(), val(I.c, e).c_str(), rcp_of(I.s, e).c_str(), log_of(I.s, e).c_str(), ftarget()));
+            line(fmt("  float gl, gs; spec_naff_sink(%s, %s, %s, %s, %s, %s, gl, gs);", flit(I.imm0).c_str(), val(I.dst, e).c_str(),
+                     loc.c_str(), rcp_of(I.s, e).c_str(), log_of(I.s, e).c_str(), ftarget()));
             if (diag_) line("  gl *= T.gw; gs *= T.gw;");
         }
         add_adj(I.dst, e, "-gl");
-        add_adj(I.a, e, "gl * " + B);
-        add_adj(I.b, e, "gl * " + A);
+        add_adj_times(I.a, e, "gl", I.b);
+        add_adj_times(I.b, e, "gl", I.a);
         add_adj(I.c, e, "gl");
         add_adj(I.s, e, "gs");
         line("}");
@@ -307,10 +336,10 @@
         const uint32_t op = I.w0 & 0xFFu, flags = (I.w0 >> 8) & 0xFFu, dist = (I.w0 >> 16) & 0xFFu;
         ++visits_;
         if (op == BSVI_OP_NAFF) {
-            const std::string A = val(I.a, e), B = val(I.b, e), v = val(I.dst, e);
+            const std::string v = val(I.dst, e);
             if (!counting_) {
                 line("{");
-                line(fmt("  const float rS = %s, loc = %s * %s + %s;", rcp_of(I.s, e).c_str(), A.c_str(), B.c_str(), val(I.c, e).c_str()));
+                line(fmt("  const float rS = %s, loc = %s;", rcp_of(I.s, e).c_str(), affine(I.a, I.b, I.c, e).c_str()));
                 line("  float gv = 0.0f, gl = 0.0f, gs = 0.0f;");
                 if (flags & (BSVI_F_LOGP | BSVI_F_WF)) {
                     const std::string gw = (flags & BSVI_F_WF) ? fmt("(%s + fweight)", wg(I.imm0).c_str()) : wg(I.imm0);
@@ -329,8 +358,8 @@
             } else {
                 add_adj(I.dst, e, "gv");
             }
-            add_adj(I.a, e, "gl * " + B);
-            add_adj(I.b, e, "gl * " + A);
+            add_adj_times(I.a, e, "gl", I.b);
+            add_adj_times(I.b, e, "gl", I.a);
             add_adj(I.c, e, "gl");
             add_adj(I.s, e, "gs");
             line("}");
@@ -548,7 +577,7 @@
     uint32_t n_pos = 0;
     Geom geom[2];
     std::vector<uint32_t> pu_ptr_host, pu_pos_host, pu_idx_host;
-    Variant variant[7];
+    Variant variant[8];
     bool exchange_ok = false;
     void* dev = nullptr;
     unsigned int* tickets = nullptr;
@@ -612,10 +641,18 @@
     uint32_t ut_mask = 0;
     for (uint32_t k = 0; k < d.n_uniform; ++k) ut_mask |= 1u << (d.uniform[k].transform & 31u);
     const bool rare_transforms = (ut_mask >> (BSVI_UT_SIGMOID + 1)) != 0;
+    uint32_t own_entries = 1;
+    for (uint32_t i = 0; i < d.n_params; ++i) own_entries = std::max(own_entries, std::min(2u, s->pu_ptr_host[i + 1] - s->pu_ptr_host[i]));
+    const char* const lean_env = getenv("BSVI_SPEC_LEAN_BODY");
+    const bool lean_body = !(lean_env && lean_env[0] == '0');
+    const bool want_previous = getenv("BSVI_SPEC_LEAN_CHAIN") != nullptr;
+    std::string previous;
     for (int gi = 0; gi < 2; ++gi) {
         const Geom& G = s->geom[gi];
-        for (int v = 0; v < 2; ++v) {
-            Emitter E(d, v == 1);
+        for (int v = 0; v < (gi == GEOM_ONE && want_previous ? 3 : 2); ++v) {
+            const bool old = v == 2;
+            const bool lean = lean_body && !old;
+            Emitter E(d, v == 1, lean);
             if (!E.run(why)) { delete s; return nullptr; }
             std::string src;
             src += "// generated by libbsvi (specialize.cpp) from a model program: do not edit\n";
@@ -629,12 +666,13 @@
             src += fmt("#define SPEC_N_PARAMS %u\n#define SPEC_N_UNIFORM %u\n#define SPEC_N_UGRAD %u\n#define SPEC_N_OBS %u\n#define SPEC_N_NOISE %u\n",
                        d.n_params, d.n_uniform, d.n_uniform_grad, d.n_obs, d.n_noise);
             src += fmt("#define SPEC_N_POS %u\n", s->n_pos);
-            src += fmt("#define SPEC_ESTIMATOR %u\n#define SPEC_MAX_THREADS %u\n#define SPEC_DIAG %d\n", d.estimator, G.max_threads, v);
+            src += fmt("#define SPEC_ESTIMATOR %u\n#define SPEC_MAX_THREADS %u\n#define SPEC_DIAG %d\n", d.estimator, G.max_threads, v == 1 ? 1 : 0);
             src += fmt("#define SPEC_ACCUMULATE_CHUNKS %d\n#define SPEC_TILE %d\n", gi == GEOM_MANY ? 1 : 0, tiled(s->n_pos, gi) ? 1 : 0);
             if (gi == GEOM_MANY && many_waves() > 2) src += fmt("#define SPEC_BOUND_THREADS %u\n", 256u * many_waves());
             src += fmt("#define SPEC_KEEP_NOISE %u\n", E.keeps_noise() ? d.n_noise : 0u);
             src += fmt("#define SPEC_GENERIC_OWNERS %d\n", all_fast ? 0 : 1);
             src += fmt("#define SPEC_RARE_TRANSFORMS %d\n#define SPEC_UT_MASK 0x%xu\n", rare_transforms ? 1 : 0, ut_mask);
+            if (!old) src += fmt("#define SPEC_OWN_ENTRIES %u\n", own_entries);
             src += "#include \"spec_prelude.h\"\n";
             src += "namespace bsvi {\n";
             src += "__device__ __forceinline__ void spec_draw(const SpecBody& A, const SpecLane& T, SpecNoise& Z) {\n";
@@ -644,6 +682,7 @@
             src += "__device__ __forceinline__ void spec_body(const SpecBody& A, SpecLane& T, const SpecNoise& Z, float* WSw) {\n";
             src += "    (void)Z;\n";
             if (v == 1) src += "    const float* const noise = A.noise;\n";
+            if (old) { previous = std::move(src); previous += E.declarations() + E.body() + "}\n}  // namespace bsvi\n#include \"spec_main.h\"\n"; continue; }
             src += E.declarations();
             src += E.body();
             src += "}\n}  // namespace bsvi\n";
@@ -652,7 +691,8 @@
         }
     }
     s->variant[4].src = "#define SPEC_WITH_DRAW_WAVE 1\n" + s->variant[0].src;
-    s->variant[6].src = "#define SPEC_WITH_DRAW_WAVE 1\n#define SPEC_WITH_DRAW_OWNERS 1\n" + s->variant[0].src;
+    s->variant[6].src = "#define SPEC_WITH_DRAW_WAVE 1\n#define SPEC_WITH_DRAW_OWNERS 1\n#define SPEC_LEAN_CHAIN 1\n" + s->variant[0].src;
+    if (want_previous) s->variant[7].src = "#define SPEC_WITH_DRAW_WAVE 1\n#define SPEC_WITH_DRAW_OWNERS 1\n" + previous;
     s->exchange_ok = true;
     s->variant[5].src = std::string("#define SPEC_WITH_EXCHANGE 1\n") + (s->draw_wave_ok ? "#define SPEC_WITH_DRAW_WAVE 1\n" : "") + s->variant[0].src;
     return s;
@@ -687,7 +727,7 @@
     return BSVI_OK;
 }
 
-const std::string& source(const Spec* s, int variant) { return s->variant[(variant >= 4 && variant <= 6) ? variant : (variant & 3)].src; }
+const std::string& source(const Spec* s, int variant) { return s->variant[(variant >= 4 && variant <= 7) ? variant : (variant & 3)].src; }
 
 static const char* kJitOptions[] = {"--offload-arch=gfx950", "-O3", "-std=c++17", "-Xclang", "-target-feature", "-Xclang", "-packed-fp32-ops"};
 static const int kJitOptionCount = (int)(sizeof(kJitOptions) / sizeof(kJitOptions[0]));
@@ -854,6 +894,7 @@
 }
 
 static thread_local int t_last_source = 0;
+static thread_local int t_last_variant = -1;
 
 int obtain(const std::string& text, std::vector<char>& code, std::string& log, int* origin) {
     {
@@ -885,6 +926,7 @@
 }
 
 int last_origin() { return t_last_source; }
+int last_variant() { return t_last_variant; }
 std::string cache_directory() { return disk_cache::enabled() ? disk_cache::directory() : std::string(); }
 std::string compiler_identity() { return disk_cache::compiler_identity(); }
 
@@ -922,6 +964,10 @@
     const char* e = getenv("BSVI_SPEC_OWNER_WAVE");
     return !(e && e[0] == '0');
 }
+static bool lean_chain() {
+    const char* e = getenv("BSVI_SPEC_LEAN_CHAIN");
+    return !(e && e[0] == '0');
+}
 static Geo geo(const Spec* s, uint32_t n_local, int mode = MODE_SUMS, bool exchange = false) {
     const uint32_t waves = (n_local + 63) / 64;
     if (waves <= s->geom[GEOM_ONE].max_threads / 64) {
@@ -932,7 +978,8 @@
                              && waves + n_service <= s->geom[GEOM_ONE].max_threads / 64 && (size_t)s->n_noise * 64u * waves <= (size_t)n_service * 64u * 68u
                              && !s->variant[exchange ? 5 : 4].failed;
         const uint32_t more = service ? n_service : extra ? 1u : 0u;
-        const bool owners = service && (size_t)s->n_noise * 64u * (waves + 1u) <= (size_t)n_service * 64u * 68u;
+        const bool owners = service && (size_t)s->n_noise * 64u * (waves + 1u) <= (size_t)n_service * 64u * 68u
+                            && waves + n_service == s->geom[GEOM_ONE].max_threads / 64;
         return Geo{1, (waves + more) * 64, GEOM_ONE, more != 0u, more, owners};
     }
     const uint32_t threads = s->geom[GEOM_MANY].max_threads;
@@ -987,9 +1034,11 @@
             v = 5;
         }
         else if (g.draw_owners && v == 0 && owner_wave()) {
-            const int rc6 = ensure_compiled(s, 6);
+            v = lean_chain() ? 6 : 7;
+            if (v == 7 && s->variant[7].src.empty())
+                return bsvi_fail(BSVI_ERR_UNSUPPORTED, "BSVI_SPEC_LEAN_CHAIN=0 needs the variable set when the program is created (the previous source is generated then)");
+            const int rc6 = ensure_compiled(s, v);
             if (rc6) return rc6;
-            v = 6;
         }
         else if (g.draw_wave && v == 0 && ensure_compiled(s, 4) == BSVI_OK) v = 4;
         else if (g.draw_wave) { g.threads -= 64 * g.extra_waves; g.draw_wave = false; }
@@ -1039,6 +1088,7 @@
     void* config[] = {HIP_LAUNCH_PARAM_BUFFER_POINTER, &A, HIP_LAUNCH_PARAM_BUFFER_SIZE, &size, HIP_LAUNCH_PARAM_END};
     const hipError_t e = hipModuleLaunchKernel(s->variant[v].fn, g.blocks, 1, 1, g.threads, 1, 1, 0, (hipStream_t)a->stream, nullptr, config);
     if (e != hipSuccess) return bsvi_fail(BSVI_ERR_HIP, std::string("hipModuleLaunchKernel (specialised kernel): ") + hipGetErrorString(e));
+    t_last_variant = v;
     return BSVI_OK;
 }
 
diff --git a/brancher_amd/native.py b/brancher_amd/native.py
--- a/brancher_amd/native.py
+++ b/brancher_amd/native.py
@@ -125,6 +125,7 @@
     "bsvi_jit_compile": (C.c_int, [C.c_char_p, C.POINTER(C.c_size_t)]),
     "bsvi_jit_load": (C.c_int, [C.c_char_p, C.POINTER(C.c_size_t), C.POINTER(C.c_int)]),
     "bsvi_jit_last_origin": (C.c_int, []),
+    "bsvi_spec_last_variant": (C.c_int, []),
     "bsvi_jit_cache_dir": (C.c_size_t, [C.c_char_p, C.c_size_t]),
     "bsvi_jit_compiler_identity": (C.c_size_t, [C.c_char_p, C.c_size_t]),
     "bsvi_program_engine": (C.c_int, [C.c_void_p, C.c_uint32, C.c_int, C.POINTER(C.c_uint32), C.POINTER(C.c_uint32),
diff --git a/include/bsvi.h b/include/bsvi.h
--- a/include/bsvi.h
+++ b/include/bsvi.h
@@ -217,6 +217,7 @@
 int bsvi_jit_compile(const char* source, size_t* code_bytes);
 int bsvi_jit_load(const char* source, size_t* code_bytes, int* origin);
 int bsvi_jit_last_origin(void);
+int bsvi_spec_last_variant(void);
 size_t bsvi_jit_cache_dir(char* buf, size_t capacity);
 size_t bsvi_jit_compiler_identity(char* buf, size_t capacity);
 int bsvi_program_engine(const bsvi_program* prog, uint32_t n_local, int mode, uint32_t* n_blocks, uint32_t* n_threads,
```

New measurement: 294,100 (median of 6 runs). 1.04x the previous value.
